# Dipet/pytorch_yolo

Measured on AMD Instinct MI355X. Metric: images/sec YOLOv3-SPP 640x640 bs=32, forward + decode + MERGE-NMS, pipelined batches, higher is better.
Workload: dtype bf16

## Files before the change

### include/yolo_hip.h

```cpp
#ifndef YOLO_HIP_H
#define YOLO_HIP_H

#include <stddef.h>
#include <stdint.h>

#ifdef __cplusplus
extern "C" {
#endif

typedef void* yolo_stream_t;

#if defined(__GNUC__)
#define YOLO_API __attribute__((visibility("default")))
#else
#define YOLO_API
#endif

enum { YOLO_E_ARG = -1, YOLO_E_UNSUPPORTED = -2, YOLO_E_WORKSPACE = -3 };
enum { YOLO_ACT_NONE = 0, YOLO_ACT_LEAKY01 = 1, YOLO_ACT_RELU6 = 2, YOLO_ACT_RELU = 3,
       YOLO_ACT_SWISH = 4  };
enum { YOLO_DT_BF16 = 0, YOLO_DT_F32 = 1, YOLO_DT_F16 = 2  };

YOLO_API const char* yolo_last_error(void);
YOLO_API int yolo_abi_version(void);
YOLO_API int yolo_set_tuning(int knob, int value);

YOLO_API int yolo_pack_input_nchw_f32(const float* x, void* y, int n, int c, int h, int w, int c_pad,
                             yolo_stream_t s);

typedef struct YoloConvDesc {
  int32_t n, h, w;
  int32_t cin;
  int32_t in_c_total, in_c_offset;
  int32_t ho, wo;
  int32_t cout;
  int32_t out_c_total, out_c_offset;
  int32_t ksize, stride, pad;
  int32_t act;
  int32_t upsample2x;
  int32_t out_dtype;
  int32_t kpad;
  int32_t cout_pad;
  int32_t res_c_total, res_c_offset;
  int32_t aux_c_total, aux_c_offset;
} YoloConvDesc;

YOLO_API int yolo_conv2d_fwd(const void* x, const void* w_packed, const float* bias, const void* residual,
                    void* y, void* y_preadd, const YoloConvDesc* d, yolo_stream_t s);

YOLO_API int yolo_conv2d_pick(const YoloConvDesc* d, int has_residual, int has_preadd, char* out, int out_len);

YOLO_API int yolo_conv2d_splitk_plan(const YoloConvDesc* d, int has_residual, int has_preadd, int* splits, size_t* ws_bytes,
                                     int* n_counters);
YOLO_API int yolo_conv2d_splitk_fwd(const void* x, const void* w_packed, const float* bias, const void* residual, void* y,
                                    void* y_preadd, const YoloConvDesc* d, int splits, void* workspace, size_t ws_bytes,
                                    int32_t* counters, yolo_stream_t s);

YOLO_API int yolo_conv1_nchw_f32_fwd(const float* x_nchw, int cin_real, const void* w_packed, const float* bias,
                                     void* y, const YoloConvDesc* d, yolo_stream_t s);
YOLO_API int yolo_conv1_pool_nchw_f32_fwd(const float* x_nchw, int cin_real, const void* w_packed, const float* bias,
                                          void* y_pooled, const YoloConvDesc* d, yolo_stream_t s);

YOLO_API int yolo_pack_conv_weight_f32(const float* w_oihw, int cout, int cin_w, int ksize, int cin,
                              int cout_pad, int kpad, uint16_t* out);

YOLO_API int yolo_conv3x3_pool_supported(int cin, int cout);
YOLO_API int yolo_conv3x3_pool_fwd(const void* x, const void* w_packed, const float* bias, void* y, const YoloConvDesc* d,
                                   int pool, yolo_stream_t s);

YOLO_API int yolo_dwconv3x3_fwd(const void* x, const float* w, const float* bias, void* y, int n, int h, int w_,
                       int c, int in_c_total, int in_c_offset, int ho, int wo, int out_c_total,
                       int out_c_offset, int stride, int act, yolo_stream_t s);

YOLO_API int yolo_dwconv_fwd(const void* x, const float* w, const float* bias, void* y, int n, int h, int w_, int c,
                             int in_c_total, int in_c_offset, int ho, int wo, int out_c_total, int out_c_offset, int ksize,
                             int stride, int pad, int act, yolo_stream_t s);

YOLO_API size_t yolo_se_workspace_bytes(int n, int c);
YOLO_API int yolo_se_fwd(const void* x, void* y, int n, int h, int w, int c, int in_c_total, int in_c_offset, int out_c_total,
                         int out_c_offset, const float* w1, const float* b1, const float* w2, const float* b2, int squeeze,
                         void* workspace, size_t ws_bytes, yolo_stream_t s);

YOLO_API int yolo_channel_shuffle2_fwd(const void* a, const void* b, void* y, int n, int h, int w, int half, int c_slot,
                                       int a_c_total, int a_c_offset, int b_c_total, int b_c_offset, int y_c_total,
                                       int y_c_offset, yolo_stream_t s);

YOLO_API int yolo_maxpool_fwd(const void* x, void* y, int n, int h, int w, int c, int in_c_total, int in_c_offset,
                     int ho, int wo, int out_c_total, int out_c_offset, int ksize, int stride, int pad,
                     int dilation, yolo_stream_t s);

YOLO_API int yolo_spp_fwd(void* buf, int n, int h, int w, int c, yolo_stream_t s);

YOLO_API int yolo_resunit_supported(int c, int h, int w);
YOLO_API int yolo_resunit_form(int c, int n, int h, int w);
YOLO_API int yolo_resunit_fwd(const void* x, const void* w1_packed, const float* b1, const void* w2_packed,
                              const float* b2, void* y, void* y_preadd, const YoloConvDesc* d, int kpad1,
                              int cout_pad1, yolo_stream_t s);

YOLO_API int yolo_stem_supported(int cin_real, int c1, int c2, int h, int w);
YOLO_API int yolo_stem_fwd(const float* x_nchw, int cin_real, const void* w1_packed, const float* b1, int kpad1,
                           const void* w2_packed, const float* b2, void* y, const YoloConvDesc* d, yolo_stream_t s);

typedef struct YoloMbconvDesc {
  int32_t n, h, w, cin, in_c_total, in_c_offset, hidden, cout, out_c_total, out_c_offset, stride, has_expand, has_res, _pad;
} YoloMbconvDesc;
YOLO_API int yolo_mbconv_dstride(int ce);
YOLO_API int yolo_mbconv_supported(int cin, int hidden, int cout, int stride);
YOLO_API int yolo_mbconv_fwd(const void* x, const void* w_exp, const float* b_exp, const float* w_dw, const float* b_dw,
                             const void* w_proj, const float* b_proj, void* y, const YoloMbconvDesc* d, yolo_stream_t s);

YOLO_API int yolo_decode_fwd(const float* head, int head_c_total, const float* anchors_px, int na, int nc, int bs,
                    int ny, int nx, float stride_px, float* io, int io_rows_total, int io_row_offset,
                    float* p, yolo_stream_t s);

YOLO_API int yolo_head_decode_supported(int cout, int na, int nc);
YOLO_API int yolo_head_decode_pick(const YoloConvDesc* d, int na, int nc, int filter, char* out, int out_len);
YOLO_API int yolo_head_decode_fwd(const void* x, const void* w_packed, const float* bias, const YoloConvDesc* d,
                                  const float* anchors_px, int na, int nc, float stride_px, float* io,
                                  int io_rows_total, int io_row_offset, float* p, yolo_stream_t s);

YOLO_API size_t yolo_nms_workspace_bytes(int bs, int rows, int nc);
YOLO_API int yolo_nms_merge(float* pred, int bs, int rows, int nc, float conf_thres, float nms_thres, float min_wh,
                   int max_per_class, int mutate_conf, float* out_dets, int32_t* out_idx,
                   int32_t* out_count, int cap, void* workspace, size_t workspace_bytes, yolo_stream_t s);

YOLO_API size_t yolo_nms_compact_workspace_bytes(int bs, int rows, int nc);
YOLO_API int yolo_head_decode_filter_fwd(const void* x, const void* w_packed, const float* bias, const YoloConvDesc* d,
                                         const float* anchors_px, int na, int nc, float stride_px, int io_rows_total,
                                         int io_row_offset, float conf_thres, float min_wh, void* workspace, size_t workspace_bytes,
                                         float* p, yolo_stream_t s);
YOLO_API int yolo_nms_merge_compact(void* workspace, size_t workspace_bytes, int bs, int rows, int nc, float nms_thres,
// ... 89 lines not shown
```

### pytorch_yolo_amd/_lib.py

```python
from __future__ import annotations

import ctypes as C
import os

_HERE = os.path.dirname(os.path.abspath(__file__))
LIB_PATH = os.environ.get("YOLO_HIP_LIB") or os.path.join(_HERE, "csrc", "libyolo_hip.so")

ABI_VERSION = 2
ACT_NONE, ACT_LEAKY01, ACT_RELU6, ACT_RELU, ACT_SWISH = 0, 1, 2, 3, 4
DT_BF16, DT_F32, DT_F16 = 0, 1, 2
OP_CONV, OP_MAXPOOL, OP_SPP, OP_DWCONV, OP_CONV1_NCHW, OP_RESUNIT, OP_STEM, OP_HEAD_DECODE, OP_CONV1_POOL = 1, 2, 3, 4, 5, 6, 7, 8, 9
OP_MBCONV, OP_CONV_POOL, OP_SHUFFLE, OP_CONV_F32, OP_MAXPOOL_F32, OP_SE = 10, 11, 12, 13, 14, 15
OP_CONV_F16, OP_MAXPOOL_F16, OP_HEAD_DECODE_F16 = 16, 17, 18
OP_CONV_T20_F16 = 19


class YoloConvDesc(C.Structure):
    _fields_ = [(n, C.c_int32) for n in (
        "n", "h", "w", "cin", "in_c_total", "in_c_offset", "ho", "wo", "cout",
        "out_c_total", "out_c_offset", "ksize", "stride", "pad", "act", "upsample2x",
        "out_dtype", "kpad", "cout_pad", "res_c_total", "res_c_offset",
        "aux_c_total", "aux_c_offset")]


class YoloOp(C.Structure):
    _fields_ = [("kind", C.c_int32), ("_pad", C.c_int32),
                ("x", C.c_void_p), ("w", C.c_void_p), ("bias", C.c_void_p),
                ("residual", C.c_void_p), ("y", C.c_void_p), ("y_aux", C.c_void_p),
                ("conv", YoloConvDesc),
                ("w_pre", C.c_void_p), ("bias_pre", C.c_void_p), ("kpad_pre", C.c_int32), ("cout_pad_pre", C.c_int32),
                ("head_anchors_px", C.c_float * 8), ("head_stride_px", C.c_float),
                ("head_na", C.c_int32), ("head_nc", C.c_int32), ("io_rows_total", C.c_int32),
                ("io_row_offset", C.c_int32), ("head_filter_conf", C.c_float),
                ("w_dw", C.c_void_p), ("bias_dw", C.c_void_p),
                ("workspace", C.c_void_p), ("counters", C.c_void_p), ("ws_bytes", C.c_size_t),
                ("splits", C.c_int32), ("head_filter_min_wh", C.c_float)]


class YoloMbconvDesc(C.Structure):
    _fields_ = [(n, C.c_int32) for n in (
        "n", "h", "w", "cin", "in_c_total", "in_c_offset", "hidden", "cout", "out_c_total", "out_c_offset",
        "stride", "has_expand", "has_res", "_pad")]


class YoloPipeStep(C.Structure):
    _fields_ = [("ops", C.POINTER(YoloOp)), ("n_ops", C.c_int32), ("k_io", C.c_int32),
                ("stream", C.c_void_p), ("nms_stream", C.c_void_p),
                ("wait_x", C.c_void_p), ("wait_io", C.c_void_p), ("heads_done", C.c_void_p), ("nms_done", C.c_void_p), ("done", C.c_void_p),
                ("io", C.c_void_p), ("bs", C.c_int32), ("rows", C.c_int32), ("nc", C.c_int32), ("max_per_class", C.c_int32),
                ("conf_thres", C.c_float), ("nms_thres", C.c_float), ("min_wh", C.c_float), ("cap", C.c_int32),
                ("out_dets", C.c_void_p), ("out_idx", C.c_void_p), ("out_count", C.c_void_p), ("workspace", C.c_void_p),
                ("workspace_bytes", C.c_size_t), ("count_host", C.c_void_p)]


SIGNATURES = {
    "yolo_last_error": (C.c_char_p, []),
    "yolo_abi_version": (C.c_int, []),
    "yolo_abi_sizeof": (C.c_int, [C.c_int]),
    "yolo_set_tuning": (C.c_int, [C.c_int, C.c_int]),
    "yolo_pack_input_nchw_f32": (C.c_int, [C.c_void_p, C.c_void_p] + [C.c_int] * 5 + [C.c_void_p]),
    "yolo_conv2d_fwd": (C.c_int, [C.c_void_p] * 6 + [C.POINTER(YoloConvDesc), C.c_void_p]),
    "yolo_conv2d_splitk_plan": (C.c_int, [C.POINTER(YoloConvDesc), C.c_int, C.c_int, C.POINTER(C.c_int), C.POINTER(C.c_size_t),
                                          C.POINTER(C.c_int)]),
    "yolo_conv2d_splitk_fwd": (C.c_int, [C.c_void_p] * 6 + [C.POINTER(YoloConvDesc), C.c_int, C.c_void_p, C.c_size_t, C.c_void_p,
                                         C.c_void_p]),
    "yolo_conv1_nchw_f32_fwd": (C.c_int, [C.c_void_p, C.c_int, C.c_void_p, C.c_void_p, C.c_void_p,
                                          C.POINTER(YoloConvDesc), C.c_void_p]),
    "yolo_conv1_pool_nchw_f32_fwd": (C.c_int, [C.c_void_p, C.c_int, C.c_void_p, C.c_void_p, C.c_void_p,
                                               C.POINTER(YoloConvDesc), C.c_void_p]),
    "yolo_conv2d_pick": (C.c_int, [C.POINTER(YoloConvDesc), C.c_int, C.c_int, C.c_char_p, C.c_int]),
    "yolo_pack_conv_weight_f32": (C.c_int, [C.c_void_p] + [C.c_int] * 6 + [C.c_void_p]),
    "yolo_stem_supported": (C.c_int, [C.c_int] * 5),
    "yolo_stem_fwd": (C.c_int, [C.c_void_p, C.c_int, C.c_void_p, C.c_void_p, C.c_int, C.c_void_p, C.c_void_p, C.c_void_p,
                                C.POINTER(YoloConvDesc), C.c_void_p]),
    "yolo_resunit_supported": (C.c_int, [C.c_int] * 3),
    "yolo_resunit_form": (C.c_int, [C.c_int] * 4),
    "yolo_resunit_fwd": (C.c_int, [C.c_void_p] * 7 + [C.POINTER(YoloConvDesc), C.c_int, C.c_int, C.c_void_p]),
    "yolo_conv3x3_pool_supported": (C.c_int, [C.c_int] * 2),
    "yolo_conv3x3_pool_fwd": (C.c_int, [C.c_void_p] * 4 + [C.POINTER(YoloConvDesc), C.c_int, C.c_void_p]),
    "yolo_mbconv_dstride": (C.c_int, [C.c_int]),
    "yolo_mbconv_supported": (C.c_int, [C.c_int] * 4),
    "yolo_mbconv_fwd": (C.c_int, [C.c_void_p] * 8 + [C.POINTER(YoloMbconvDesc), C.c_void_p]),
    "yolo_dwconv3x3_fwd": (C.c_int, [C.c_void_p] * 4 + [C.c_int] * 12 + [C.c_void_p]),
    "yolo_dwconv_fwd": (C.c_int, [C.c_void_p] * 4 + [C.c_int] * 14 + [C.c_void_p]),
    "yolo_se_workspace_bytes": (C.c_size_t, [C.c_int] * 2),
    "yolo_se_fwd": (C.c_int, [C.c_void_p] * 2 + [C.c_int] * 8 + [C.c_void_p] * 4 + [C.c_int, C.c_void_p, C.c_size_t, C.c_void_p]),
    "yolo_channel_shuffle2_fwd": (C.c_int, [C.c_void_p] * 3 + [C.c_int] * 11 + [C.c_void_p]),
    "yolo_maxpool_fwd": (C.c_int, [C.c_void_p] * 2 + [C.c_int] * 14 + [C.c_void_p]),
    "yolo_spp_fwd": (C.c_int, [C.c_void_p] + [C.c_int] * 4 + [C.c_void_p]),
    "yolo_decode_fwd": (C.c_int, [C.c_void_p, C.c_int, C.c_void_p] + [C.c_int] * 5 + [C.c_float, C.c_void_p,
                                  C.c_int, C.c_int, C.c_void_p, C.c_void_p]),
    "yolo_head_decode_supported": (C.c_int, [C.c_int] * 3),
    "yolo_head_decode_pick": (C.c_int, [C.POINTER(YoloConvDesc), C.c_int, C.c_int, C.c_int, C.c_char_p, C.c_int]),
    "yolo_head_decode_fwd": (C.c_int, [C.c_void_p] * 3 + [C.POINTER(YoloConvDesc), C.c_void_p, C.c_int, C.c_int, C.c_float,
                                       C.c_void_p, C.c_int, C.c_int, C.c_void_p, C.c_void_p]),
    "yolo_nms_workspace_bytes": (C.c_size_t, [C.c_int] * 3),
    "yolo_nms_merge": (C.c_int, [C.c_void_p] + [C.c_int] * 3 + [C.c_float] * 3 + [C.c_int] * 2 +
                       [C.c_void_p] * 3 + [C.c_int, C.c_void_p, C.c_size_t, C.c_void_p]),
    "yolo_nms_compact_workspace_bytes": (C.c_size_t, [C.c_int] * 3),
    "yolo_head_decode_filter_fwd": (C.c_int, [C.c_void_p] * 3 + [C.POINTER(YoloConvDesc), C.c_void_p, C.c_int, C.c_int, C.c_float,
                                              C.c_int, C.c_int, C.c_float, C.c_float, C.c_void_p, C.c_size_t, C.c_void_p, C.c_void_p]),
    "yolo_nms_merge_compact": (C.c_int, [C.c_void_p, C.c_size_t] + [C.c_int] * 3 + [C.c_float, C.c_int] + [C.c_void_p] * 3 +
                               [C.c_int, C.c_void_p]),
    "yolo_scale_coords": (C.c_int, [C.c_void_p, C.c_int, C.c_int, C.c_int, C.c_void_p, C.c_int, C.c_void_p]),
    "yolo_letterbox_u8_fwd": (C.c_int, [C.c_void_p] + [C.c_int] * 4 + [C.c_double] + [C.c_int] * 6 + [C.c_void_p, C.c_void_p] +
                              [C.c_int] * 4 + [C.c_float, C.c_void_p]),
    "yolo_conv2d_f32_fwd": (C.c_int, [C.c_void_p] * 6 + [C.POINTER(YoloConvDesc), C.c_void_p]),
    "yolo_maxpool_f32_fwd": (C.c_int, [C.c_void_p] * 2 + [C.c_int] * 14 + [C.c_void_p]),
    "yolo_pack_input_nchw_f32_nhwc": (C.c_int, [C.c_void_p, C.c_void_p] + [C.c_int] * 5 + [C.c_void_p]),
    "yolo_pack_conv_weight_f32_f32": (C.c_int, [C.c_void_p] + [C.c_int] * 6 + [C.c_void_p]),
    "yolo_conv2d_f16_fwd": (C.c_int, [C.c_void_p] * 6 + [C.POINTER(YoloConvDesc), C.c_void_p]),
    "yolo_conv3x3_t20_f16_supported": (C.c_int, [C.POINTER(YoloConvDesc), C.c_int, C.c_int]),
    "yolo_conv3x3_t20_f16_fwd": (C.c_int, [C.c_void_p] * 6 + [C.POINTER(YoloConvDesc), C.c_int, C.c_void_p]),
    "yolo_conv2d_f16_pick": (C.c_int, [C.POINTER(YoloConvDesc), C.c_int, C.c_int, C.c_char_p, C.c_int]),
    "yolo_head_decode_f16_pick": (C.c_int, [C.POINTER(YoloConvDesc), C.c_int, C.c_int, C.c_int, C.c_char_p, C.c_int]),
    "yolo_head_decode_f16_fwd": (C.c_int, [C.c_void_p] * 3 + [C.POINTER(YoloConvDesc), C.c_void_p, C.c_int, C.c_int, C.c_float,
                                           C.c_void_p, C.c_int, C.c_int, C.c_void_p, C.c_void_p]),
    "yolo_head_decode_filter_f16_fwd": (C.c_int, [C.c_void_p] * 3 + [C.POINTER(YoloConvDesc), C.c_void_p, C.c_int, C.c_int, C.c_float,
                                                  C.c_int, C.c_int, C.c_float, C.c_float, C.c_void_p, C.c_size_t, C.c_void_p, C.c_void_p]),
    "yolo_maxpool_f16_fwd": (C.c_int, [C.c_void_p] * 2 + [C.c_int] * 14 + [C.c_void_p]),
    "yolo_pack_input_nchw_f32_f16": (C.c_int, [C.c_void_p, C.c_void_p] + [C.c_int] * 5 + [C.c_void_p]),
    "yolo_pack_conv_weight_f32_f16": (C.c_int, [C.c_void_p] + [C.c_int] * 6 + [C.c_void_p]),
    "yolo_run_ops": (C.c_int, [C.POINTER(YoloOp), C.c_int, C.c_void_p]),
    "yolo_stream_create_cu_mask": (C.c_int, [C.POINTER(C.c_uint32), C.c_int, C.POINTER(C.c_void_p)]),
    "yolo_stream_destroy": (C.c_int, [C.c_void_p]),
    "yolo_set_launch_cus": (C.c_int, [C.c_int]),
    "yolo_event_create": (C.c_int, [C.POINTER(C.c_void_p)]),
    "yolo_event_destroy": (C.c_int, [C.c_void_p]),
    "yolo_event_record": (C.c_int, [C.c_void_p, C.c_void_p]),
    "yolo_event_synchronize": (C.c_int, [C.c_void_p]),
    "yolo_pipeline_step": (C.c_int, [C.POINTER(YoloPipeStep)]),
    "yolo_pack_detections": (C.c_int, [C.c_void_p, C.c_void_p, C.c_void_p, C.c_int, C.c_int, C.c_void_p, C.c_void_p, C.c_void_p]),
}

_lib = None


def load():
    global _lib
    if _lib is not None:
        return _lib
    if not os.path.exists(LIB_PATH):
        raise RuntimeError(
            f"{LIB_PATH} is missing: build it with `python -m pytorch_yolo_amd.build` "
            "(hipcc --offload-arch=gfx950). pytorch_yolo_amd has no CPU / eager fallback.")
    lib = C.CDLL(LIB_PATH)
    for name, (res, args) in SIGNATURES.items():
        fn = getattr(lib, name)
        fn.restype = res
        fn.argtypes = args
    if lib.yolo_abi_version() != ABI_VERSION:
        raise RuntimeError(f"libyolo_hip.so ABI version {lib.yolo_abi_version()} != {ABI_VERSION} of this binding: rebuild with "
                           "`python -m pytorch_yolo_amd.build --force`")
# ... 12 lines not shown
```

### pytorch_yolo_amd/csrc/conv1x1_stream.hip

```cpp
#include "conv_common.h"

using namespace yolo_conv;

namespace {

struct ActParams {
  bool floor0, swish;
  float slope, hi;
  __device__ explicit ActParams(int act)
      : floor0(act == YOLO_ACT_RELU || act == YOLO_ACT_RELU6), swish(act == YOLO_ACT_SWISH), slope(act == YOLO_ACT_LEAKY01 ? 0.1f : 1.f),
        hi(act_hi(act)) {}
  __device__ __forceinline__ float plain(float v) const { return fminf(fmaxf(v, floor0 ? 0.f : slope * v), hi); }
};

template <int N, int K>
__global__ __launch_bounds__(256, 2) void conv1x1_stream_kernel(const ConvArgs a, int n_tiles_px) {
  constexpr int P = 128, NF = N / 64, KC = K / 32;
  constexpr int XB = KC * P * 64;
  constexpr int SP = N * 2 + 16;
  static_assert((N == 64 || N == 128) && (K == 128 || K == 256), "shape");
  __shared__ __attribute__((aligned(16))) char smem[XB > P * SP ? XB : P * SP];

  const int tid = threadIdx.x, lane = tid & 63;
  const int wave = __builtin_amdgcn_readfirstlane(tid >> 6);
  const YoloConvDesc& d = a.d;
  const ActParams ap(d.act);
  const int c16 = lane & 15, q = lane >> 4;
  const __amdgpu_buffer_rsrc_t rx = __builtin_amdgcn_make_buffer_rsrc((void*)a.x, 0, a.x_bytes, 0x00020000);
  const uint32_t y_pitch = (uint32_t)d.out_c_total * 2u;
  const __amdgpu_buffer_rsrc_t ry = __builtin_amdgcn_make_buffer_rsrc(a.y, 0, (uint32_t)a.M * y_pitch, 0x00020000);

  bf16x8 wreg[NF][KC];
  f32x4 bv[NF];
#pragma unroll
  for (int f = 0; f < NF; ++f) {
    const int row = wave * 16 * NF + f * 16 + c16;
#pragma unroll
    for (int kc = 0; kc < KC; ++kc) wreg[f][kc] = *reinterpret_cast<const bf16x8*>(a.w + (long)row * d.kpad + kc * 32 + q * 8);
    bv[f] = *reinterpret_cast<const f32x4*>(a.bias + wave * 16 * NF + f * 16 + q * 4);
  }
  const int drow = lane >> 2, dchunk = (lane & 3) ^ swz32(lane >> 4);
  const uint32_t x_pitch = (uint32_t)d.in_c_total * 2u;
  const uint32_t lane_src = (uint32_t)drow * x_pitch + (uint32_t)(d.in_c_offset + dchunk * 8) * 2u;
  const uint32_t xfrag = (uint32_t)(c16 * 64 + ((q ^ swz32(c16 >> 2)) << 4));
  constexpr int LPR = N / 8, RPI = 64 / LPR;
  const int orow = lane / LPR, ocol = lane % LPR;

  for (int t = blockIdx.x; t < n_tiles_px; t += gridDim.x) {
    const int p0 = t * P;
#pragma unroll
    for (int i = 0; i < KC * 2; ++i) {
      const int piece = i * 4 + wave, kc = piece >> 3, pb = piece & 7;
      const int px = p0 + pb * 16 + drow;
      const uint32_t vo = px < a.M ? (uint32_t)(p0 + pb * 16) * x_pitch + lane_src : kOobOffset;
      if (!(a.debug & kCdNoPixelDma)) lds_dma16s(rx, smem + piece * 1024, vo, (uint32_t)kc * 64u);
    }
    wait_vmcnt<0>();
    __syncthreads();
    f32x4 acc[NF][8];
#pragma unroll
    for (int f = 0; f < NF; ++f)
#pragma unroll
      for (int j = 0; j < 8; ++j) acc[f][j] = f32x4{0.f, 0.f, 0.f, 0.f};
    if (!(a.debug & kCdNoMfma))
#pragma unroll
    for (int kc = 0; kc < KC; ++kc)
#pragma unroll
      for (int j = 0; j < 8; ++j) {
        const bf16x8 xf = *reinterpret_cast<const bf16x8*>(smem + (kc * 8 + j) * 1024 + xfrag);
#pragma unroll
        for (int f = 0; f < NF; ++f) acc[f][j] = __builtin_amdgcn_mfma_f32_16x16x32_bf16(wreg[f][kc], xf, acc[f][j], 0, 0, 0);
      }
    __syncthreads();
    if (a.debug & kCdNoEpilogue) continue;
    auto stage = [&](auto act) {
#pragma unroll
      for (int f = 0; f < NF; ++f)
#pragma unroll
        for (int j = 0; j < 8; ++j) {
          bf16x4 o;
#pragma unroll
          for (int e = 0; e < 4; ++e) o[e] = (bf16_t)act(acc[f][j][e] + bv[f][e]);
          *reinterpret_cast<bf16x4*>(smem + (j * 16 + c16) * SP + (wave * 16 * NF + f * 16 + q * 4) * 2) = o;
        }
    };
    if (ap.swish) stage([](float v) { return v / (1.f + expf(-v)); });
    else stage([&](float v) { return ap.plain(v); });
    __syncthreads();
#pragma unroll
    for (int i = 0; i < P / (4 * RPI); ++i) {
      const int row = (i * 4 + wave) * RPI + orow;
      const u32x4 v = *reinterpret_cast<const u32x4*>(smem + row * SP + ocol * 16);
      const uint32_t vo = p0 + row < a.M ? (uint32_t)(p0 + row) * y_pitch + (uint32_t)(d.out_c_offset + ocol * 8) * 2u : kOobOffset;
      __builtin_amdgcn_raw_buffer_store_b128(v, ry, vo, 0, 0);
    }
    wait_lds();
    __builtin_amdgcn_s_barrier();
  }
}

template <int N, int K, int P>
__global__ __launch_bounds__(256, 2) void conv1x1_stream2_kernel(const ConvArgs a, int n_tiles_px) {
  constexpr int NF = N / 64, KC = K / 32, PB = P / 16;
  constexpr int XB = KC * P * 64;
  constexpr int SP = N * 2 + 16;
  constexpr int NPW = KC * PB / 4;
  constexpr int LPR = N / 8, RPI = 64 / LPR, NST = P / (4 * RPI);
  constexpr int BUF = ((XB > P * SP ? XB : P * SP) + 1023) / 1024 * 1024;
  static_assert(N == 128 && (KC * PB) % 4 == 0 && P % (4 * RPI) == 0 && 2 * BUF <= 80 * 1024, "shape");
  static_assert(NPW + 2 * NST <= 60, "vmcnt is a 6-bit counter");
  __shared__ __attribute__((aligned(16))) char smem[2 * BUF];

  const int tid = threadIdx.x, lane = tid & 63;
  const int wave = __builtin_amdgcn_readfirstlane(tid >> 6);
  const YoloConvDesc& d = a.d;
  const ActParams ap(d.act);
  const int c16 = lane & 15, q = lane >> 4;
  const __amdgpu_buffer_rsrc_t rx = __builtin_amdgcn_make_buffer_rsrc((void*)a.x, 0, a.x_bytes, 0x00020000);
  const uint32_t y_pitch = (uint32_t)d.out_c_total * 2u;
  const __amdgpu_buffer_rsrc_t ry = __builtin_amdgcn_make_buffer_rsrc(a.y, 0, (uint32_t)a.M * y_pitch, 0x00020000);

  bf16x8 wreg[NF][KC];
  f32x4 bv[NF];
#pragma unroll
  for (int f = 0; f < NF; ++f) {
    const int row = wave * 16 * NF + f * 16 + c16;
#pragma unroll
    for (int kc = 0; kc < KC; ++kc) wreg[f][kc] = *reinterpret_cast<const bf16x8*>(a.w + (long)row * d.kpad + kc * 32 + q * 8);
    bv[f] = *reinterpret_cast<const f32x4*>(a.bias + wave * 16 * NF + f * 16 + q * 4);
  }
  const int drow = lane >> 2, dchunk = (lane & 3) ^ swz32(lane >> 4);
  const uint32_t x_pitch = (uint32_t)d.in_c_total * 2u;
  const uint32_t lane_src = (uint32_t)drow * x_pitch + (uint32_t)(d.in_c_offset + dchunk * 8) * 2u;
  const uint32_t xfrag = (uint32_t)(c16 * 64 + ((q ^ swz32(c16 >> 2)) << 4));
  const int orow = lane / LPR, ocol = lane % LPR;

  auto issue_tile = [&](int j) {
    const long t = (long)blockIdx.x + (long)j * gridDim.x;
    const long p0 = t * P;
    char* const buf = smem + (j & 1) * BUF;
#pragma unroll
    for (int i = 0; i < NPW; ++i) {
      const int piece = i * 4 + wave, kc = piece / PB, pb = piece - kc * PB;
      const long px = p0 + pb * 16 + drow;
      const uint32_t vo = (t < n_tiles_px && px < a.M) ? (uint32_t)(p0 + pb * 16) * x_pitch + lane_src : kOobOffset;
      lds_dma16s(rx, buf + piece * 1024, vo, (uint32_t)kc * 64u);
    }
#if defined(__HIP_DEVICE_COMPILE__)
    asm volatile("" ::: "memory");
#endif
  };

  const int nt = ((int)blockIdx.x < n_tiles_px) ? (n_tiles_px - 1 - (int)blockIdx.x) / (int)gridDim.x + 1 : 0;
  issue_tile(0);
  issue_tile(1);
  for (int j = 0; j < nt; ++j) {
    const long p0 = ((long)blockIdx.x + (long)j * gridDim.x) * P;
    char* const buf = smem + (j & 1) * BUF;
    if (j == 0) wait_vmcnt<NPW>();
    else if (j == 1) wait_vmcnt<NPW + NST>();
    else wait_vmcnt<NPW + 2 * NST>();
    __builtin_amdgcn_s_barrier();
    f32x4 acc[NF][PB];
#pragma unroll
    for (int f = 0; f < NF; ++f)
#pragma unroll
      for (int b = 0; b < PB; ++b) acc[f][b] = f32x4{0.f, 0.f, 0.f, 0.f};
#pragma unroll
    for (int kc = 0; kc < KC; ++kc)
#pragma unroll
      for (int b = 0; b < PB; ++b) {
        const bf16x8 xf = *reinterpret_cast<const bf16x8*>(buf + (kc * PB + b) * 1024 + xfrag);
#pragma unroll
        for (int f = 0; f < NF; ++f) acc[f][b] = __builtin_amdgcn_mfma_f32_16x16x32_bf16(wreg[f][kc], xf, acc[f][b], 0, 0, 0);
      }
    wait_lds();
    __builtin_amdgcn_s_barrier();
    auto stage = [&](auto act) {
#pragma unroll
      for (int f = 0; f < NF; ++f)
#pragma unroll
        for (int b = 0; b < PB; ++b) {
          bf16x4 o;
#pragma unroll
          for (int e = 0; e < 4; ++e) o[e] = (bf16_t)act(acc[f][b][e] + bv[f][e]);
          *reinterpret_cast<bf16x4*>(buf + (b * 16 + c16) * SP + (wave * 16 * NF + f * 16 + q * 4) * 2) = o;
        }
    };
    if (ap.swish) stage([](float v) { return v / (1.f + expf(-v)); });
    else stage([&](float v) { return ap.plain(v); });
    wait_lds();
    __builtin_amdgcn_s_barrier();
    u32x4 v[NST];
#pragma unroll
    for (int i = 0; i < NST; ++i) v[i] = *reinterpret_cast<const u32x4*>(buf + ((i * 4 + wave) * RPI + orow) * SP + ocol * 16);
    wait_lds();
    __builtin_amdgcn_s_barrier();
    issue_tile(j + 2);
#pragma unroll
    for (int i = 0; i < NST; ++i) {
      const int row = (i * 4 + wave) * RPI + orow;
      const uint32_t vo = p0 + row < a.M ? (uint32_t)(p0 + row) * y_pitch + (uint32_t)(d.out_c_offset + ocol * 8) * 2u : kOobOffset;
      __builtin_amdgcn_raw_buffer_store_b128(v[i], ry, vo, 0, 0);
    }
#if defined(__HIP_DEVICE_COMPILE__)
    asm volatile("" ::: "memory");
#endif
  }
  wait_vmcnt<0>();
}

template <int N, int K, int P>
int launch_stream2(const ConvArgs& a, hipStream_t s) {
  const int tiles = (a.M + P - 1) / P;
  const int grid = tiles < 512 ? tiles : 512;
  if (pick_only("stream1x1p<%d couts,K %d,%d px> grid %d", N, K, P, grid)) return 0;
  hipLaunchKernelGGL((conv1x1_stream2_kernel<N, K, P>), dim3((unsigned)grid), dim3(256), 0, s, a, tiles);
  return yolo_check_launch("yolo_conv2d_fwd(1x1 stream, pipelined)");
}

template <int N, int K>
int launch_stream(const ConvArgs& a, hipStream_t s) {
  const int tiles = (a.M + 127) / 128;
  const int grid = tiles < 512 ? tiles : 512;
  if (pick_only("stream1x1<%d couts,K %d> grid %d", N, K, grid)) return 0;
  hipLaunchKernelGGL((conv1x1_stream_kernel<N, K>), dim3((unsigned)grid), dim3(256), 0, s, a, tiles);
  return yolo_check_launch("yolo_conv2d_fwd(1x1 stream)");
}

}

int yolo_conv::launch_stream1x1(const ConvArgs& a, int force, hipStream_t s) {
  const YoloConvDesc& d = a.d;
  if (d.ksize != 1 || d.stride != 1 || d.pad != 0 || d.upsample2x || d.out_dtype != YOLO_DT_BF16 || a.res || a.aux) return 1;
  if (d.in_c_offset % 8 || d.in_c_total % 8 || d.out_c_offset % 8 || d.out_c_total % 8) return 1;
  if ((size_t)a.M * d.out_c_total * 2 >= kOobOffset) return 1;
  if (!force && a.M < 40000) return 1;
  if (!(a.debug & kCdStreamFirstForm)) {
    if (d.cout == 128 && d.cin == 256) return launch_stream2<128, 256, 80>(a, s);
    if (d.cout == 128 && d.cin == 128) return launch_stream2<128, 128, 80>(a, s);
    if (d.cout == 128 && d.cin == 384) return launch_stream2<128, 384, 48>(a, s);
  }
  if (d.cout == 128 && d.cin == 256) return launch_stream<128, 256>(a, s);
  if (d.cout == 128 && d.cin == 128) return launch_stream<128, 128>(a, s);
  if (d.cout == 64 && d.cin == 128) return launch_stream<64, 128>(a, s);
  if (d.cout == 64 && d.cin == 256) return launch_stream<64, 256>(a, s);
  return 1;
}
```

### pytorch_yolo_amd/csrc/conv_common.h

```cpp
#pragma once
#include "common.h"

#include <type_traits>
#include <utility>

namespace yolo_conv {

template <typename F, int... Is>
__device__ __forceinline__ void static_for_impl(F&& f, std::integer_sequence<int, Is...>) {
  (f(std::integral_constant<int, Is>{}), ...);
}
template <int N, typename F>
__device__ __forceinline__ void static_for(F&& f) {
  static_for_impl(f, std::make_integer_sequence<int, N>{});
}

template <typename T>
struct Pack;
template <>
struct Pack<bf16_t> {
  using x4 = bf16x4;
  using x8 = bf16x8;
};
template <>
struct Pack<f16_t> {
  using x4 = f16x4;
  using x8 = f16x8;
};
template <typename T>
__device__ __forceinline__ T narrow(float v) {
  if constexpr (std::is_same<T, f16_t>::value) {
    const float m = __builtin_fabsf(v);
    if (m > 65504.f && m < __builtin_inff()) v = __builtin_copysignf(65504.f, v);
  }
  return (T)v;
}

constexpr uint32_t kOobOffset = 0xF0000000u;

struct HeadDecodeArgs {
  float* io = nullptr;
  float* p = nullptr;
  int na = 0, no = 0, io_rows_total = 0, io_row_offset = 0;
  float stride = 0.f;
  float anchor_w[4] = {}, anchor_h[4] = {};
  float* rec = nullptr;
  unsigned long long* row_keys = nullptr;
  float conf_thres = 0.f, min_wh = 0.f;
};

struct ConvArgs {
  const bf16_t* x = nullptr;
  const bf16_t* w = nullptr;
  const float* bias = nullptr;
  const bf16_t* res = nullptr;
  void* y = nullptr;
  bf16_t* aux = nullptr;
  YoloConvDesc d = {};
  int M = 0;
  int n_tiles = 0;
  int steps = 0;
  uint32_t x_bytes = 0, w_bytes = 0;
  HeadDecodeArgs hd;
  int splits = 1;
  float* ws = nullptr;
  int* cnt = nullptr;
  int debug = 0;
#ifdef YOLO_STAMPS
  unsigned long long* stamps = nullptr;
#endif
};

inline size_t conv_x_bytes(const YoloConvDesc& d) { return (size_t)d.n * d.h * d.w * d.in_c_total * 2; }
inline size_t conv_w_bytes(const YoloConvDesc& d) { return (size_t)d.cout_pad * d.kpad * 2; }

inline ConvArgs make_conv_args(const void* x, const void* w, const float* bias, const void* res, void* y, void* aux, const YoloConvDesc& d) {
  ConvArgs a;
  a.x = (const bf16_t*)x;
  a.w = (const bf16_t*)w;
  a.bias = bias;
  a.res = (const bf16_t*)res;
  a.y = y;
  a.aux = (bf16_t*)aux;
  a.d = d;
  a.M = d.n * d.ho * d.wo;
  a.x_bytes = (uint32_t)conv_x_bytes(d);
  a.w_bytes = (uint32_t)conv_w_bytes(d);
  return a;
}

#ifdef YOLO_STAMPS
struct BlockStamp {
  unsigned long long* base_;
  unsigned long long* p;
  unsigned long long t0, c0;
  __device__ __forceinline__ unsigned long long* slot_() const {
    return base_ + 4 * ((size_t)blockIdx.x + (size_t)gridDim.x * (blockIdx.y + (size_t)gridDim.y * blockIdx.z)) + 1;
  }
  __device__ __forceinline__ explicit BlockStamp(unsigned long long* base) : base_(base), p(nullptr), t0(0), c0(0) {
    if (base && threadIdx.x == 0) {
      p = slot_() - 1;
      t0 = __builtin_amdgcn_s_memrealtime();
      c0 = __builtin_amdgcn_s_memtime();
    }
  }
  __device__ __forceinline__ ~BlockStamp() {
    if (p) {
      const unsigned long long c1 = __builtin_amdgcn_s_memtime();
      const unsigned hw = __builtin_amdgcn_s_getreg((31 << 11) | 4), xcc = __builtin_amdgcn_s_getreg((31 << 11) | 20);
      p[0] = t0;
      p[2] = c1 - c0;
      p[3] = (unsigned long long)hw | ((unsigned long long)xcc << 32);
    }
    if ((threadIdx.x & 63) == 0 && base_) atomicMax(slot_(), (unsigned long long)__builtin_amdgcn_s_memrealtime());
  }
};
inline unsigned long long* stamp_buffer_from_env() {
  static long launch_idx = 0;
  const char* e = getenv("YOLO_STAMP_PTR");
  if (!e) return nullptr;
  const char* st = getenv("YOLO_STAMP_STRIDE");
  const long stride = st ? atol(st) : 0;
  return (unsigned long long*)strtoull(e, nullptr, 0) + stride * launch_idx++;
}
#define YOLO_BLOCK_STAMP(args) BlockStamp block_stamp_((args).stamps)
#define YOLO_SET_STAMPS(args) (args).stamps = stamp_buffer_from_env()
#else
#define YOLO_BLOCK_STAMP(args)
#define YOLO_SET_STAMPS(args)
#endif

__device__ __forceinline__ void lds_dma16(__amdgpu_buffer_rsrc_t rsrc, char* lds_wave_base, uint32_t voffset) {
  __builtin_amdgcn_raw_ptr_buffer_load_lds(rsrc, (__attribute__((address_space(3))) void*)lds_wave_base, 16,
                                           voffset, 0, 0, 0);
}

__device__ __forceinline__ int swz32(int v) { return (0x78 >> (2 * (v & 3))) & 3; }

__device__ __forceinline__ float act_hi(int act) { return act == YOLO_ACT_RELU6 ? 6.f : __builtin_nanf(""); }

__device__ __forceinline__ float apply_act(float v, int act) {
  if (act == YOLO_ACT_SWISH) return v / (1.f + expf(-v));
  const bool floor0 = act == YOLO_ACT_RELU || act == YOLO_ACT_RELU6;
  const float slope = act == YOLO_ACT_LEAKY01 ? 0.1f : 1.f;
  return fminf(fmaxf(v, floor0 ? 0.f : slope * v), act_hi(act));
}

template <int N>
__device__ __forceinline__ void wait_vmcnt() {
#if defined(__HIP_DEVICE_COMPILE__)
  asm volatile("s_waitcnt vmcnt(%0)" ::"n"(N) : "memory");
#endif
}

typedef float f32x2 __attribute__((ext_vector_type(2)));
__device__ __forceinline__ float raw_max(float x, float y) {
  float r;
// ... 163 lines not shown
```

### pytorch_yolo_amd/csrc/conv_igemm.hip

```cpp
#include "conv_common.h"
#include "nms_common.h"
#include "head_epilogue.h"
#include <stdlib.h>

using namespace yolo_conv;

#ifdef YOLO_ABL_NOLDS
template <typename X8>
__device__ __forceinline__ X8 lds_frag_stub() {
  X8 v;
  asm volatile("" : "=v"(v));
  return v;
}
#define YOLO_LDS_FRAG(p) lds_frag_stub<X8>()
#else
#define YOLO_LDS_FRAG(p) (*reinterpret_cast<const X8*>(p))
#endif

namespace {

__device__ __forceinline__ f32x4 mfma16(bf16x8 w, bf16x8 x, f32x4 c) { return __builtin_amdgcn_mfma_f32_16x16x32_bf16(w, x, c, 0, 0, 0); }
__device__ __forceinline__ f32x4 mfma16(f16x8 w, f16x8 x, f32x4 c) { return __builtin_amdgcn_mfma_f32_16x16x32_f16(w, x, c, 0, 0, 0); }
__device__ __forceinline__ f32x16 mfma32(bf16x8 w, bf16x8 x, f32x16 c) { return __builtin_amdgcn_mfma_f32_32x32x16_bf16(w, x, c, 0, 0, 0); }
__device__ __forceinline__ f32x16 mfma32(f16x8 w, f16x8 x, f32x16 c) { return __builtin_amdgcn_mfma_f32_32x32x16_f16(w, x, c, 0, 0, 0); }

template <int BM, int BN, int WAVES_M, int WAVES_N, int BK, int NS, bool FAST, bool LDS_EPI, bool MFMA16 = false, bool DECODE = false,
          int NP = 0, bool SPLITK = false, typename T = bf16_t>
__global__ __launch_bounds__(64 * (WAVES_M * WAVES_N + NP)) void conv_igemm_kernel(const ConvArgs a) {
  using X4 = typename Pack<T>::x4;
  using X8 = typename Pack<T>::x8;
  static_assert(!SPLITK || (FAST && LDS_EPI && MFMA16 && !DECODE), "split-K: 16x16x32 path with the LDS epilogue");
  constexpr int NW = WAVES_M * WAVES_N;
  constexpr int NL = NP > 0 ? NP : NW;
  static_assert(NP == 0 || (NS <= 3 && FAST && NP % 2 == 0), "loader waves: 2- or 3-stage ring, FAST path");
  static_assert(NW == 4 || NW == 8 || NW == 16, "4, 8 or 16 waves");
  static_assert(BK == 32 || BK == 64, "BK");
  static_assert(NS >= 2 && NS <= 4, "ring depth");
  constexpr int TM = BM / WAVES_M, TN = BN / WAVES_N;
  constexpr int NI = TM / 32, MI = TN / 32;
  constexpr int ROWB = BK * 2;
  constexpr int CPR = BK / 8;
  constexpr int RPP = 1024 / ROWB;
  constexpr int BNL = BN < NL * RPP ? NL * RPP : BN;
  constexpr int PIT = BM / (NL * RPP), WIT = BNL / (NL * RPP);
  constexpr int LPS = PIT + WIT;
  constexpr int STAGE_B = (BM + BNL) * ROWB;
  static_assert(TM % 32 == 0 && TN % 32 == 0 && PIT >= 1 && WIT >= 1, "tile");
  static_assert(NS * STAGE_B <= 160 * 1024, "LDS");

  constexpr int RING_B = NS * STAGE_B;
  constexpr int DP = BN + 4;
  constexpr int EPI_B = DECODE ? BM * DP * 4 : (LDS_EPI ? NW * TM * kEpiPitch : 0);
  constexpr int LDS_B = EPI_B > RING_B ? EPI_B : RING_B;
  static_assert(!DECODE || (!LDS_EPI && !MFMA16 && BM % NW == 0), "DECODE instances use the plain 32x32 accumulators");
  __shared__ __attribute__((aligned(16))) char smem[LDS_B];

  YOLO_BLOCK_STAMP(a);
  const int tid = threadIdx.x, lane = tid & 63;
  const int wave = __builtin_amdgcn_readfirstlane(tid >> 6);
  const int wm = wave / WAVES_N, wn = wave % WAVES_N;
  const int lw = NP == 0 ? wave : wave - NW;
  const YoloConvDesc& d = a.d;

  int m0, n0;
  {
    const int swz = xcd_swizzle(blockIdx.x, gridDim.x);
    const int mt = swz / a.n_tiles;
    m0 = mt * BM;
    n0 = (swz - mt * a.n_tiles) * BN;
  }

  const __amdgpu_buffer_rsrc_t rx = __builtin_amdgcn_make_buffer_rsrc((void*)a.x, 0, a.x_bytes, 0x00020000);
  const __amdgpu_buffer_rsrc_t rw = __builtin_amdgcn_make_buffer_rsrc((void*)a.w, 0, a.w_bytes, 0x00020000);

  const int frow = lane / CPR;
  const int fsw = (BK == 32) ? swz32(lane >> 4) : (((lane >> 4) + 4 * (lw & 1)) & 7);
  const int chunk = (lane & (CPR - 1)) ^ fsw;
  const int ntaps = d.ksize * d.ksize;
  int px_base[PIT], px_hi0[PIT], px_wi0[PIT];
  uint32_t px_mask[PIT];
  const int hw_out = d.ho * d.wo;
#pragma unroll
  for (int it = 0; it < PIT; ++it) {
    const int m = m0 + (it * NL + lw) * RPP + frow;
    const bool ok = m < a.M;
    const int mm = ok ? m : 0;
    const int b = mm / hw_out, rem = mm - b * hw_out;
    const int oh = rem / d.wo, ow = rem - oh * d.wo;
    px_hi0[it] = oh * d.stride - d.pad;
    px_wi0[it] = ow * d.stride - d.pad;
    px_base[it] = ((b * d.h + px_hi0[it]) * d.w + px_wi0[it]) * d.in_c_total + d.in_c_offset;
    uint32_t mask;
    if (d.ksize == 3) {
      uint32_t cb = 0, rb = 0;
#pragma unroll
      for (int t = 0; t < 3; ++t) {
        cb |= (uint32_t)((unsigned)(px_wi0[it] + t) < (unsigned)d.w) << t;
        rb |= (uint32_t)((unsigned)(px_hi0[it] + t) < (unsigned)d.h) << t;
      }
      mask = ((rb & 1) ? cb : 0) | ((rb & 2) ? cb << 3 : 0) | ((rb & 4) ? cb << 6 : 0);
    } else {
      mask = ((unsigned)px_hi0[it] < (unsigned)d.h && (unsigned)px_wi0[it] < (unsigned)d.w) ? 1u : 0u;
    }
    if (!ok) mask = 0;
    px_mask[it] = mask;
    if (FAST) px_base[it] = (px_base[it] + chunk * 8) * 2;
  }
  uint32_t w_off[WIT];
#pragma unroll
  for (int it = 0; it < WIT; ++it) {
    const int row = (it * NL + lw) * RPP + frow;
    w_off[it] = row < BN ? (uint32_t)(((n0 + row) * d.kpad + chunk * 8) * 2) : kOobOffset;
  }
  int tap = FAST ? 0 : (chunk * 8) / d.cin;
  int kc = FAST ? 0 : chunk * 8 - tap * d.cin;
  if constexpr (SPLITK) {
    const int k0 = blockIdx.y * a.steps * BK;
    tap = k0 / d.cin;
    kc = k0 - tap * d.cin;
#pragma unroll
    for (int it = 0; it < WIT; ++it)
      if (w_off[it] != kOobOffset) w_off[it] += (uint32_t)k0 * 2u;
  }

  int st_dh = 0, st_dw = 0;
  auto stage_begin = [&]() {
    st_dh = st_dw = 0;
    if (d.ksize == 3) {
      st_dh = (tap * 11) >> 5;
      st_dw = tap - 3 * st_dh;
    }
  };
  auto issue = [&](int buf, int step, int lo, int hi) {
    char* const wb = smem + buf * STAGE_B + lw * 1024;
    char* const xb = wb + BNL * ROWB;
    if (FAST) {
      const uint32_t tap_off = (uint32_t)(((st_dh * d.w + st_dw) * d.in_c_total + kc) * 2);
      const uint32_t bit = (kc + chunk * 8 < d.cin) ? 1u << tap : 0u;
#pragma unroll
      for (int it = 0; it < PIT; ++it) {
        if (it < lo || it >= hi) continue;
        const uint32_t voff = (px_mask[it] & bit) ? (uint32_t)px_base[it] + tap_off : kOobOffset;
        if (!(a.debug & kCdNoPixelDma)) lds_dma16(rx, xb + it * (NL * 1024), voff);
      }
#pragma unroll
      for (int it = 0; it < WIT; ++it) {
        if (PIT + it < lo || PIT + it >= hi) continue;
        if (!(a.debug & kCdNoWeightDma)) lds_dma16s(rw, wb + it * (NL * 1024), w_off[it], (uint32_t)step * (BK * 2u));
      }
    } else {
      const bool tap_ok = tap < ntaps;
      const int tap_off = (st_dh * d.w + st_dw) * d.in_c_total + kc;
#pragma unroll
      for (int it = 0; it < PIT; ++it) {
        if (it < lo || it >= hi) continue;
        const bool ok = tap_ok && ((px_mask[it] >> (tap_ok ? tap : 0)) & 1u);
        const uint32_t voff = ok ? (uint32_t)(px_base[it] + tap_off) * 2u : kOobOffset;
        lds_dma16(rx, xb + it * (NL * 1024), voff);
      }
#pragma unroll
      for (int it = 0; it < WIT; ++it) {
        if (PIT + it < lo || PIT + it >= hi) continue;
        const uint32_t voff = w_off[it] == kOobOffset ? kOobOffset : w_off[it] + (uint32_t)step * (BK * 2u);
        lds_dma16(rw, wb + it * (NL * 1024), voff);
      }
    }
  };
  auto stage_end = [&]() {
    kc += BK;
    if (FAST) {
      if (kc >= d.cin) {
        kc = 0;
        ++tap;
      }
    } else {
      while (kc >= d.cin) {
        kc -= d.cin;
        ++tap;
      }
    }
  };

  if constexpr (NP > 0) {
    if (wave >= NW) {
#pragma unroll
      for (int p = 0; p < NS - 1; ++p)
        if (p < a.steps) {
          stage_begin();
          issue(p, p, 0, LPS);
          stage_end();
        }
      int slot = NS - 1;
      for (int s = 0; s < a.steps; ++s) {
        if (NS == 3 && s + 1 < a.steps) wait_vmcnt<LPS>();
        else wait_vmcnt<0>();
        __builtin_amdgcn_s_barrier();
        if (s + NS - 1 < a.steps) {
          stage_begin();
          issue(slot, s + NS - 1, 0, LPS);
          stage_end();
        }
        if (++slot == NS) slot = 0;
      }
      return;
    }
  }

  static_assert(!MFMA16 || LDS_EPI, "the 16x16x32 path only has the LDS epilogue");
  constexpr int MI16 = MFMA16 ? TN / 16 : 1, NI16 = MFMA16 ? TM / 16 : 1;
  f32x16 acc[MFMA16 ? 1 : MI][MFMA16 ? 1 : NI];
  f32x4 acc16[MI16][NI16];
#pragma unroll
  for (int i = 0; i < (MFMA16 ? 1 : MI); ++i)
#pragma unroll
    for (int j = 0; j < (MFMA16 ? 1 : NI); ++j)
#pragma unroll
      for (int e = 0; e < 16; ++e) acc[i][j][e] = 0.f;
#pragma unroll
  for (int i = 0; i < MI16; ++i)
#pragma unroll
    for (int j = 0; j < NI16; ++j)
#pragma unroll
      for (int e = 0; e < 4; ++e) acc16[i][j][e] = 0.f;

  const int r32 = lane & 31, khalf = lane >> 5;
  const int steps = a.steps;
  constexpr int KS = BK / 16;

  if constexpr (NP == 0) {
#pragma unroll
  for (int p = 0; p < NS - 1; ++p)
    if (p < steps) {
      stage_begin();
      issue(p, p, 0, LPS);
      stage_end();
    }
  }

  auto pix_of = [&](int row) -> long {
    const int pix = m0 + wm * TM + row;
    return pix < a.M ? (long)pix : -1L;
  };

  int buf = 0;
  for (int s = 0; s < steps; ++s) {
    if constexpr (NP == 0) {
      const int younger = min(NS - 2, steps - 1 - s);
      if (younger >= 2) wait_vmcnt<2 * LPS>();
      else if (younger == 1) wait_vmcnt<1 * LPS>();
      else wait_vmcnt<0>();
    }
#ifndef YOLO_ABL_NOBARRIER
    __builtin_amdgcn_s_barrier();
#endif
    const bool more = NP == 0 && s + NS - 1 < steps;
    int nb = buf + NS - 1;
    if (nb >= NS) nb -= NS;
    if (more) stage_begin();
    const char* wbuf = smem + buf * STAGE_B;
    const char* xbuf = wbuf + BNL * ROWB;
// ... 141 lines not shown
            for (int z = 0; z < a.splits; ++z)
#pragma unroll
              for (int e = 0; e < 4; ++e) sum[e] += __hip_atomic_load(a.ws + z * slice + o + e, __ATOMIC_RELAXED, __HIP_MEMORY_SCOPE_AGENT);
          acc16[i][j] = sum;
        }
      if (tid == 0) __hip_atomic_store(a.cnt + blockIdx.x, 0, __ATOMIC_RELAXED, __HIP_MEMORY_SCOPE_AGENT);
    }
    epilogue_lds16<MI, NI16, TM, T>(a, acc16, smem + wave * (TM * kEpiPitch), lane, n0 + wn * TN, pix_of);
  } else if constexpr (LDS_EPI) {
    __syncthreads();
    epilogue_lds<MI, NI, TM, T>(a, acc, smem + wave * (TM * kEpiPitch), lane, n0 + wn * TN, pix_of);
  } else {
#pragma unroll
  for (int j = 0; j < NI; ++j) {
    const int pix = m0 + wm * TM + j * 32 + r32;
    if (pix >= a.M) continue;
    long out_pix = pix;
    int out_row_pitch = 0;
    if (d.upsample2x) {
      const int b = pix / hw_out, rem = pix - b * hw_out;
      const int oh = rem / d.wo, ow = rem - oh * d.wo;
      out_row_pitch = 2 * d.wo;
      out_pix = ((long)(b * 2 * d.ho + 2 * oh)) * out_row_pitch + 2 * ow;
    }
#pragma unroll
    for (int i = 0; i < MI; ++i) {
#pragma unroll
      for (int g4 = 0; g4 < 4; ++g4) {
        const int c0 = n0 + wn * TN + i * 32 + g4 * 8 + khalf * 4;
        if (c0 >= d.cout) continue;
        const f32x4 bv = *reinterpret_cast<const f32x4*>(a.bias + c0);
        float v[4];
#pragma unroll
        for (int e = 0; e < 4; ++e) v[e] = apply_act(acc[i][j][g4 * 4 + e] + bv[e], d.act);
        const bool full = c0 + 3 < d.cout;
        if (a.aux) {
          T* ap = reinterpret_cast<T*>(a.aux) + (long)pix * d.aux_c_total + d.aux_c_offset + c0;
          if (full) {
            X4 o = {narrow<T>(v[0]), narrow<T>(v[1]), narrow<T>(v[2]), narrow<T>(v[3])};
            *reinterpret_cast<X4*>(ap) = o;
          } else {
            for (int e = 0; e < 4 && c0 + e < d.cout; ++e) ap[e] = narrow<T>(v[e]);
          }
        }
        if (a.res) {
          const T* rp = reinterpret_cast<const T*>(a.res) + (long)pix * d.res_c_total + d.res_c_offset + c0;
          if (full) {
            const X4 rv = *reinterpret_cast<const X4*>(rp);
#pragma unroll
            for (int e = 0; e < 4; ++e) v[e] += (float)rv[e];
          } else {
            for (int e = 0; e < 4 && c0 + e < d.cout; ++e) v[e] += (float)rp[e];
          }
        }
        const int reps = d.upsample2x ? 4 : 1;
        for (int rep = 0; rep < reps; ++rep) {
          const long op = out_pix + (rep >> 1) * out_row_pitch + (rep & 1);
          const long eo = op * d.out_c_total + d.out_c_offset + c0;
          if (f32_out) {
            float* yp = reinterpret_cast<float*>(a.y) + eo;
            if (full) {
              f32x4 o = {v[0], v[1], v[2], v[3]};
              *reinterpret_cast<f32x4*>(yp) = o;
            } else {
              for (int e = 0; e < 4 && c0 + e < d.cout; ++e) yp[e] = v[e];
            }
          } else {
            T* yp = reinterpret_cast<T*>(a.y) + eo;
            if (full) {
              X4 o = {narrow<T>(v[0]), narrow<T>(v[1]), narrow<T>(v[2]), narrow<T>(v[3])};
              *reinterpret_cast<X4*>(yp) = o;
            } else {
              for (int e = 0; e < 4 && c0 + e < d.cout; ++e) yp[e] = narrow<T>(v[e]);
            }
          }
        }
      }
    }
  }
  }
}

template <int BM, int BN, int WAVES_M, int WAVES_N, int BK, int NS, bool FAST, bool LDS_EPI, bool MFMA16 = false, bool DECODE = false,
          int NP = 0, bool SPLITK = false, typename T = bf16_t>
int launch_cfg(const ConvArgs& a, hipStream_t s) {
  const int m_tiles = (a.M + BM - 1) / BM;
  ConvArgs b = a;
  b.n_tiles = (a.d.cout + BN - 1) / BN;
  b.steps = (a.d.ksize * a.d.ksize * a.d.cin + BK - 1) / BK;
  const long grid = (long)m_tiles * b.n_tiles;
  if (grid > 0x7fffffffL) return yolo_set_error(YOLO_E_UNSUPPORTED, "conv grid too large");
  if (pick_only("%s<%dx%d,%dx%d waves%s,BK%d,%d stages%s%s%s%s> grid %ld", std::is_same<T, f16_t>::value ? "igemm_f16" : "igemm", BM, BN, WAVES_M, WAVES_N, NP ? "+4 loaders" : "", BK, NS,
                FAST ? "" : ",generic", MFMA16 ? ",16x16x32" : ",32x32x16", DECODE ? ",decode" : "", SPLITK ? ",splitK" : "", grid))
    return 0;
  unsigned gy = 1;
  if constexpr (SPLITK) {
    YOLO_REQUIRE(a.splits >= 2 && b.steps % a.splits == 0 && a.ws && a.cnt, "split-K: %d K steps do not split %d ways", b.steps, a.splits);
    b.steps /= a.splits;
    gy = (unsigned)a.splits;
  }
  hipLaunchKernelGGL((conv_igemm_kernel<BM, BN, WAVES_M, WAVES_N, BK, NS, FAST, LDS_EPI, MFMA16, DECODE, NP, SPLITK, T>),
                     dim3((unsigned)grid, gy), dim3(64 * (WAVES_M * WAVES_N + NP)), 0, s, b);
  return yolo_check_launch("yolo_conv2d_fwd");
}

}

namespace yolo_conv {
static thread_local char* g_pick = nullptr;
static thread_local int g_pick_len = 0;
char* pick_buffer() { return g_pick; }
bool pick_only(const char* fmt, ...) {
  if (!g_pick) return false;
  va_list ap;
  va_start(ap, fmt);
  vsnprintf(g_pick, g_pick_len, fmt, ap);
  va_end(ap);
  return true;
}
}

static int env_int(const char* name, int unset) {
  const char* e = getenv(name);
  return e ? atoi(e) : unset;
}
Tuning& tuning() {
  static Tuning t{env_int("YOLO_CONV_VARIANT", -1), env_int("YOLO_CONV_DEBUG", 0), env_int("YOLO_CONV_PP", 0),
                  env_int("YOLO_RESUNIT_DEBUG", 0), env_int("YOLO_MBCONV_DEBUG", 0)};
  return t;
}

extern "C" int yolo_set_tuning(int knob, int value) {
  static constexpr int Tuning::* kKnobs[] = {&Tuning::variant, &Tuning::conv_debug, &Tuning::families, &Tuning::resunit, &Tuning::mbconv};
  YOLO_REQUIRE(knob >= 0 && knob < 5, "set_tuning: unknown knob %d", knob);
  int& slot = tuning().*kKnobs[knob];
  const int old = slot;
  slot = value;
  return old;
}

namespace {

#define YOLO_IGEMM_INSTANCES(X)                                                         \
  X(k64x256_8w_decode, 64, 256, 1, 8, 64, 2, true, false, false, true, 0, false)        \
  X(k64x256_bk32_decode, 64, 256, 1, 4, 32, 2, true, false, false, true, 0, false)      \
  X(k64x256_bk32_generic_decode, 64, 256, 1, 4, 32, 2, false, false, false, true, 0, false) \
  X(k256x32_m32, 256, 32, 4, 1, 32, 2, true, true, false, false, 0, false)              \
  X(k256x32_m32_direct, 256, 32, 4, 1, 32, 2, true, false, false, false, 0, false)      \
  X(k256x32_m32_generic, 256, 32, 4, 1, 32, 2, false, true, false, false, 0, false)     \
  X(k256x32_m32_generic_direct, 256, 32, 4, 1, 32, 2, false, false, false, false, 0, false) \
  X(k256x64_m32, 256, 64, 4, 1, 32, 2, true, true, false, false, 0, false)              \
  X(k256x64_m32_direct, 256, 64, 4, 1, 32, 2, true, false, false, false, 0, false)      \
  X(k256x64_m32_generic, 256, 64, 4, 1, 32, 2, false, true, false, false, 0, false)     \
  X(k256x64_m32_generic_direct, 256, 64, 4, 1, 32, 2, false, false, false, false, 0, false) \
  X(k128x128_bk32_3st_m32, 128, 128, 2, 2, 32, 3, true, true, false, false, 0, false)   \
  X(k128x128_bk32_3st_m32_direct, 128, 128, 2, 2, 32, 3, true, false, false, false, 0, false) \
  X(k128x128_bk32_3st_m32_generic, 128, 128, 2, 2, 32, 3, false, true, false, false, 0, false) \
  X(k128x128_bk32_3st_m32_generic_direct, 128, 128, 2, 2, 32, 3, false, false, false, false, 0, false) \
  X(k128x128_m32, 128, 128, 2, 2, 64, 2, true, true, false, false, 0, false)            \
  X(k128x128_m32_direct, 128, 128, 2, 2, 64, 2, true, false, false, false, 0, false)    \
  X(k128x128_bk32_m32, 128, 128, 2, 2, 32, 2, true, true, false, false, 0, false)       \
  X(k128x128_bk32_m32_direct, 128, 128, 2, 2, 32, 2, true, false, false, false, 0, false) \
  X(k128x64_m32, 128, 64, 2, 2, 64, 2, true, true, false, false, 0, false)              \
  X(k128x64_m32_direct, 128, 64, 2, 2, 64, 2, true, false, false, false, 0, false)      \
  X(k64x128_m32, 64, 128, 2, 2, 64, 2, true, true, false, false, 0, false)              \
  X(k64x128_m32_direct, 64, 128, 2, 2, 64, 2, true, false, false, false, 0, false)      \
  X(k64x64_m32, 64, 64, 2, 2, 64, 2, true, true, false, false, 0, false)                \
  X(k64x64_m32_direct, 64, 64, 2, 2, 64, 2, true, false, false, false, 0, false)        \
  X(k256x128_8w_m32, 256, 128, 4, 2, 64, 2, true, true, false, false, 0, false)         \
  X(k256x128_8w_m32_direct, 256, 128, 4, 2, 64, 2, true, false, false, false, 0, false) \
  X(k256x128_8w_bk32_m32, 256, 128, 4, 2, 32, 2, true, true, false, false, 0, false)    \
  X(k256x128_8w_bk32_m32_direct, 256, 128, 4, 2, 32, 2, true, false, false, false, 0, false) \
  X(k256x256_8w_m32, 256, 256, 4, 2, 64, 2, true, true, false, false, 0, false)         \
  X(k256x256_8w_m32_direct, 256, 256, 4, 2, 64, 2, true, false, false, false, 0, false) \
  X(k64x64_4st, 64, 64, 2, 2, 64, 4, true, true, true, false, 0, false)                 \
  X(k64x64_4st_splitk, 64, 64, 2, 2, 64, 4, true, true, true, false, 0, true)           \
  X(k64x64, 64, 64, 2, 2, 64, 2, true, true, true, false, 0, false)                     \
  X(k128x128, 128, 128, 2, 2, 64, 2, true, true, true, false, 0, false)                 \
  X(k128x128_8w, 128, 128, 2, 4, 64, 2, true, true, true, false, 0, false)              \
  X(k128x128_8w_3st, 128, 128, 2, 4, 64, 3, true, true, true, false, 0, false)          \
  X(k128x256_8w, 128, 256, 2, 4, 64, 2, true, true, true, false, 0, false)              \
  X(k128x256_16w_3st, 128, 256, 2, 8, 64, 3, true, true, true, false, 0, false)         \
  X(k128x256_loaders, 128, 256, 2, 4, 64, 2, true, true, true, false, 4, false)         \
  X(k128x256_loaders_3st, 128, 256, 2, 4, 64, 3, true, true, true, false, 4, false)     \
// ... 87 lines not shown
    case 8: return EPI(k128x64_m32);
    case 10: return EPI(k64x128_m32);
    case 11: return EPI(k64x64_m32);
    case 9: return EPI(k256x128_8w_bk32_m32);
    case 5: return EPI(k256x256_8w_m32);
    default: return EPI(k128x128_m32);
  }
#undef EPI
}

#define YOLO_IGEMM_F16_INSTANCES(X)                                                     \
  X(k64x256_8w_decode, 64, 256, 1, 8, 64, 2, true, false, false, true, 0, false)        \
  X(k64x256_bk32_decode, 64, 256, 1, 4, 32, 2, true, false, false, true, 0, false)      \
  X(k64x256_bk32_generic_decode, 64, 256, 1, 4, 32, 2, false, false, false, true, 0, false) \
  X(k256x32_m32, 256, 32, 4, 1, 32, 2, true, true, false, false, 0, false)              \
  X(k256x32_m32_direct, 256, 32, 4, 1, 32, 2, true, false, false, false, 0, false)      \
  X(k256x32_m32_generic, 256, 32, 4, 1, 32, 2, false, true, false, false, 0, false)     \
  X(k256x32_m32_generic_direct, 256, 32, 4, 1, 32, 2, false, false, false, false, 0, false) \
  X(k256x64_m32, 256, 64, 4, 1, 32, 2, true, true, false, false, 0, false)              \
  X(k256x64_m32_direct, 256, 64, 4, 1, 32, 2, true, false, false, false, 0, false)      \
  X(k256x64_m32_generic, 256, 64, 4, 1, 32, 2, false, true, false, false, 0, false)     \
  X(k256x64_m32_generic_direct, 256, 64, 4, 1, 32, 2, false, false, false, false, 0, false) \
  X(k128x128_bk32_3st_m32, 128, 128, 2, 2, 32, 3, true, true, false, false, 0, false)   \
  X(k128x128_bk32_3st_m32_direct, 128, 128, 2, 2, 32, 3, true, false, false, false, 0, false) \
  X(k128x128_bk32_3st_m32_generic, 128, 128, 2, 2, 32, 3, false, true, false, false, 0, false) \
  X(k128x128_bk32_3st_m32_generic_direct, 128, 128, 2, 2, 32, 3, false, false, false, false, 0, false) \
  X(k64x64_4st, 64, 64, 2, 2, 64, 4, true, true, true, false, 0, false)                 \
  X(k64x64, 64, 64, 2, 2, 64, 2, true, true, true, false, 0, false)                     \
  X(k64x64_m32_direct, 64, 64, 2, 2, 64, 2, true, false, false, false, 0, false)        \
  X(k128x128_8w, 128, 128, 2, 4, 64, 2, true, true, true, false, 0, false)              \
  X(k128x128_8w_3st, 128, 128, 2, 4, 64, 3, true, true, true, false, 0, false)          \
  X(k128x128_m32_direct, 128, 128, 2, 2, 64, 2, true, false, false, false, 0, false)    \
  X(k128x256_8w, 128, 256, 2, 4, 64, 2, true, true, true, false, 0, false)              \
  X(k128x256_16w_3st, 128, 256, 2, 8, 64, 3, true, true, true, false, 0, false)         \
  X(k256x128_8w_bk32, 256, 128, 4, 2, 32, 2, true, true, true, false, 0, false)         \
  X(k256x128_8w_bk32_m32_direct, 256, 128, 4, 2, 32, 2, true, false, false, false, 0, false) \
  X(k256x256_16w, 256, 256, 4, 4, 64, 2, true, true, true, false, 0, false)             \
  X(k256x256_8w_m32_direct, 256, 256, 4, 2, 64, 2, true, false, false, false, 0, false)

enum class IgemmF16Id {
#define X(id, ...) id,
  YOLO_IGEMM_F16_INSTANCES(X)
#undef X
};

int launch_igemm_f16(IgemmF16Id id, const ConvArgs& a, hipStream_t s) {
  switch (id) {
#define X(id, ...) \
  case IgemmF16Id::id: return launch_cfg<__VA_ARGS__, f16_t>(a, s);
    YOLO_IGEMM_F16_INSTANCES(X)
#undef X
  }
  return yolo_set_error(YOLO_E_UNSUPPORTED, "conv: unknown fp16 kernel instance %d", (int)id);
}

IgemmF16Id choose_igemm_f16(const YoloConvDesc& d, bool has_res, bool has_aux, bool head, int n_cu) {
  using I = IgemmF16Id;
  if (head) {
    if (d.cin % 64 == 0) return I::k64x256_8w_decode;
    return d.cin % 32 == 0 ? I::k64x256_bk32_decode : I::k64x256_bk32_generic_decode;
  }
  const long M = (long)d.n * d.ho * d.wo;
  const bool one_tap = d.ksize == 1 && d.cin % 8 == 0;
  const bool fast64 = d.cin % 64 == 0, fast32 = d.cin % 32 == 0 || one_tap;
  const bool epi = lds_epilogue_views(d, has_res, has_aux, YOLO_DT_F16);
#define EPI(id) (epi ? I::id : I::id##_direct)
  if (d.cout <= 32) return fast32 ? EPI(k256x32_m32) : EPI(k256x32_m32_generic);
  if (few_pixels_64_couts(d, M, n_cu) && epi) return I::k64x64_4st;
  if (d.cout <= 64) return fast32 ? EPI(k256x64_m32) : EPI(k256x64_m32_generic);
  if (!fast64) return fast32 ? EPI(k128x128_bk32_3st_m32) : EPI(k128x128_bk32_3st_m32_generic);
#undef EPI
  const long tiles128 = ((M + 127) / 128) * ((d.cout + 127) / 128);
  if (d.ksize == 1 && tiles128 < n_cu) {
    if (!epi) return I::k64x64_m32_direct;
    return tiles128 >= 64 ? I::k128x128_8w_3st : I::k64x64;
  }
  if (d.ksize == 1 && d.cin <= 512 && M >= 40000) return epi ? I::k256x128_8w_bk32 : I::k256x128_8w_bk32_m32_direct;
  if (fills_256x256(d, M, n_cu)) return epi ? I::k256x256_16w : I::k256x256_8w_m32_direct;
  if (!epi) return I::k128x128_m32_direct;
  if (one_round_128x256(d, M, n_cu)) return d.ksize == 1 ? I::k128x256_16w_3st : I::k128x256_8w;
  return I::k128x128_8w;
}

struct SplitK {
  int splits = 1;
  float* ws = nullptr;
  int* cnt = nullptr;
};

int conv2d_launch_ex(const void* x, const void* w, const float* bias, const void* res, void* y, void* y_aux, const YoloConvDesc* dp,
                     const HeadDecodeArgs* hd, const SplitK& sk, hipStream_t s, int dt = YOLO_DT_BF16) {
  YOLO_REQUIRE(x && w && bias && (y || hd) && dp, "conv: null pointer");
  const YoloConvDesc& d = *dp;
  YOLO_REQUIRE(d.ksize == 1 || d.ksize == 3, "conv: ksize %d unsupported (1 or 3)", d.ksize);
  YOLO_REQUIRE(d.stride == 1 || d.stride == 2, "conv: stride %d unsupported", d.stride);
  YOLO_REQUIRE(d.cin > 0 && d.cin % 8 == 0, "conv: cin %d must be a positive multiple of 8", d.cin);
  YOLO_REQUIRE(d.in_c_offset % 8 == 0 && d.in_c_total % 8 == 0 && d.in_c_offset + d.cin <= d.in_c_total,
               "conv: bad input view (cin %d, offset %d, total %d)", d.cin, d.in_c_offset, d.in_c_total);
  YOLO_REQUIRE(d.out_c_offset % 4 == 0 && d.out_c_total % 4 == 0 && d.out_c_offset + d.cout <= d.out_c_total,
               "conv: bad output view (cout %d, offset %d, total %d)", d.cout, d.out_c_offset, d.out_c_total);
  YOLO_REQUIRE(d.kpad % 64 == 0 && d.kpad >= d.ksize * d.ksize * d.cin, "conv: kpad %d must be a multiple of 64", d.kpad);
  YOLO_REQUIRE(d.cout_pad % 128 == 0 && d.cout_pad >= d.cout, "conv: cout_pad %d", d.cout_pad);
  const int ho_std = (d.h + 2 * d.pad - d.ksize) / d.stride + 1, wo_std = (d.w + 2 * d.pad - d.ksize) / d.stride + 1;
  YOLO_REQUIRE((d.ho == ho_std || (d.ho == ho_std + 1 && (d.ho - 1) * d.stride - d.pad < d.h)) &&
                   (d.wo == wo_std || (d.wo == wo_std + 1 && (d.wo - 1) * d.stride - d.pad < d.w)),
               "conv: output size %dx%d inconsistent with input %dx%d k%d s%d p%d", d.ho, d.wo, d.h, d.w, d.ksize,
               d.stride, d.pad);
  const bool std_out = d.ho == ho_std && d.wo == wo_std;
  if (res) YOLO_REQUIRE(d.res_c_total % 4 == 0 && d.res_c_offset % 4 == 0 && !d.upsample2x, "conv: bad residual view");
  if (y_aux) YOLO_REQUIRE(d.aux_c_total % 4 == 0 && d.aux_c_offset % 4 == 0, "conv: bad aux view");
  YOLO_REQUIRE(conv_x_bytes(d) < kOobOffset && conv_w_bytes(d) < kOobOffset, "conv: tensor larger than 3.75 GiB not supported");
  const long M = (long)d.n * d.ho * d.wo;
  YOLO_REQUIRE(M > 0 && M < 0x7fffffffL / 4, "conv: M out of range");

  const Tuning& t = tuning();
  ConvArgs a = make_conv_args(x, w, bias, res, y, y_aux, d);
  a.debug = t.conv_debug;
  a.splits = sk.splits;
  a.ws = sk.ws;
  a.cnt = sk.cnt;
  YOLO_SET_STAMPS(a);
  if (hd) a.hd = *hd;
  if (dt == YOLO_DT_F16) {
    YOLO_REQUIRE(d.out_dtype == YOLO_DT_F16 || d.out_dtype == YOLO_DT_F32, "conv_f16: out_dtype %d (YOLO_DT_F16 or YOLO_DT_F32)", d.out_dtype);
    YOLO_REQUIRE(a.splits <= 1, "conv_f16: no split-K form");
    a.debug = 0;
    return launch_igemm_f16(choose_igemm_f16(d, res != nullptr, y_aux != nullptr, hd != nullptr, g_launch_cus), a, s);
  }
  const bool others = !hd && t.variant < 0 && std_out && lds_epilogue_views(d, res != nullptr, y_aux != nullptr) && !(t.conv_debug & kCdNoLdsEpilogue);
  if (others && !(t.families & kFamT20Never) && a.splits <= 1) {
    const int rc = launch_t20_3x3(a, t.families & kFamT20Always ? 1 : 0, s);
    if (rc != 1) return rc;
  }
  if (others && d.ksize == 1 && !(t.families & kFamStreamNever) && a.splits <= 1) {
    const int rc = launch_stream1x1(a, t.families & kFamStreamAlways ? 1 : 0, s);
    if (rc != 1) return rc;
  }
  if (others && !(t.conv_debug & kCdNoHalo) && !(t.families & kFamNoHalo)) {
    const int rc = launch_halo3x3(a, s);
    if (rc != 1) return rc;
  }
  return launch_igemm(choose_igemm(d, res != nullptr, y_aux != nullptr, hd != nullptr, a.splits, g_launch_cus, t), a, s);
}

YoloConvDesc head_desc(const YoloConvDesc& d) {
  YoloConvDesc dd = d;
  dd.out_dtype = YOLO_DT_F32;
  dd.out_c_total = (d.cout + 3) & ~3;
  dd.out_c_offset = 0;
  return dd;
}

HeadDecodeArgs make_head_args(float* io, float* p, int na, int nc, int io_rows_total, int io_row_offset, float stride_px,
                              const float* anchors_px) {
  HeadDecodeArgs h;
  h.io = io;
  h.p = p;
  h.na = na;
  h.no = nc + 5;
  h.io_rows_total = io_rows_total;
  h.io_row_offset = io_row_offset;
  h.stride = stride_px;
  for (int i = 0; i < na; ++i) {
    h.anchor_w[i] = anchors_px[2 * i] / stride_px;
    h.anchor_h[i] = anchors_px[2 * i + 1] / stride_px;
  }
  return h;
}

}

namespace yolo_conv {
int launch_cus() { return g_launch_cus; }
}

extern "C" int yolo_set_launch_cus(int n_cu) {
  YOLO_REQUIRE(n_cu >= 8 && n_cu <= 1024, "set_launch_cus: %d out of range", n_cu);
  const int old = g_launch_cus;
  g_launch_cus = n_cu;
  return old;
}

int yolo_conv2d_launch(const void* x, const void* w, const float* bias, const void* res, void* y, void* y_aux,
                       const YoloConvDesc* dp, hipStream_t s) {
  return conv2d_launch_ex(x, w, bias, res, y, y_aux, dp, nullptr, SplitK(), s);
}

static int conv1_nchw(const float* x_nchw, int cin_real, const void* w_packed, const float* bias, void* y, const YoloConvDesc* dp,
                      bool pool, yolo_stream_t s) {
  YOLO_REQUIRE(x_nchw && w_packed && bias && y && dp, "conv1: null pointer");
  const YoloConvDesc& d = *dp;
  YOLO_REQUIRE(cin_real >= 1 && cin_real <= 8 && d.cin == 8, "conv1: 1..8 input channels (packed K uses cin = 8)");
  YOLO_REQUIRE(d.out_c_offset % 8 == 0 && d.out_c_total % 8 == 0 && d.out_c_offset + d.cout <= d.out_c_total, "conv1: bad output view");
  YOLO_REQUIRE((d.stride == 1 && d.ho == d.h && d.wo == d.w) ||
                   (d.stride == 2 && !pool && d.ho == (d.h - 1) / 2 + 1 && d.wo == (d.w - 1) / 2 + 1),
               "conv1: 3x3 / pad 1 at stride 1, or at stride 2 (cout 32, no pool) only");
  ConvArgs a = make_conv_args(nullptr, w_packed, bias, nullptr, y, nullptr, d);
  a.n_tiles = 1;
  a.x_bytes = a.w_bytes = 0;
  YOLO_SET_STAMPS(a);
  const int rc = d.stride == 2 ? launch_conv1_s2_nchw(a, x_nchw, cin_real, (hipStream_t)s)
                               : launch_conv1_nchw(a, x_nchw, cin_real, pool, (hipStream_t)s);
  if (rc == 1) return yolo_set_error(YOLO_E_UNSUPPORTED, "conv1: shape not covered (3x3 s1 with cout 16 or 32, 3x3 s2 with cout 32; bf16 out)");
  return rc;
}

extern "C" int yolo_conv1_nchw_f32_fwd(const float* x_nchw, int cin_real, const void* w_packed, const float* bias, void* y,
                                       const YoloConvDesc* dp, yolo_stream_t s) {
  return conv1_nchw(x_nchw, cin_real, w_packed, bias, y, dp, false, s);
}

extern "C" int yolo_conv1_pool_nchw_f32_fwd(const float* x_nchw, int cin_real, const void* w_packed, const float* bias,
                                            void* y_pooled, const YoloConvDesc* dp, yolo_stream_t s) {
  return conv1_nchw(x_nchw, cin_real, w_packed, bias, y_pooled, dp, true, s);
}

static int conv2d_pick(const YoloConvDesc* d, int has_residual, int has_preadd, char* out, int out_len, int dt) {
  YOLO_REQUIRE(d && out && out_len > 0, "conv2d_pick: bad arguments");
  out[0] = 0;
  yolo_conv::g_pick = out;
  yolo_conv::g_pick_len = out_len;
  static const char dummy[16] = {0};
  const int rc = conv2d_launch_ex(dummy, dummy, (const float*)dummy, has_residual ? dummy : nullptr, (void*)dummy,
                                  has_preadd ? (void*)dummy : nullptr, d, nullptr, SplitK(), nullptr, dt);
  yolo_conv::g_pick = nullptr;
  return rc;
}
extern "C" int yolo_conv2d_pick(const YoloConvDesc* d, int has_residual, int has_preadd, char* out, int out_len) {
  return conv2d_pick(d, has_residual, has_preadd, out, out_len, YOLO_DT_BF16);
}
extern "C" int yolo_conv2d_f16_pick(const YoloConvDesc* d, int has_residual, int has_preadd, char* out, int out_len) {
  return conv2d_pick(d, has_residual, has_preadd, out, out_len, YOLO_DT_F16);
}

extern "C" int yolo_conv2d_f16_fwd(const void* x, const void* w_packed, const float* bias, const void* residual, void* y,
                                   void* y_preadd, const YoloConvDesc* d, yolo_stream_t s) {
  return conv2d_launch_ex(x, w_packed, bias, residual, y, y_preadd, d, nullptr, SplitK(), (hipStream_t)s, YOLO_DT_F16);
}

extern "C" int yolo_conv2d_fwd(const void* x, const void* w_packed, const float* bias, const void* residual, void* y,
                               void* y_preadd, const YoloConvDesc* d, yolo_stream_t s) {
  return yolo_conv2d_launch(x, w_packed, bias, residual, y, y_preadd, d, (hipStream_t)s);
}

extern "C" int yolo_conv2d_splitk_plan(const YoloConvDesc* dp, int has_residual, int has_preadd, int* splits, size_t* ws_bytes,
                                       int* n_counters) {
  YOLO_REQUIRE(dp && splits && ws_bytes && n_counters, "splitk_plan: null pointer");
  const YoloConvDesc& d = *dp;
  *splits = 1;
  *ws_bytes = 0;
  *n_counters = 0;
  constexpr int kPlanCus = 256;
  const long M = (long)d.n * d.ho * d.wo;
  if (!lds_epilogue_views(d, has_residual, has_preadd) || d.cin % 64 != 0 || d.upsample2x || (long)d.h * d.w >= 80 * 80) return 0;
  long tiles;
  if (few_pixels_64_couts(d, M, kPlanCus)) tiles = (M + 63) / 64;
  else if (d.ksize == 3 && d.stride == 1 && !fills_256x256(d, M, kPlanCus) && one_round_128x256(d, M, kPlanCus)) tiles = ((M + 127) / 128) * (d.cout / 256);
  else return 0;
  const int steps = d.ksize * d.ksize * d.cin / 64;
  if (tiles == 0 || tiles >= 200) return 0;
  int best = 1;
  for (int sp = 2; sp <= 8; ++sp)
    if (steps % sp == 0 && steps / sp >= 6 && tiles * sp <= 256) best = sp;
  if (best > 1) {
    *splits = best;
    *ws_bytes = (size_t)best * d.n * d.ho * d.wo * d.cout * sizeof(float);
    *n_counters = (int)tiles;
  }
  return 0;
}

extern "C" int yolo_conv2d_splitk_fwd(const void* x, const void* w_packed, const float* bias, const void* residual, void* y,
                                      void* y_preadd, const YoloConvDesc* d, int splits, void* workspace, size_t ws_bytes,
                                      int32_t* counters, yolo_stream_t s) {
  YOLO_REQUIRE(d && splits >= 2 && workspace && counters, "splitk: bad arguments");
  int want;
  size_t need;
  int ncnt;
  const int rc0 = yolo_conv2d_splitk_plan(d, residual != nullptr, y_preadd != nullptr, &want, &need, &ncnt);
  if (rc0) return rc0;
  YOLO_REQUIRE(want >= 2, "splitk: this layer does not take a split-K launch");
  YOLO_REQUIRE((size_t)splits * d->n * d->ho * d->wo * d->cout * sizeof(float) <= ws_bytes, "splitk: workspace too small");
  return conv2d_launch_ex(x, w_packed, bias, residual, y, y_preadd, d, nullptr, SplitK{splits, (float*)workspace, counters}, (hipStream_t)s);
}

extern "C" int yolo_head_decode_supported(int cout, int na, int nc) {
  return na >= 1 && na <= 4 && nc >= 1 && cout == na * (5 + nc) && cout <= 256 && 5 + nc <= 128;
}

static int head_decode(const void* x, const void* w_packed, const float* bias, const YoloConvDesc* dp, const float* anchors_px, int na,
                       int nc, float stride_px, float* io, int io_rows_total, int io_row_offset, float* p, yolo_stream_t s, int dt) {
  YOLO_REQUIRE(dp && anchors_px && io, "head_decode: null pointer");
  const YoloConvDesc& d = *dp;
  YOLO_REQUIRE(yolo_head_decode_supported(d.cout, na, nc), "head_decode: cout %d != na*(5+nc) = %d*%d or out of range", d.cout, na,
               5 + nc);
  YOLO_REQUIRE(d.stride == 1 && !d.upsample2x, "head_decode: stride-1 head convs only");
  YOLO_REQUIRE(io_row_offset >= 0 && io_row_offset + na * d.ho * d.wo <= io_rows_total, "head_decode: rows out of range");
  YOLO_REQUIRE(stride_px > 0.f, "head_decode: bad stride");
  const HeadDecodeArgs h = make_head_args(io, p, na, nc, io_rows_total, io_row_offset, stride_px, anchors_px);
  const YoloConvDesc dd = head_desc(d);
  return conv2d_launch_ex(x, w_packed, bias, nullptr, nullptr, nullptr, &dd, &h, SplitK(), (hipStream_t)s, dt);
}
extern "C" int yolo_head_decode_fwd(const void* x, const void* w_packed, const float* bias, const YoloConvDesc* dp,
                                    const float* anchors_px, int na, int nc, float stride_px, float* io, int io_rows_total,
                                    int io_row_offset, float* p, yolo_stream_t s) {
  return head_decode(x, w_packed, bias, dp, anchors_px, na, nc, stride_px, io, io_rows_total, io_row_offset, p, s, YOLO_DT_BF16);
}
extern "C" int yolo_head_decode_f16_fwd(const void* x, const void* w_packed, const float* bias, const YoloConvDesc* dp,
                                        const float* anchors_px, int na, int nc, float stride_px, float* io, int io_rows_total,
                                        int io_row_offset, float* p, yolo_stream_t s) {
  return head_decode(x, w_packed, bias, dp, anchors_px, na, nc, stride_px, io, io_rows_total, io_row_offset, p, s, YOLO_DT_F16);
}

static int head_decode_pick(const YoloConvDesc* dp, int na, int nc, int filter, char* out, int out_len, int dt) {
  YOLO_REQUIRE(dp && out && out_len > 0, "head_decode_pick: bad arguments");
  YOLO_REQUIRE(yolo_head_decode_supported(dp->cout, na, nc), "head_decode_pick: cout %d != na*(5+nc)", dp->cout);
  out[0] = 0;
  static float dummy[16] = {0};
  static const float ones[8] = {1.f, 1.f, 1.f, 1.f, 1.f, 1.f, 1.f, 1.f};
  HeadDecodeArgs h = make_head_args(filter ? nullptr : dummy, nullptr, na, nc, na * dp->ho * dp->wo, 0, 1.f, ones);
// ... 105 lines not shown
```

### pytorch_yolo_amd/csrc/runtime.hip

```cpp
#include "common.h"

static thread_local char g_err[512] = "";

int yolo_set_error(int code, const char* fmt, ...) {
  va_list ap;
  va_start(ap, fmt);
  vsnprintf(g_err, sizeof(g_err), fmt, ap);
  va_end(ap);
  return code;
}

extern "C" const char* yolo_last_error(void) { return g_err; }
extern "C" int yolo_abi_version(void) { return 2; }
extern "C" int yolo_abi_sizeof(int which) {
  switch (which) {
    case 0: return (int)sizeof(YoloConvDesc);
    case 1: return (int)sizeof(YoloOp);
    case 2: return (int)sizeof(YoloMbconvDesc);
    case 3: return (int)sizeof(YoloPipeStep);
    default: return -1;
  }
}

extern "C" int yolo_stream_create_cu_mask(const uint32_t* cu_mask, int n_words, yolo_stream_t* out) {
  YOLO_REQUIRE(cu_mask && out && n_words > 0 && n_words <= 64, "stream_create_cu_mask: bad arguments");
  bool any = false;
  for (int i = 0; i < n_words; ++i) any |= cu_mask[i] != 0;
  YOLO_REQUIRE(any, "stream_create_cu_mask: empty mask");
  hipStream_t st = nullptr;
  hipError_t e = hipExtStreamCreateWithCUMask(&st, (uint32_t)n_words, cu_mask);
  if (e != hipSuccess) return yolo_set_error((int)e, "hipExtStreamCreateWithCUMask: %s", hipGetErrorString(e));
  *out = (yolo_stream_t)st;
  return 0;
}
extern "C" int yolo_stream_destroy(yolo_stream_t s) {
  YOLO_REQUIRE(s, "stream_destroy: null stream");
  hipError_t e = hipStreamDestroy((hipStream_t)s);
  if (e != hipSuccess) return yolo_set_error((int)e, "hipStreamDestroy: %s", hipGetErrorString(e));
  return 0;
}

extern "C" int yolo_run_ops(const YoloOp* ops, int n_ops, yolo_stream_t s) {
  YOLO_REQUIRE(ops || n_ops == 0, "run_ops: null op list");
  for (int i = 0; i < n_ops; ++i) {
    const YoloOp& o = ops[i];
    const YoloConvDesc& d = o.conv;
    int rc;
    switch (o.kind) {
      case YOLO_OP_CONV:
        rc = o.splits >= 2 ? yolo_conv2d_splitk_fwd(o.x, o.w, o.bias, o.residual, o.y, o.y_aux, &d, o.splits, o.workspace, o.ws_bytes,
                                                    o.counters, s)
                           : yolo_conv2d_launch(o.x, o.w, o.bias, o.residual, o.y, o.y_aux, &d, (hipStream_t)s);
        break;
      case YOLO_OP_CONV1_NCHW:
        rc = yolo_conv1_nchw_f32_fwd((const float*)o.x, d.res_c_total, o.w, o.bias, o.y, &d, s);
        break;
      case YOLO_OP_CONV1_POOL:
        rc = yolo_conv1_pool_nchw_f32_fwd((const float*)o.x, d.res_c_total, o.w, o.bias, o.y, &d, s);
        break;
      case YOLO_OP_MAXPOOL:
        rc = yolo_maxpool_fwd(o.x, o.y, d.n, d.h, d.w, d.cin, d.in_c_total, d.in_c_offset, d.ho, d.wo, d.out_c_total,
                              d.out_c_offset, d.ksize, d.stride, d.pad, d.upsample2x , s);
        break;
      case YOLO_OP_SPP:
        rc = yolo_spp_fwd(o.y, d.n, d.h, d.w, d.cin, s);
        break;
      case YOLO_OP_DWCONV:
        rc = d.ksize == 0 ? yolo_dwconv3x3_fwd(o.x, (const float*)o.w, o.bias, o.y, d.n, d.h, d.w, d.cin, d.in_c_total, d.in_c_offset, d.ho,
                                               d.wo, d.out_c_total, d.out_c_offset, d.stride, d.act, s)
                          : yolo_dwconv_fwd(o.x, (const float*)o.w, o.bias, o.y, d.n, d.h, d.w, d.cin, d.in_c_total, d.in_c_offset, d.ho,
                                            d.wo, d.out_c_total, d.out_c_offset, d.ksize, d.stride, d.pad, d.act, s);
        break;
      case YOLO_OP_SE:
        rc = yolo_se_fwd(o.x, o.y, d.n, d.h, d.w, d.cin, d.in_c_total, d.in_c_offset, d.out_c_total, d.out_c_offset, (const float*)o.w,
                         o.bias, (const float*)o.w_pre, o.bias_pre, o.kpad_pre, o.workspace, o.ws_bytes, s);
        break;
      case YOLO_OP_RESUNIT:
        rc = yolo_resunit_fwd(o.x, o.w_pre, o.bias_pre, o.w, o.bias, o.y, o.y_aux, &d, o.kpad_pre, o.cout_pad_pre, s);
        break;
      case YOLO_OP_STEM:
        rc = yolo_stem_fwd((const float*)o.x, d.res_c_total, o.w_pre, o.bias_pre, o.kpad_pre, o.w, o.bias, o.y, &d, s);
        break;
      case YOLO_OP_HEAD_DECODE:
        if (!o.y && o.workspace) {
          rc = yolo_head_decode_filter_fwd(o.x, o.w, o.bias, &d, o.head_anchors_px, o.head_na, o.head_nc, o.head_stride_px, o.io_rows_total,
                                           o.io_row_offset, o.head_filter_conf, o.head_filter_min_wh, o.workspace, o.ws_bytes,
                                           (float*)o.y_aux, s);
          break;
        }
        rc = yolo_head_decode_fwd(o.x, o.w, o.bias, &d, o.head_anchors_px, o.head_na, o.head_nc, o.head_stride_px, (float*)o.y,
                                  o.io_rows_total, o.io_row_offset, (float*)o.y_aux, s);
        break;
      case YOLO_OP_SHUFFLE:
        rc = yolo_channel_shuffle2_fwd(o.x, o.residual, o.y, d.n, d.h, d.w, d.cout, d.cin, d.in_c_total, d.in_c_offset, d.res_c_total,
                                       d.res_c_offset, d.out_c_total, d.out_c_offset, s);
        break;
      case YOLO_OP_CONV_F32:
        rc = yolo_conv2d_f32_fwd((const float*)o.x, (const float*)o.w, o.bias, (const float*)o.residual, (float*)o.y, (float*)o.y_aux, &d, s);
        break;
      case YOLO_OP_MAXPOOL_F32:
        rc = yolo_maxpool_f32_fwd((const float*)o.x, (float*)o.y, d.n, d.h, d.w, d.cin, d.in_c_total, d.in_c_offset, d.ho, d.wo,
                                  d.out_c_total, d.out_c_offset, d.ksize, d.stride, d.pad, d.upsample2x , s);
        break;
      case YOLO_OP_CONV_F16:
        rc = yolo_conv2d_f16_fwd(o.x, o.w, o.bias, o.residual, o.y, o.y_aux, &d, s);
        break;
      case YOLO_OP_CONV_T20_F16:
        rc = yolo_conv3x3_t20_f16_fwd(o.x, o.w, o.bias, o.residual, o.y, o.y_aux, &d, 1, s);
        break;
      case YOLO_OP_MAXPOOL_F16:
        rc = yolo_maxpool_f16_fwd(o.x, o.y, d.n, d.h, d.w, d.cin, d.in_c_total, d.in_c_offset, d.ho, d.wo, d.out_c_total, d.out_c_offset,
                                  d.ksize, d.stride, d.pad, d.upsample2x , s);
        break;
      case YOLO_OP_HEAD_DECODE_F16:
        if (!o.y && o.workspace) {
          rc = yolo_head_decode_filter_f16_fwd(o.x, o.w, o.bias, &d, o.head_anchors_px, o.head_na, o.head_nc, o.head_stride_px,
                                               o.io_rows_total, o.io_row_offset, o.head_filter_conf, o.head_filter_min_wh, o.workspace,
                                               o.ws_bytes, (float*)o.y_aux, s);
          break;
        }
        rc = yolo_head_decode_f16_fwd(o.x, o.w, o.bias, &d, o.head_anchors_px, o.head_na, o.head_nc, o.head_stride_px, (float*)o.y,
                                      o.io_rows_total, o.io_row_offset, (float*)o.y_aux, s);
        break;
      case YOLO_OP_CONV_POOL:
        rc = yolo_conv3x3_pool_fwd(o.x, o.w, o.bias, o.y, &d, 1, s);
        break;
      case YOLO_OP_MBCONV: {
        YoloMbconvDesc m;
        m.n = d.n, m.h = d.h, m.w = d.w, m.cin = d.cin, m.in_c_total = d.in_c_total, m.in_c_offset = d.in_c_offset;
        m.hidden = o.kpad_pre, m.cout = d.cout, m.out_c_total = d.out_c_total, m.out_c_offset = d.out_c_offset;
        m.stride = d.stride, m.has_expand = o.w_pre != nullptr, m.has_res = d.res_c_total != 0, m._pad = 0;
        rc = yolo_mbconv_fwd(o.x, o.w_pre, o.bias_pre, o.w_dw, o.bias_dw, o.w, o.bias, o.y, &m, s);
// ... 66 lines not shown
```

### pytorch_yolo_amd/csrc/tuning.h

```cpp
#pragma once

struct Tuning {
  int variant = -1, conv_debug = 0, families = 0, resunit = 0, mbconv = 0;
};
Tuning& tuning();

enum : int {
  kCdNoPixelDma = 1,
  kCdNoWeightDma = 2,
  kCdNoMfma = 4,
  kCdNoEpilogue = 8,
  kCdNoLdsEpilogue = 16,
  kCdNoHalo = 32,
  kCdNo128x256 = 128,
  kCdNoLoaderWaves = 256,
  kCd256x256EightWaves = 512,
  kCdHalo256Couts = 1024,
  kCdMfma32x32 = 2048,
  kCdFourWaves = 8192,
  kCdLoadersTwoStages = 16384,
  kCdTinyGrid64x64 = 32768,
  kCdHaloMfma32x32 = 65536,
  kCd64x64TwoStages = 4194304,
  kCdT20NoChunkPairs = 16777216,
  kCdStreamFirstForm = 33554432,
  kCdOneTapGeneric = 268435456,
};

enum : int {
  kFamNoHalo = 8,
  kFamT20Always = 16,
  kFamT20Never = 64,
  kFamStreamNever = 1024,
  kFamStreamAlways = 2048,
};

enum : int {
  kRuNoMfmaA = 1,
  kRuNoMfmaB = 2,
  kRuNoEpilogue = 4,
  kRuNoPixelDma = 8,
  kRuT20NoEpilogue = 8,
  kRuNoMidRows = 16,
  kRuGeneric64 = 32,
  kRuT20Always = 64,
  kRuT20Never = 128,
  kRuT20OnePerCu = 512,
  kRuT20DumpTile0 = 1024,
};

enum : int {
  kMbFullTile = 1,
  kMbNoExpand = 2,
  kMbNoDepthwise = 4,
  kMbNoProject = 8,
  kMbNoXLoads = 16,
  kMbHalfTile = 32,
  kMbStripForm = 128,
  kMbFullBarriers = 256,
};

enum : int {
  kStemNoLoads = 1,
  kStemNoPhaseA = 2,
  kStemNoPhaseB = 4,
  kStemNoStores = 8,
  kStemProducersOnly = 64,
};

enum : int {
  kMbwNoExpand = 2,
  kMbwNoDepthwise = 4,
  kMbwNoProject = 8,
  kMbwNoWeightDma = 16,
};

enum : int {
  kDwOnePixel = 1,
  kDwFourRows = 2,
};
```

### pytorch_yolo_amd/diag.py

```python
from __future__ import annotations

import os

import torch

from ._lib import OP_CONV, OP_HEAD_DECODE, OP_RESUNIT, OP_STEM, YoloOp

DEPTH_FIRST_DEFAULT = ""


class GuardedAlloc:
    REDZONE_BYTE = 0x7F

    def _redzone(self) -> int:
        return int(os.environ.get("YOLO_REDZONE", "0")) // 256 * 256

    def _guarded(self, nbytes: int):
        rz = self._redzone()
        raw = torch.full((nbytes + 2 * rz,), self.REDZONE_BYTE, dtype=torch.uint8, device=self.device)
        self._redzones.append((raw, rz, nbytes))
        return raw, rz

    def _zeros(self, shape, dtype):
        if not self._redzone():
# ... 22 lines not shown
    def redzone_report(self):
        bad = []
        for i, (raw, rz, nbytes) in enumerate(self._redzones):
            lo = int((raw[:rz] != self.REDZONE_BYTE).sum())
            hi = int((raw[rz + nbytes:] != self.REDZONE_BYTE).sum())
            if lo or hi:
                bad.append((i, nbytes, lo, hi))
        return bad


def rewrite_list(plan, ops, op_launches):
    if plan.f32 or plan.f16:
        return ops, op_launches
    _shrink(plan, ops)
    return _depth_first(plan, ops, op_launches)


def _shrink(plan, ops):
    n = plan.rec.input.n
    for i in (int(v) for v in os.environ.get("YOLO_SHRINK_OPS", "").split(",") if v.strip()):
        op = ops[i]
        if op.kind != OP_HEAD_DECODE and op.splits < 2 and op.conv.n == n and op.conv.n > 1:
            sub = YoloOp.from_buffer_copy(op)
            sub.conv.n = 1
            ops[i] = sub


def _depth_first(plan, ops, op_launches):
    n = plan.rec.input.n
    spec = os.environ.get("YOLO_DEPTH_FIRST", DEPTH_FIRST_DEFAULT if n >= 16 else "")
    plan.depth_first = []
    plan._x_patch = [(0, 0)]
    if not spec or spec == "0":
        return ops, op_launches
    segs = []
    for part in spec.split(","):
        rng, s_ = part.split(":")
        a, b = (int(v) for v in rng.split("-"))
        s_ = int(s_)
        b = min(b, len(ops))
        ok = s_ >= 2 and n % s_ == 0 and 0 <= a < b and (not segs or a >= segs[-1][1])
        ok = ok and all(op.kind in (OP_STEM, OP_RESUNIT, OP_CONV) and op.splits < 2 and op.conv.n == n for op in ops[a:b])
        if ok:
            segs.append((a, b, s_))
    if not segs:
        return ops, op_launches
    new_ops, new_launches, pos = [], [], 0
    x_patch = []
    for a, b, s_ in segs:
        new_ops += ops[pos:a]; new_launches += op_launches[pos:a]
        for j in range(s_):
            for i in range(a, b):
                sub, x_off = _sub_op(ops[i], j, s_, plan.rec.c_in)
                if i == 0 and plan.fused_input:
                    x_patch.append((len(new_ops), x_off))
                new_ops.append(sub); new_launches.append(op_launches[i])
        pos = b
        plan.depth_first.append((a, b, s_))
    new_ops += ops[pos:]; new_launches += op_launches[pos:]
    if x_patch:
        plan._x_patch = x_patch
    return new_ops, new_launches


def _sub_op(op, j, s_, c_in):
    sub = YoloOp.from_buffer_copy(op)
    d = sub.conv
    n_sub = d.n // s_
    first = j * n_sub
    d.n = n_sub
    x_off = 0
    if op.kind == OP_STEM:
        x_off = first * c_in * d.h * d.w * 4
    else:
        sub.x = op.x + first * op.conv.h * op.conv.w * op.conv.in_c_total * 2
    up = 4 if op.conv.upsample2x else 1
    m_out = first * op.conv.ho * op.conv.wo
    if op.y:
        sub.y = op.y + m_out * up * op.conv.out_c_total * 2
    if op.residual:
        sub.residual = op.residual + m_out * op.conv.res_c_total * 2
    if op.y_aux:
        sub.y_aux = op.y_aux + m_out * op.conv.aux_c_total * 2
    return sub, x_off
```

### pytorch_yolo_amd/emit.py

```python
from __future__ import annotations

import os

import torch

from . import diag
from . import kernels as K
from ._lib import (ACT_LEAKY01, ACT_NONE, ACT_RELU, ACT_RELU6, ACT_SWISH, DT_BF16, DT_F16, DT_F32, OP_SE, OP_CONV, OP_CONV1_NCHW, OP_CONV_F16, OP_CONV_T20_F16,
                   OP_CONV_F32, OP_DWCONV, OP_CONV1_POOL, OP_CONV_POOL, OP_HEAD_DECODE_F16, OP_MAXPOOL_F16, OP_MAXPOOL_F32, OP_MBCONV,
                   OP_SHUFFLE, OP_HEAD_DECODE, OP_MAXPOOL, OP_RESUNIT, OP_SPP, OP_STEM, YoloOp)

_ACT = {"leaky": ACT_LEAKY01, "relu6": ACT_RELU6, "relu": ACT_RELU, "none": ACT_NONE, "swish": ACT_SWISH}


def _ptr(s):
    return s.buf.tensor.data_ptr()


def _in_view(d, x):
    d.n, d.h, d.w, d.cin, d.in_c_total, d.in_c_offset = x.n, x.h, x.w, x.c, x.buf.c_total, x.c_offset


def _out_view(d, y):
    d.ho, d.wo, d.out_c_total, d.out_c_offset = y.h, y.w, y.buf.c_total, y.c_offset
# ... 2 lines not shown
def _slice_of(s):
    return (s.buf.c_total, s.c_offset) if s is not None else (0, 0)


def _keep(plan, *tensors):
    return tuple(None if t is None else plan._dev(t).data_ptr() for t in tensors)


def _op(kind, **fields):
    op = YoloOp()
    op.kind = kind
    for name, value in fields.items():
        setattr(op, name, value)
    return op


def _emit_stem(plan, L):
    nd1, nd, y = L.pre[0], L.node, L.dst
    mid = nd.srcs[0]
    w1p, b1p, kpad1, _ = K.pack_conv_weight(*nd1.attrs["weight"], 8)
    w2p, b2p, kpad2, cout_pad2 = K.pack_conv_weight(*nd.attrs["weight"], 32)
    op = _op(OP_STEM, x=None, y=_ptr(y), kpad_pre=kpad1)
    op.w_pre, op.bias_pre, op.w, op.bias = _keep(plan, w1p, b1p, w2p, b2p)
    op.conv = K.conv_desc(n=mid.n, h=mid.h, w=mid.w, cin=32, in_c_total=32, in_c_offset=0, cout=64,
                          out_c_total=y.buf.c_total, out_c_offset=y.c_offset, ksize=3, stride=2,
                          act=_ACT[nd.attrs["act"]], kpad=kpad2, cout_pad=cout_pad2)
    op.conv.res_c_total = plan.rec.c_in
    return [op]


def _emit_head(plan, L):
    nd, x = L.node, L.src
    hd = next(h for h in plan.heads if h["sym"] is nd.outs[0])
    w, b = nd.attrs["weight"]
    wp, bp, kpad, cout_pad = (K.pack_conv_weight_f16 if plan.f16 else K.pack_conv_weight)(w, b, x.c)
    op = _op(OP_HEAD_DECODE_F16 if plan.f16 else OP_HEAD_DECODE, x=_ptr(x), y=None, y_aux=None)
    op.w, op.bias = _keep(plan, wp, bp)
    op.conv = K.conv_desc(n=x.n, h=x.h, w=x.w, cin=x.c, in_c_total=x.buf.c_total, in_c_offset=x.c_offset,
                          cout=w.shape[0], out_c_total=K.roundup(w.shape[0], 8), out_c_offset=0,
                          ksize=w.shape[2], stride=1, act=_ACT[nd.attrs["act"]], kpad=kpad,
                          cout_pad=cout_pad, out_dtype=DT_F32)
    for i, (aw, ah) in enumerate(hd["anchors"]):
        op.head_anchors_px[2 * i], op.head_anchors_px[2 * i + 1] = float(aw), float(ah)
    op.head_stride_px, op.head_na, op.head_nc = float(hd["stride"]), hd["na"], plan.n_class
    op.io_rows_total, op.io_row_offset = plan.rows_total, hd["row"]
    hd["op"] = op
    return [op]


def _emit_mbconv(plan, L):
    nd, dwn, x, y = L.node, L.pre[-1], L.src, L.dst
    we_b = L.pre[0].attrs["weight"] if len(L.pre) == 2 else (None, None)
    packed = K.pack_mbconv(we_b[0], we_b[1], *dwn.attrs["weight"], *nd.attrs["weight"], stride=dwn.attrs["stride"])
    op = _op(OP_MBCONV, x=_ptr(x), y=_ptr(y), kpad_pre=dwn.srcs[0].c)
    op.w_pre, op.bias_pre, op.w_dw, op.bias_dw, op.w, op.bias = _keep(plan, *packed)
    d = op.conv
    _in_view(d, x)
    _out_view(d, y)
    d.cout, d.ksize, d.stride, d.res_c_total = y.c, 3, dwn.attrs["stride"], 1 if nd.attrs["has_res"] else 0
    return [op]


def _emit_resunit(plan, L):
    nd, pa, x, y = L.node, L.pre[0], L.src, L.dst
    mid = nd.srcs[0]
    aux = nd.outs[1] if len(nd.outs) > 1 else None
    w1p, b1p, kpad1, cout_pad1 = K.pack_conv_weight(*pa.attrs["weight"], x.c)
    w2p, b2p, kpad2, cout_pad2 = K.pack_conv_weight(*nd.attrs["weight"], mid.c)
    op = _op(OP_RESUNIT, x=_ptr(x), y=_ptr(y), y_aux=_ptr(aux) if aux is not None else None, kpad_pre=kpad1, cout_pad_pre=cout_pad1)
    op.w_pre, op.bias_pre, op.w, op.bias = _keep(plan, w1p, b1p, w2p, b2p)
    op.conv = K.conv_desc(n=x.n, h=x.h, w=x.w, cin=mid.c, in_c_total=x.buf.c_total, in_c_offset=x.c_offset,
                          cout=x.c, out_c_total=y.buf.c_total, out_c_offset=y.c_offset, ksize=3, stride=1,
                          act=_ACT[nd.attrs["act"]], kpad=kpad2, cout_pad=cout_pad2, aux=_slice_of(aux))
    return [op]


def _emit_conv(plan, L):
    nd, x, dst = L.node, L.src, L.dst
    y = nd.outs[0]
    w, b = nd.attrs["weight"]
    pack, plain = (K.pack_conv_weight_f32, OP_CONV_F32) if plan.f32 else (K.pack_conv_weight, OP_CONV)
    if plan.f16:
        pack, plain = K.pack_conv_weight_f16, OP_CONV_F16
    wp, bp, kpad, cout_pad = pack(w, b, x.c)
    res = nd.srcs[1] if nd.attrs["has_res"] else None
    aux = nd.outs[1] if len(nd.outs) > 1 else None
    d = K.conv_desc(n=x.n, h=x.h, w=x.w, cin=x.c, in_c_total=x.buf.c_total if x.buf is not None else x.c, in_c_offset=x.c_offset,
                    cout=w.shape[0], out_c_total=dst.buf.c_total, out_c_offset=dst.c_offset,
                    ksize=w.shape[2], stride=nd.attrs["stride"], act=_ACT[nd.attrs["act"]],
                    kpad=kpad, cout_pad=cout_pad, upsample2x=1 if L.up else 0,
                    out_dtype=DT_F32 if (plan.f32 or y.f32) else (DT_F16 if plan.f16 else DT_BF16), pad=nd.attrs.get("pad"),
                    res=_slice_of(res), aux=_slice_of(aux))
    if not L.up and not L.pooled:
        d.ho, d.wo = y.h, y.w
    if L.reads_nchw:
        kind = OP_CONV1_POOL if L.pooled else OP_CONV1_NCHW
        d.res_c_total = plan.rec.c_in
    else:
        kind = OP_CONV_POOL if L.pooled else plain
        if kind == OP_CONV_F16 and os.environ.get("YOLO_FP16_T20", "1") != "0" and K.conv3x3_t20_f16_supported(d, res is not None, aux is not None):
            kind = OP_CONV_T20_F16
    op = _op(kind, x=None if L.reads_nchw else _ptr(x), y=_ptr(dst), residual=_ptr(res) if res is not None else None,
             y_aux=_ptr(aux) if aux is not None else None, conv=d)
    op.w, op.bias = _keep(plan, wp, bp)
    if kind == OP_CONV and os.environ.get("YOLO_SPLITK", "0") == "1":
        sp, wb, _ = K.conv2d_splitk_plan(d, res is not None, aux is not None)
        if sp >= 2:
            op.splits, op.ws_bytes = sp, wb
    return [op]


def _emit_dwconv(plan, L):
    nd, x, y = L.node, L.src, L.dst
    w, b = nd.attrs["weight"]
    kk = w.shape[2] * w.shape[3]
    op = _op(OP_DWCONV, x=_ptr(x), y=_ptr(y))
    op.w, op.bias = _keep(plan, w.detach().float().reshape(x.c, kk).t().contiguous(), b.detach().float().contiguous())
    d = op.conv
    _in_view(d, x)
    _out_view(d, y)
    d.stride, d.act = nd.attrs["stride"], _ACT[nd.attrs["act"]]
    d.ksize, d.pad = nd.attrs.get("ksize", 0), nd.attrs.get("pad", 0)
    return [op]


def _emit_se(plan, L):
    nd, x, y = L.node, L.src, L.dst
    sq = nd.attrs["w1"].shape[0]
    f = lambda t: t.detach().float()
    ws_bytes = K.se_workspace_bytes(x.n, x.c) // 4 * 4
    op = _op(OP_SE, x=_ptr(x), y=_ptr(y), kpad_pre=sq, ws_bytes=ws_bytes)
    op.w, op.w_pre, op.bias, op.bias_pre, op.workspace = _keep(plan, f(nd.attrs["w1"]).reshape(sq, x.c).contiguous(),
                               f(nd.attrs["w2"]).reshape(x.c, sq).t().contiguous(),
                               f(nd.attrs["b1"]).contiguous(), f(nd.attrs["b2"]).contiguous(),
                               torch.zeros(ws_bytes // 4, dtype=torch.float32))
    _in_view(op.conv, x)
    _out_view(op.conv, y)
    return [op]


def _emit_shuffle(plan, L):
    nd, y = L.node, L.dst
    a_, b_ = nd.srcs
    op = _op(OP_SHUFFLE, x=_ptr(a_), residual=_ptr(b_), y=_ptr(y))
    d = op.conv
    _in_view(d, a_)
    d.res_c_total, d.res_c_offset = b_.buf.c_total, b_.c_offset
    d.out_c_total, d.out_c_offset, d.cout = y.buf.c_total, y.c_offset, nd.attrs["half"]
    return [op]


def _maxpool(kind, x, y, size, stride, pad, dil, out_c_offset):
    op = _op(kind, x=_ptr(x), y=_ptr(y))
    d = op.conv
    _in_view(d, x)
    _out_view(d, y)
    d.out_c_offset = out_c_offset
    d.ksize, d.stride, d.pad, d.upsample2x = size, stride, pad, dil
    return op


def _emit_pool(plan, L):
    a = L.node.attrs
    return [_maxpool(OP_MAXPOOL_F32 if plan.f32 else (OP_MAXPOOL_F16 if plan.f16 else OP_MAXPOOL), L.src, L.dst, a["size"], a["stride"], a["pad"], a["dil"], L.dst.c_offset)]


def _emit_spp(plan, L):
    x, y = L.src, L.dst
    if plan.f32:
        return [_maxpool(OP_MAXPOOL_F32, x, y, k, 1, k // 2, 1, y.c_offset + lvl * x.c) for lvl, k in enumerate((5, 9, 13))]
    op = _op(OP_SPP, y=_ptr(y))
    op.conv.n, op.conv.h, op.conv.w, op.conv.cin = x.n, x.h, x.w, x.c
    return [op]


EMITTERS = {"conv": _emit_conv, "stem": _emit_stem, "resunit": _emit_resunit, "mbconv": _emit_mbconv, "head": _emit_head,
            "dwconv": _emit_dwconv, "se": _emit_se, "shuffle": _emit_shuffle, "pool": _emit_pool, "spp": _emit_spp}


def build_ops(plan):
    plan.heads = []
    row = 0
    for x, layer in plan.rec.heads:
        na = len(layer.anchors_px)
        stride = plan.img_size / max(x.w, x.h)
        plan.heads.append(dict(sym=x, anchors=layer.anchors_px, stride=stride, row=row, na=na, layer=layer, op=None))
        row += na * x.h * x.w
    plan.rows_total = row
    ops, op_launches = [], []
    for L in plan.launches:
        if (plan.f32 or plan.f16) and L.kind in ("dwconv", "shuffle", "se"):
            raise NotImplementedError(f"precision='{plan.precision}' covers the Darknet families (YOLOv3-SPP / -tiny / YOLOv3 / Lite); "
                                      f"no {plan.precision} kernel for '{L.kind}' layers")
        assert not (L.reads_nchw and ops)
        for op in EMITTERS[L.kind](plan, L):
            ops.append(op); op_launches.append(L)
    ops, op_launches = diag.rewrite_list(plan, ops, op_launches)
    index = {id(op): i for i, op in enumerate(ops)}
    for hd in plan.heads:
        if hd["op"] is not None:
            hd["op"] = index[id(hd["op"])]
    splitk = [K.conv2d_splitk_plan(op.conv, bool(op.residual), bool(op.y_aux)) for op in ops if op.splits >= 2]
    if splitk:
        plan._splitk_ws = torch.empty((max(wb for _, wb, _ in splitk) + 3) // 4, dtype=torch.float32, device=plan.device)
        plan._splitk_cnt = torch.zeros(max(nc for _, _, nc in splitk), dtype=torch.int32, device=plan.device)
        for op in ops:
            if op.splits >= 2:
                op.workspace, op.counters = plan._splitk_ws.data_ptr(), plan._splitk_cnt.data_ptr()
    plan.n_ops = len(ops)
    plan.op_launches = op_launches
    plan.op_nodes = [L.node for L in op_launches]
    plan.op_array = (YoloOp * len(ops))(*ops)


_CONVS = (OP_CONV, OP_CONV1_NCHW, OP_CONV1_POOL, OP_CONV_POOL, OP_HEAD_DECODE, OP_CONV_F32, OP_CONV_F16, OP_HEAD_DECODE_F16, OP_CONV_T20_F16)


def conv_flops(op_array, n_ops: int, c_in: int) -> float:
    total = 0.0
    first = True
    for i in range(n_ops):
        op = op_array[i]
        d = op.conv
        if op.kind in _CONVS:
            cin = c_in if first else d.cin
            first = False
            total += 2.0 * d.n * d.ho * d.wo * d.cout * d.ksize * d.ksize * cin
        elif op.kind == OP_STEM:
            first = False
            total += 2.0 * d.n * d.h * d.w * 32 * 9 * c_in + 2.0 * d.n * d.ho * d.wo * 64 * 9 * 32
        elif op.kind == OP_RESUNIT:
            total += 2.0 * d.n * d.h * d.w * (d.cout * d.cin) * 10
        elif op.kind == OP_DWCONV:
            total += 2.0 * d.n * d.ho * d.wo * d.cin * 9
        elif op.kind == OP_MBCONV:
            hid = op.kpad_pre
            total += (2.0 * d.n * d.h * d.w * d.cin * hid if op.w_pre else 0.0) + 2.0 * d.n * d.ho * d.wo * hid * (9 + d.cout)
    return total


def algorithmic_bytes(op_array, n_ops: int, c_in: int, detect: bool = False) -> float:
    total = 0.0
    first = True
    for i in range(n_ops):
        op = op_array[i]
        d = op.conv
        m_in, m_out = d.n * d.h * d.w, d.n * d.ho * d.wo
        if op.kind in _CONVS:
            x_b = m_in * (c_in * 4 if (first and op.kind in (OP_CONV1_NCHW, OP_CONV1_POOL)) else d.cin * (4 if op.kind == OP_CONV_F32 else 2))
            first = False
            pooled = 4 if op.kind in (OP_CONV1_POOL, OP_CONV_POOL) else 1
            y_b = m_out * d.cout * (4 if d.out_dtype == DT_F32 else 2) * (4 if d.upsample2x else 1) / pooled
            if op.kind in (OP_HEAD_DECODE, OP_HEAD_DECODE_F16):
                y_b = 2.0 * m_out * d.cout * 4
                if detect:
                    y_b = m_out * op.head_na * 8.0
            total += x_b + y_b + d.cout * d.ksize * d.ksize * d.cin * 2
            total += (m_out * d.cout * 2 if op.residual else 0) + (m_out * d.cout * 2 if op.y_aux else 0)
        elif op.kind == OP_STEM:
            first = False
            total += m_in * c_in * 4 + m_out * 64 * 2
        elif op.kind == OP_RESUNIT:
            total += m_in * d.cout * 2 * (3 if op.y_aux else 2)
        elif op.kind == OP_MBCONV:
            total += m_in * d.cin * 2 + m_out * d.cout * 2
        elif op.kind in (OP_MAXPOOL, OP_DWCONV, OP_MAXPOOL_F32, OP_MAXPOOL_F16):
            total += (m_in + m_out) * d.cin * (4 if op.kind == OP_MAXPOOL_F32 else 2)
        elif op.kind == OP_SE:
            total += 3.0 * m_in * d.cin * 2
        elif op.kind == OP_SPP:
            total += m_in * d.cin * 2 * 4
        elif op.kind == OP_SHUFFLE:
            total += 2.0 * m_in * d.cin * 2
    return total
```

### pytorch_yolo_amd/engine.py

```python
from __future__ import annotations

import atexit
import ctypes as C
import os

import torch

from . import emit, planner
from . import kernels as K
from ._lib import YoloOp
from .diag import DEPTH_FIRST_DEFAULT, GuardedAlloc
from .graph import Buf, Node, Recorder, Sym
from .planner import FUSE_RESUNIT_DEFAULT, Launch


class _Runs:
    def new_outputs(self, want_p: bool = True):
        no = self.n_class + 5
        io = torch.empty((self.bs, self.rows_total, no), dtype=torch.float32, device=self.device)
        ps = tuple(torch.empty((self.bs, hd["na"], hd["sym"].h, hd["sym"].w, no), dtype=torch.float32, device=self.device) if want_p else None
                   for hd in self.heads)
        return io, ps

    def run(self, x: torch.Tensor):
        io, ps = self.new_outputs()
        self._launch(x, io, ps)
        return io, ps

    def run_graph(self, x: torch.Tensor):
        if self._graph is None:
            self._static_x = torch.empty_like(x)
            self._static_out = self.new_outputs()
            side = torch.cuda.Stream(device=self.device)
            side.wait_stream(torch.cuda.current_stream())
            with torch.cuda.stream(side):
                self._static_x.copy_(x)
                self._launch(self._static_x, *self._static_out)
            torch.cuda.current_stream().wait_stream(side)
            graph = torch.cuda.CUDAGraph()
            with torch.cuda.graph(graph):
                self._launch(self._static_x, *self._static_out)
            self._graph = graph
        self._static_x.copy_(x)
        self._graph.replay()
        return self._static_out


class Plan(GuardedAlloc, _Runs):
    n_streams = 1

    def __init__(self, rec: Recorder, device, n_class: int, img_size: int, precision: str = "bf16"):
        if precision not in ("bf16", "fp32", "fp16"):
            raise ValueError(f"precision must be 'bf16', 'fp32' or 'fp16', got {precision!r}")
        self.f32 = precision == "fp32"
        self.f16 = precision == "fp16"
        self.precision = precision
        self.device = device
        self.rec = rec
        self.bs = rec.input.n
        self.n_class = n_class
        self.img_size = img_size
        self._keep = []
        self._redzones = []
        self._compact_ws = None
        self._bound = None
        self._graph = None
        self._static_out = None
        self.depth_first, self._x_patch = [], [(0, 0)]
        self.launches = planner.fuse(rec, self.f32, n_class, self.f16)
        self.fused_input = any(L.reads_nchw for L in self.launches)
        self._bufs = planner.place(rec, self.launches)
        self.shared_buffers = planner.alloc(rec, self.launches, self._bufs, self.f32, self._zeros, self.f16)
        emit.build_ops(self)

    def set_input_ptr(self, ptr: int):
        for idx, off in self._x_patch:
            self.op_array[idx].x = ptr + off

    @property
    def input_buffer(self) -> torch.Tensor:
        return self.rec.input.buf.tensor

    def feed(self, x: torch.Tensor):
        if self.fused_input:
            if x.dtype != torch.float32 or not x.is_contiguous() or tuple(x.shape[1:]) != (self.rec.c_in, self.rec.input.h, self.rec.input.w):
                raise RuntimeError("input must be contiguous float32 NCHW of the planned shape")
            self.set_input_ptr(x.data_ptr())
        elif self.f32:
            K.pack_input_f32(x, self.input_buffer)
        elif self.f16:
            K.pack_input_f16(x, self.input_buffer)
        else:
            K.pack_input(x, self.input_buffer)

    def _launch(self, x: torch.Tensor, io: torch.Tensor, ps, timing=None, before_io=None, compact=None):
        self.feed(x)
        self._bind_outputs(io, ps, compact)
        if timing is not None:
            timing[0].record()
        fused = [hd["op"] for hd in self.heads if hd["op"] is not None]
        k = min(fused) if fused else self.n_ops
        if before_io is None or k == 0:
            if before_io is not None:
                before_io()
            K.run_ops(self.op_array, self.n_ops)
        else:
            K.run_ops(self.op_array, k)
            before_io()
            if k < self.n_ops:
                K.run_ops(C.cast(C.byref(self.op_array, k * C.sizeof(YoloOp)), C.POINTER(YoloOp)), self.n_ops - k)
        if timing is not None:
            timing[1].record()
        self._decode_unfused(io, ps)

    @property
    def compact_ok(self) -> bool:
        return not self.f32 and all(hd["op"] is not None for hd in self.heads)

    def compact_workspace(self) -> torch.Tensor:
        ws = self._compact_ws
        if ws is None:
            ws = self._compact_ws = torch.empty(K.nms_compact_workspace_bytes(self.rec.input.n, self.rows_total, self.n_class),
                                                dtype=torch.uint8, device=self.device)
        return ws

    def _bind_outputs(self, io, ps, compact=None):
        if compact is not None:
            if not self.compact_ok:
                raise RuntimeError("the compact NMS form needs every head to decode in its conv epilogue")
            ws, conf, min_wh = compact
            for hd, p in zip(self.heads, ps):
                op = self.op_array[hd["op"]]
                op.y, op.y_aux = None, (p.data_ptr() if p is not None else None)
                op.workspace, op.ws_bytes = ws.data_ptr(), ws.numel()
                op.head_filter_conf, op.head_filter_min_wh = float(conf), float(min_wh)
            self._bound = (ws.data_ptr(), float(conf), tuple(None if p is None else p.data_ptr() for p in ps))
            return
        if io.shape[1] != self.rows_total or not io.is_contiguous():
            raise RuntimeError("io must be a contiguous [bs, rows_total, 5+nc] tensor")
        for hd, p in zip(self.heads, ps):
            if hd["op"] is not None:
                op = self.op_array[hd["op"]]
                op.y, op.y_aux = io.data_ptr(), (p.data_ptr() if p is not None else None)
                op.workspace, op.ws_bytes = None, 0
        self._bound = (io.data_ptr(), None, tuple(None if p is None else p.data_ptr() for p in ps))

    def _decode_unfused(self, io, ps):
        for hd, p in zip(self.heads, ps):
            if hd["op"] is None:
                K.decode(hd["sym"].buf.tensor, hd["anchors"], self.n_class, hd["stride"], io, hd["row"], p)

    def launch_detect(self, x, io, ps, nms_out, conf_thres, nms_thres, timing=None, join=True, after_nms=None, whole_batch=False,
# ... 360 lines not shown
```

### pytorch_yolo_amd/kernels.py

```python
from __future__ import annotations

import ctypes as C

import torch

from . import _lib
from ._lib import (ACT_LEAKY01, ACT_NONE, ACT_RELU6, DT_BF16, DT_F16, DT_F32, YoloConvDesc, YoloMbconvDesc,
                   check, load)

__all__ = ["stream_ptr", "pack_input", "conv2d", "conv2d_pick", "head_decode_pick", "stem", "resunit", "resunit_supported", "resunit_form", "maxpool", "spp", "dwconv3x3", "dwconv", "se", "se_workspace_bytes", "mbconv", "mbconv_supported", "mbconv_form", "pack_mbconv", "conv3x3_pool", "conv3x3_pool_supported", "conv2d_splitk", "conv2d_splitk_plan", "decode", "head_decode", "head_decode_supported",
           "nms_merge", "pack_conv_weight", "roundup", "run_ops"]


def roundup(v: int, m: int) -> int:
    return (v + m - 1) // m * m


def stream_ptr() -> int:
    return torch.cuda.current_stream().cuda_stream


def _ptr(t):
    return None if t is None else C.c_void_p(t.data_ptr())

# ... 82 lines not shown
def conv2d_f16_pick(desc: YoloConvDesc, has_residual=False, has_preadd=False) -> str:
    buf = C.create_string_buffer(256)
    check(load().yolo_conv2d_f16_pick(C.byref(desc), int(has_residual), int(has_preadd), buf, 256), "conv2d_f16_pick")
    return buf.value.decode()


def head_decode_f16_pick(desc: YoloConvDesc, na: int, nc: int, filter: bool = False) -> str:
    buf = C.create_string_buffer(256)
    check(load().yolo_head_decode_f16_pick(C.byref(desc), na, nc, int(filter), buf, 256), "head_decode_f16_pick")
    return buf.value.decode()


def maxpool_f16(x, y, *, n, h, w, c, in_view, out_view, ksize, stride, pad, dilation=1):
    _need_cuda(x, y)
    ho = (h + 2 * pad - dilation * (ksize - 1) - 1) // stride + 1
    wo = (w + 2 * pad - dilation * (ksize - 1) - 1) // stride + 1
    check(load().yolo_maxpool_f16_fwd(_ptr(x), _ptr(y), n, h, w, c, in_view[0], in_view[1], ho, wo, out_view[0],
                                      out_view[1], ksize, stride, pad, dilation, stream_ptr()), "maxpool_f16")
    return y


def head_decode_f16(x, w_packed, bias, desc: YoloConvDesc, anchors_px, nc, stride_px, io, io_row_offset, p=None):
    _need_cuda(x, w_packed, bias, io, p)
    na = len(anchors_px)
    flat = (C.c_float * (2 * na))(*[float(v) for a in anchors_px for v in a])
    check(load().yolo_head_decode_f16_fwd(_ptr(x), _ptr(w_packed), _ptr(bias), C.byref(desc), flat, na, nc, float(stride_px),
                                          _ptr(io), io.shape[1], io_row_offset, _ptr(p), stream_ptr()), "head_decode_f16")
    return io


def head_decode_filter_f16(x, w_packed, bias, desc: YoloConvDesc, anchors_px, nc, stride_px, rows_total, io_row_offset, conf_thres,
                           workspace, *, min_wh=2.0, p=None):
    _need_cuda(x, w_packed, bias, workspace, p)
    na = len(anchors_px)
    flat = (C.c_float * (2 * na))(*[float(v) for a in anchors_px for v in a])
    check(load().yolo_head_decode_filter_f16_fwd(_ptr(x), _ptr(w_packed), _ptr(bias), C.byref(desc), flat, na, nc, float(stride_px),
                                                 rows_total, io_row_offset, float(conf_thres), float(min_wh), _ptr(workspace),
                                                 workspace.numel() * workspace.element_size(), _ptr(p), stream_ptr()),
          "head_decode_filter_f16")


def pack_input_f32(x: torch.Tensor, out: torch.Tensor) -> torch.Tensor:
    _need_cuda(x, out)
    if x.dtype != torch.float32 or not x.is_contiguous():
        raise RuntimeError("pack_input_f32: x must be contiguous float32 NCHW")
    n, c, h, w = x.shape
    if out.dtype != torch.float32 or tuple(out.shape[:3]) != (n, h, w) or not out.is_contiguous():
        raise RuntimeError("pack_input_f32: out must be contiguous f32 [n,h,w,c_pad]")
    check(load().yolo_pack_input_nchw_f32_nhwc(_ptr(x), _ptr(out), n, c, h, w, out.shape[3], stream_ptr()), "pack_input_f32")
    return out


def conv2d_f32(x, w_packed, bias, y, desc: YoloConvDesc, residual=None, y_preadd=None):
    _need_cuda(x, w_packed, bias, y, residual, y_preadd)
    for t in (x, w_packed, bias, y, residual, y_preadd):
        if t is not None and t.dtype != torch.float32:
            raise RuntimeError("conv2d_f32: every tensor must be float32")
    check(load().yolo_conv2d_f32_fwd(_ptr(x), _ptr(w_packed), _ptr(bias), _ptr(residual), _ptr(y), _ptr(y_preadd),
                                     C.byref(desc), stream_ptr()), "conv2d_f32")
    return y


def maxpool_f32(x, y, *, n, h, w, c, in_view, out_view, ksize, stride, pad, dilation=1):
    _need_cuda(x, y)
    ho = (h + 2 * pad - dilation * (ksize - 1) - 1) // stride + 1
    wo = (w + 2 * pad - dilation * (ksize - 1) - 1) // stride + 1
    check(load().yolo_maxpool_f32_fwd(_ptr(x), _ptr(y), n, h, w, c, in_view[0], in_view[1], ho, wo, out_view[0],
                                      out_view[1], ksize, stride, pad, dilation, stream_ptr()), "maxpool_f32")
    return y


def pack_input(x: torch.Tensor, out: torch.Tensor) -> torch.Tensor:
    _need_cuda(x, out)
    if x.dtype != torch.float32 or not x.is_contiguous():
        raise RuntimeError("pack_input: x must be contiguous float32 NCHW")
    n, c, h, w = x.shape
    if out.dtype != torch.bfloat16 or tuple(out.shape[:3]) != (n, h, w) or not out.is_contiguous():
        raise RuntimeError("pack_input: out must be contiguous bf16 [n,h,w,c_pad]")
    check(load().yolo_pack_input_nchw_f32(_ptr(x), _ptr(out), n, c, h, w, out.shape[3], stream_ptr()), "pack_input")
    return out


def conv_desc(*, n, h, w, cin, in_c_total, in_c_offset, cout, out_c_total, out_c_offset, ksize, stride,
              act, kpad, cout_pad, upsample2x=0, out_dtype=DT_BF16, res=(0, 0), aux=(0, 0), pad=None) -> YoloConvDesc:
    pad = (ksize - 1) // 2 if pad is None else pad
    d = YoloConvDesc()
    d.n, d.h, d.w, d.cin, d.in_c_total, d.in_c_offset = n, h, w, cin, in_c_total, in_c_offset
    d.ho, d.wo = (h + 2 * pad - ksize) // stride + 1, (w + 2 * pad - ksize) // stride + 1
    d.cout, d.out_c_total, d.out_c_offset = cout, out_c_total, out_c_offset
    d.ksize, d.stride, d.pad, d.act, d.upsample2x, d.out_dtype = ksize, stride, pad, act, upsample2x, out_dtype
    d.kpad, d.cout_pad = kpad, cout_pad
    d.res_c_total, d.res_c_offset = res
    d.aux_c_total, d.aux_c_offset = aux
    return d


def conv2d_pick(desc: YoloConvDesc, has_residual=False, has_preadd=False) -> str:
    buf = C.create_string_buffer(256)
    check(load().yolo_conv2d_pick(C.byref(desc), int(has_residual), int(has_preadd), buf, 256), "conv2d_pick")
    return buf.value.decode()


def head_decode_pick(desc: YoloConvDesc, na: int, nc: int, filter: bool = False) -> str:
    buf = C.create_string_buffer(256)
    check(load().yolo_head_decode_pick(C.byref(desc), na, nc, int(filter), buf, 256), "head_decode_pick")
    return buf.value.decode()


def conv2d(x, w_packed, bias, y, desc: YoloConvDesc, residual=None, y_preadd=None):
    _need_cuda(x, w_packed, bias, y, residual, y_preadd)
    check(load().yolo_conv2d_fwd(_ptr(x), _ptr(w_packed), _ptr(bias), _ptr(residual), _ptr(y), _ptr(y_preadd),
                                 C.byref(desc), stream_ptr()), "conv2d")
    return y


def conv2d_splitk_plan(desc: YoloConvDesc, has_residual=False, has_preadd=False):
    sp, wb, nc = C.c_int(1), C.c_size_t(0), C.c_int(0)
    check(load().yolo_conv2d_splitk_plan(C.byref(desc), int(has_residual), int(has_preadd), C.byref(sp), C.byref(wb), C.byref(nc)),
          "conv2d_splitk_plan")
    return sp.value, wb.value, nc.value


def conv2d_splitk(x, w_packed, bias, y, desc: YoloConvDesc, splits, workspace, counters, residual=None, y_preadd=None):
    _need_cuda(x, w_packed, bias, y, residual, y_preadd, workspace, counters)
    check(load().yolo_conv2d_splitk_fwd(_ptr(x), _ptr(w_packed), _ptr(bias), _ptr(residual), _ptr(y), _ptr(y_preadd), C.byref(desc),
                                        splits, _ptr(workspace), workspace.numel() * workspace.element_size(), _ptr(counters),
                                        stream_ptr()), "conv2d_splitk")
    return y


def stem(x_nchw, cin_real, w1_packed, b1, kpad1, w2_packed, b2, y, desc: YoloConvDesc):
    _need_cuda(x_nchw, w1_packed, b1, w2_packed, b2, y)
    check(load().yolo_stem_fwd(_ptr(x_nchw), cin_real, _ptr(w1_packed), _ptr(b1), kpad1, _ptr(w2_packed), _ptr(b2), _ptr(y),
                               C.byref(desc), stream_ptr()), "stem")
    return y


def resunit_supported(c: int, h: int, w: int) -> bool:
    return bool(load().yolo_resunit_supported(c, h, w))


def resunit_form(c: int, n: int, h: int, w: int) -> int:
    return int(load().yolo_resunit_form(c, n, h, w))


def resunit(x, w1_packed, b1, w2_packed, b2, y, desc: YoloConvDesc, kpad1: int, cout_pad1: int, y_preadd=None):
    _need_cuda(x, w1_packed, b1, w2_packed, b2, y, y_preadd)
    check(load().yolo_resunit_fwd(_ptr(x), _ptr(w1_packed), _ptr(b1), _ptr(w2_packed), _ptr(b2), _ptr(y), _ptr(y_preadd),
                                  C.byref(desc), kpad1, cout_pad1, stream_ptr()), "resunit")
    return y


def maxpool(x, y, *, n, h, w, c, in_view, out_view, ksize, stride, pad, dilation=1):
    _need_cuda(x, y)
    ho = (h + 2 * pad - dilation * (ksize - 1) - 1) // stride + 1
    wo = (w + 2 * pad - dilation * (ksize - 1) - 1) // stride + 1
    check(load().yolo_maxpool_fwd(_ptr(x), _ptr(y), n, h, w, c, in_view[0], in_view[1], ho, wo, out_view[0],
                                  out_view[1], ksize, stride, pad, dilation, stream_ptr()), "maxpool")
    return y


def spp(buf, *, n, h, w, c):
    _need_cuda(buf)
    check(load().yolo_spp_fwd(_ptr(buf), n, h, w, c, stream_ptr()), "spp")
    return buf


def se_workspace_bytes(n, c) -> int:
    return int(load().yolo_se_workspace_bytes(n, c))


def dwconv(x, wkc, bias, y, *, n, h, w, c, in_view, out_view, ho, wo, ksize, stride, pad, act):
    _need_cuda(x, wkc, bias, y)
    check(load().yolo_dwconv_fwd(_ptr(x), _ptr(wkc), _ptr(bias), _ptr(y), n, h, w, c, in_view[0], in_view[1], ho, wo, out_view[0],
                                 out_view[1], ksize, stride, pad, act, stream_ptr()), "dwconv")
    return y


def se(x, y, w1, b1, w2, b2, workspace, *, n, h, w, c, in_view, out_view):
    _need_cuda(x, y, w1, b1, w2, b2, workspace)
    check(load().yolo_se_fwd(_ptr(x), _ptr(y), n, h, w, c, in_view[0], in_view[1], out_view[0], out_view[1], _ptr(w1), _ptr(b1),
                             _ptr(w2), _ptr(b2), w1.shape[0], _ptr(workspace), workspace.numel() * workspace.element_size(),
                             stream_ptr()), "se")
# ... 210 lines not shown
```

### pytorch_yolo_amd/models/yolo_base.py

```python
from __future__ import annotations

import os
from collections import OrderedDict

import numpy as np
import torch
from torch import nn

from .. import engine
from ..utils.torch_utils import fold_conv_bn, fuse_conv_and_bn
from .yolo_layer import YOLOLayer

DEFAULT_ANCHORS = (((10.0, 14.0), (23.0, 27.0), (37.0, 58.0)),
                   ((81.0, 82.0), (135.0, 169.0), (344.0, 319.0)))

_STRUCT_EPOCH = [0]
_DATA_PTR = torch.Tensor.data_ptr
_VERSION = __import__("operator").attrgetter("_version")
MAX_CACHED_PLANS = 8


class ConvBlock(nn.Module):

    def __init__(self, in_channels, out_channels, size=3, stride=1, pad=True):
# ... 4 lines not shown
            raise NotImplementedError("HIP conv supports 1x1/3x3, stride 1/2")
        self.sequence = nn.Sequential(OrderedDict([
            ("conv", nn.Conv2d(in_channels, out_channels, size, stride, (size - 1) // 2, bias=False)),
            ("batch_norm", nn.BatchNorm2d(out_channels)),
            ("activation", nn.LeakyReLU(0.1, inplace=True)),
        ]))
        self.in_channels, self.out_channels = in_channels, out_channels
        self.size, self.stride = size, stride

    @property
    def is_fused(self) -> bool:
        return not hasattr(self.sequence, "batch_norm")

    def folded(self):
        if self.is_fused:
            conv = self.sequence[0]
            return conv.weight.detach().float().cpu(), conv.bias.detach().float().cpu()
        conv, bn = self.sequence.conv, self.sequence.batch_norm
        return fold_conv_bn(conv.weight, conv.bias, bn.weight, bn.bias, bn.running_mean, bn.running_var, bn.eps)

    def fuse(self):
        if self.is_fused:
            return
        rest = [m for name, m in self.sequence.named_children() if name not in ("conv", "batch_norm")]
        self.sequence = nn.Sequential(fuse_conv_and_bn(self.sequence.conv, self.sequence.batch_norm), *rest)
        _STRUCT_EPOCH[0] += 1

    def _trace(self, g: engine.Recorder, x, **kw):
        return g.conv(x, self.folded(), stride=self.stride, act="leaky", name=getattr(self, "_trace_name", None), **kw)

    def forward(self, x):
        return engine.run_standalone(lambda g, s: self._trace(g, s), x)


class MaxPool(nn.Module):

    def __init__(self, size, stride):
        super().__init__()
        self.size, self.stride = size, stride

    def _trace(self, g, x):
        return g.maxpool(x, self.size, self.stride)

    def forward(self, x):
        return engine.run_standalone(lambda g, s: self._trace(g, s), x)


class ConvPoolBlock(ConvBlock):

    def __init__(self, in_channels, out_channels, conv_size=3, conv_stride=1, conv_pad=True,
                 pool_size=2, pool_stride=2):
        super().__init__(in_channels, out_channels, conv_size, conv_stride, conv_pad)
        self.sequence.add_module("max_pool", MaxPool(pool_size, pool_stride))

    @property
    def pool(self) -> MaxPool:
        return self.sequence[-1]

    def _trace(self, g, x, **kw):
        return self.pool._trace(g, super()._trace(g, x, **kw))


class YOLOBase(nn.Module):

    def __init__(self, in_channels=3, n_class=80, kernels_divider=1, anchors=DEFAULT_ANCHORS,
                 onnx=False, in_shape=None, hyper_params=None):
        super().__init__()
        if onnx:
            raise NotImplementedError("onnx=True selects the export branch, which is out of scope (SURVEY §2 #13)")
        self.header_info = np.zeros(5, dtype=np.int32)
        self.seen = self.header_info[3]
        self.hyper_params = hyper_params
        self.n_class = n_class
        self.onnx = False
        self.in_channels = in_channels
        self.anchors = anchors
        self.kernels_divider = kernels_divider
        self.in_shape = in_shape
        self.yolo_layer_input_size = 15 + 3 * n_class
        self.encoder = None
        self._plans = {}
        self._tensors = None
        self.use_hip_graph = False
        self.n_streams = 2
        self.precision = os.environ.get("YOLO_PRECISION", "bf16")

    def _create_yolo_layers(self, device="cpu"):
        return [YOLOLayer(a, self.n_class, self.anchors, False) for a in self.anchors]

    def invalidate(self):
        self._plans = {}
        self._tensors = None

    def _fingerprint(self):
        if self.__dict__.get("_tensors") is None or self.__dict__.get("_epoch_seen") != _STRUCT_EPOCH[0]:
            self._epoch_seen = _STRUCT_EPOCH[0]
            for m in self.modules():
                if not m.__dict__.get("_yolo_hooked"):
                    m.register_load_state_dict_post_hook(lambda _mod, _keys, _self=self: _self.invalidate())
                    m.__dict__["_yolo_hooked"] = True
            self._tensors = list(self.parameters()) + list(self.buffers())
        return hash((self._epoch_seen, tuple(map(_DATA_PTR, self._tensors)), tuple(map(_VERSION, self._tensors))))

    def _apply(self, fn, *a, **kw):
        self.invalidate()
        return super()._apply(fn, *a, **kw)

    def load_state_dict(self, *a, **kw):
        self.invalidate()
        return super().load_state_dict(*a, **kw)

    def fuse(self):
        for m in self.modules():
            if isinstance(m, ConvBlock):
                m.fuse()
        self.invalidate()

    def load_darknet_weights(self, weights_path, warnings=True):
        from ..utils.darknet_io import load_darknet_weights
        return load_darknet_weights(self, weights_path)

    def save_darknet_weights(self, path, warnings=True):
        from ..utils.darknet_io import save_darknet_weights
        save_darknet_weights(self, path)

    def _trace(self, g: engine.Recorder, x):
        raise NotImplementedError

    def plan_for(self, x: torch.Tensor) -> engine.Plan:
        if x.dim() != 4 or x.shape[1] != self.in_channels:
            raise RuntimeError(f"expected input [bs,{self.in_channels},H,W], got {tuple(x.shape)}")
        if not x.is_cuda:
            raise RuntimeError("pytorch_yolo_amd runs on a ROCm device only: move the input to cuda "
                               "(there is no CPU fallback)")
        bs, c, h, w = x.shape
        n_streams = self.n_streams if (self.n_streams > 1 and bs % self.n_streams == 0 and bs // self.n_streams >= 4) else 1
        key = (tuple(x.shape), x.device, n_streams, self.precision)
        fp = self._fingerprint()
        if self.__dict__.get("_plans_fp") != fp:
            self._plans = {}
            self._plans_fp = fp
        plan = self._plans.pop(key, None)
        if plan is not None:
            self._plans[key] = plan
        if plan is None:
            for name, m in self.named_modules():
                m._trace_name = name

            def make(sub_bs):
                rec = engine.Recorder(sub_bs, c, h, w)
                self._trace(rec, rec.input)
                return engine.Plan(rec, x.device, self.n_class, max(h, w), self.precision)
            with torch.cuda.device(x.device):
                plan = make(bs) if n_streams == 1 else engine.StreamedPlan(make, bs, n_streams, x.device)
            self._plans[key] = plan
            while len(self._plans) > MAX_CACHED_PLANS:
                self._plans.pop(next(iter(self._plans)))
        return plan

    def forward(self, x):
        if self.training:
            raise NotImplementedError(
                "training-mode forward (batch-statistics BN, raw p list) is outside the inference hot path; "
                "call .eval() first")
        if x.dtype != torch.float32:
            x = x.float()
        x = x.contiguous()
        plan = self.plan_for(x)
        for hd in plan.heads:
            hd["layer"]._sync_grid_attrs(hd["sym"].h, hd["sym"].w, plan.img_size, x.device)
        with torch.cuda.device(x.device):
            if self.use_hip_graph:
                return plan.run_graph(x)
            return plan.run(x)

    def detect_stream(self, batches, conf_thres=0.5, nms_thres=0.5, depth=None):
        from ..utils.utils import nms_capacity, split_detections
        if self.training:
            raise NotImplementedError("detect_stream() is an inference call: .eval() first")
        ring, pending, plan, shape, dev = [], [], None, None, None
        try:
            for x in batches:
                x = x.float().contiguous()
                if shape is None:
                    shape, dev = tuple(x.shape), x.device
                    plan = self.plan_for(x)
                    if depth is None:
                        depth = max(2, plan.n_streams) * (2 if plan.conv_flops() < 1e12 else 1)
                    depth = max(2, int(depth))
                    cap = nms_capacity(plan.rows_total, self.n_class)
                    pool = plan.__dict__.setdefault("_stream_rings", {})
                    ring = pool.pop(depth, None) or []
                    for item in ring:
                        if item[4] is not None:
                            item[4].step.conf_thres, item[4].step.nms_thres = float(conf_thres), float(nms_thres)
                    with torch.cuda.device(x.device):
                        for slot in range(0 if ring else depth):
                            out = (torch.empty((shape[0], cap, 7), dtype=torch.float32, device=x.device),
                                   torch.empty((shape[0], cap), dtype=torch.int32, device=x.device),
                                   torch.empty((shape[0],), dtype=torch.int32, device=x.device))
                            fast = plan.fast_pipeline(slot, None, out, conf_thres, nms_thres) if hasattr(plan, "fast_pipeline") else None
                            io, ps = (None, ()) if fast is not None else plan.new_outputs(want_p=False)
                            ring.append((io, ps, out, torch.cuda.Event(), fast))
                elif tuple(x.shape) != shape or x.device != dev:
                    raise RuntimeError(f"detect_stream: batch {tuple(x.shape)} on {x.device} differs from the first one "
                                       f"{shape} on {dev}")
                while len(pending) >= len(ring):
                    yield self._collect(pending.pop(0))
                k = self.__dict__.setdefault("_stream_calls", 0)
                self._stream_calls = k + 1
                io, ps, out, done, fast = ring[k % len(ring)]
                with torch.cuda.device(x.device):
                    pending.append((x, out, done, fast))
                    if fast is not None:
                        fast.launch(x)
                        continue
                    ready = torch.cuda.Event()
                    ready.record()
                    plan.launch_detect(x, io, ps, out, conf_thres, nms_thres, join=False, whole_batch=True, wait_for=ready, compact=True,
                                       after_nms=lambda i, lo, hi, done=done: done.record(torch.cuda.current_stream()))
            while pending:
                yield self._collect(pending.pop(0))
        finally:
            if pending and dev is not None:
                torch.cuda.synchronize(dev)
                pending.clear()
            if plan is not None and ring and len(ring) == depth:
                plan.__dict__.setdefault("_stream_rings", {})[depth] = ring

    @staticmethod
    def _collect(item):
        from ..utils.utils import split_detections
        _, out, done, fast = item
        if fast is not None:
            return fast.collect()
# ... 22 lines not shown
```

### pytorch_yolo_amd/planner.py

```python
from __future__ import annotations

import os
from dataclasses import dataclass
from typing import List, Optional

import torch

from . import kernels as K
from .graph import Buf, Node, Recorder, Sym

FUSE_RESUNIT_DEFAULT = 64 | 128

NO_LAUNCH = ("input", "up", "cat", "slice", "head")


@dataclass(eq=False)
class Launch:
    kind: str
    node: Node
    pre: tuple = ()
    src: Optional[Sym] = None
    dst: Optional[Sym] = None
    up: bool = False
    pooled: bool = False
    reads_nchw: bool = False
    layer: object = None


class _Fusion:

    def __init__(self, rec: Recorder, f32: bool, n_class: int, f16: bool = False):
        env = os.environ.get
        self.rec, self.n_class = rec, n_class
        plain = f32 or f16
        self.resunit_mask = 0 if plain else int(env("YOLO_FUSE_RESUNIT", str(FUSE_RESUNIT_DEFAULT)))
        self.mbconv = "0" if plain else env("YOLO_FUSE_MBCONV", "1")
        self.pool, self.stem, self.conv1_s2 = (not plain and env(k, "1") == "1" for k in (
            "YOLO_FUSE_POOL", "YOLO_FUSE_STEM", "YOLO_FUSE_CONV1_S2"))
        self.head = not f32 and env("YOLO_FUSE_HEAD", "1") == "1"
        self.nchw = not plain


def _ksize(nd):
    return nd.attrs["weight"][0].shape[2]


def _only_consumer(s: Sym, kind: str):
    return s.consumers[0] if len(s.consumers) == 1 and s.consumers[0].kind == kind else None


def _pool_2x2(s: Sym):
    ndp = _only_consumer(s, "pool")
    if ndp is None or (ndp.attrs["size"], ndp.attrs["stride"], ndp.attrs["pad"], ndp.attrs["dil"]) != (2, 2, 0, 1) or s.h % 2 or s.w % 2:
        return None
    return ndp


def fuse_upsample(fz, nd):
    if nd.kind != "up":
        return None
    x = nd.srcs[0]
    if x.producer.kind != "conv" or len(x.consumers) != 1:
        raise RuntimeError("upsample must directly follow a conv with no other consumer")
    return Launch("conv", x.producer, pre=(nd,), src=x.producer.srcs[0], dst=nd.outs[0], up=True)


def fuse_resunit(fz, nd):
    if nd.kind != "conv" or not nd.attrs["has_res"]:
        return None
    mid, res = nd.srcs
    pa = mid.producer
    if pa is None or pa.kind != "conv" or pa.attrs["has_res"] or len(pa.outs) != 1 or len(mid.consumers) != 1:
        return None
    (w1, _), (w2, _) = pa.attrs["weight"], nd.attrs["weight"]
    c = res.c
    if (pa.srcs[0] is not res or w1.shape[2] != 1 or w2.shape[2] != 3 or nd.attrs["stride"] != 1 or pa.attrs["stride"] != 1
            or w2.shape[0] != c or w1.shape[0] * 2 != c or w1.shape[1] != c or pa.attrs["act"] != nd.attrs["act"] or nd.outs[0].f32):
        return None
    if (fz.resunit_mask & c) and K.resunit_supported(c, res.h, res.w) and (c == 64 or K.resunit_form(c, res.n, res.h, res.w) == 3):
        return Launch("resunit", nd, pre=(pa,), src=res, dst=nd.outs[0])
    return None


def fuse_mbconv(fz, nd):
    if (fz.mbconv == "0" or nd.kind != "conv" or len(nd.outs) != 1 or nd.outs[0].f32 or nd.attrs["act"] != "none"
            or nd.attrs["stride"] != 1 or _ksize(nd) != 1):
        return None
    dsym = nd.srcs[0]
    dwn = dsym.producer
    if dwn is None or dwn.kind != "dwconv" or dwn.attrs["act"] != "relu6" or len(dsym.consumers) != 1:
        return None
    esym = dwn.srcs[0]
    ex = esym.producer
    has_exp = (ex is not None and ex.kind == "conv" and _ksize(ex) == 1 and ex.attrs["act"] == "relu6" and ex.attrs["stride"] == 1
               and not ex.attrs["has_res"] and len(ex.outs) == 1 and len(esym.consumers) == 1 and not esym.f32)
    x = ex.srcs[0] if has_exp else esym
    if x is fz.rec.input or x.f32 or (nd.attrs["has_res"] and nd.srcs[1] is not x):
        return None
    form = K.mbconv_form(x.c, esym.c, nd.attrs["weight"][0].shape[0], dwn.attrs["stride"])
    if form == 1 or (form == 2 and has_exp and fz.mbconv != "narrow"):
        return Launch("mbconv", nd, pre=(ex, dwn) if has_exp else (dwn,), src=x, dst=nd.outs[0])
    return None


def fuse_conv_pool(fz, nd):
    if (not fz.pool or nd.kind != "conv" or nd.attrs["has_res"] or len(nd.outs) != 1 or nd.attrs["stride"] != 1
            or nd.srcs[0] is fz.rec.input):
        return None
    w, _ = nd.attrs["weight"]
    mid = nd.outs[0]
    ndp = _pool_2x2(mid)
    if w.shape[2] != 3 or mid.f32 or ndp is None or not K.conv3x3_pool_supported(w.shape[1], w.shape[0]):
        return None
    return Launch("conv", nd, pre=(ndp,), src=nd.srcs[0], dst=ndp.outs[0], pooled=True)


def _first_conv_stride(fz, nd):
    x = fz.rec.input
    if not fz.nchw or nd.kind != "conv" or nd.srcs[0] is not x or len(x.consumers) != 1 or fz.rec.c_in > 8:
        return 0
    cout, stride = nd.attrs["weight"][0].shape[0], nd.attrs["stride"]
    s1 = cout in (16, 32) and stride == 1
    s2 = cout == 32 and stride == 2 and fz.conv1_s2
    ok = (s1 or s2) and _ksize(nd) == 3 and "pad" not in nd.attrs and not nd.attrs["has_res"] and len(nd.outs) == 1 and not nd.outs[0].f32
    return stride if ok else 0


def fuse_stem(fz, nd1):
    nd2 = _only_consumer(nd1.outs[0], "conv") if fz.stem and _first_conv_stride(fz, nd1) == 1 else None
    if (nd2 is None or tuple(nd2.attrs["weight"][0].shape) != (64, 32, 3, 3) or nd2.attrs["stride"] != 2 or nd2.attrs["has_res"]
            or len(nd2.outs) != 1 or nd2.outs[0].f32 or nd2.attrs["act"] != nd1.attrs["act"] or nd2.srcs[0] is not nd1.outs[0]):
        return None
    return Launch("stem", nd2, pre=(nd1,), src=nd1.srcs[0], dst=nd2.outs[0], reads_nchw=True)


def fuse_conv1_pool(fz, nd):
    ndp = _pool_2x2(nd.outs[0]) if fz.pool and _first_conv_stride(fz, nd) == 1 else None
    return None if ndp is None else Launch("conv", nd, pre=(ndp,), src=nd.srcs[0], dst=ndp.outs[0], pooled=True, reads_nchw=True)


def fuse_conv1_nchw(fz, nd):
    return Launch("conv", nd, src=nd.srcs[0], dst=nd.outs[0], reads_nchw=True) if _first_conv_stride(fz, nd) else None


def _head_layer(rec, nd):
    if nd.kind != "conv" or not nd.outs[0].f32 or _only_consumer(nd.outs[0], "head") is None:
        return None
    return next((layer for x, layer in rec.heads if x is nd.outs[0]), None)


def fuse_head(fz, nd):
    layer = _head_layer(fz.rec, nd) if fz.head else None
    if layer is None or nd.attrs["has_res"] or len(nd.outs) != 1 or nd.attrs["stride"] != 1:
        return None
    if not K.head_decode_supported(nd.attrs["weight"][0].shape[0], len(layer.anchors_px), fz.n_class):
        return None
    return Launch("head", nd, src=nd.srcs[0], layer=layer)


RULES = (fuse_upsample,
         fuse_resunit,
         fuse_mbconv,
         fuse_conv_pool,
         fuse_stem,
         fuse_conv1_pool,
         fuse_conv1_nchw,
         fuse_head)


def fuse(rec: Recorder, f32: bool, n_class: int, f16: bool = False) -> List[Launch]:
    fz = _Fusion(rec, f32, n_class, f16)
    claimed = {}
    for rule in RULES:
        for nd in rec.nodes:
            launch = rule(fz, nd)
            if launch is not None and not any(id(m) in claimed for m in (launch.node,) + launch.pre):
                claimed.update((id(m), launch) for m in (launch.node,) + launch.pre)
    launches = []
    for nd in rec.nodes:
        launch = claimed.get(id(nd))
        if launch is None and nd.kind not in NO_LAUNCH:
            launch = Launch(nd.kind, nd, src=nd.srcs[0], dst=nd.outs[0])
        if launch is not None and launch.node is nd:
            launches.append(launch)
    return launches


def place(rec: Recorder, launches: List[Launch]) -> List[Buf]:
    nodes = rec.nodes
    order = {id(nd): i for i, nd in enumerate(nodes)}
    by_node = {id(L.node): L for L in launches}
    swallowed = {id(m) for L in launches for m in L.pre}
    bufs = []

    def own_buf(s: Sym):
        s.buf, s.c_offset = Buf(s.n, s.h, s.w, s.c, f32=s.f32), 0
        bufs.append(s.buf)

    for nd in nodes:
        if nd.kind == "cat":
            y = nd.outs[0]
            if y.buf is None:
                own_buf(y)
            off = y.c_offset
            for x in nd.srcs:
                if x.buf is not None:
                    raise RuntimeError("a tensor feeds two concats: needs a copy (not required by any model here)")
                x.buf, x.c_offset = y.buf, off
                off += x.c
        elif nd.kind == "spp":
            y, x = nd.outs[0], nd.srcs[0]
            if y.buf is None:
                own_buf(y)
            if y.c_offset != 0 or y.buf.c_total != y.c:
                raise RuntimeError("spp output must own its buffer")
            if x.buf is not None:
                raise RuntimeError("spp input already placed")
            x.buf, x.c_offset = y.buf, 3 * x.c
    for nd in nodes:
        if nd.kind == "up" and nd.outs[0].buf is None:
            own_buf(nd.outs[0])
    in_place = []
    for L in launches:
        nd = L.node
        if L.kind == "conv" and nd.attrs["has_res"]:
            res, y = nd.srcs[1], nd.outs[0]
            dead = all(order[id(cn)] <= order[id(nd)] for cn in res.consumers)
            if dead and y.buf is None and res.buf is not None and not y.f32:
                y.buf, y.c_offset = res.buf, res.c_offset
            elif dead and y.buf is None and res.buf is None:
                in_place.append(nd)
    fused_input = any(L.reads_nchw for L in launches)
    for nd in nodes:
        L = by_node.get(id(nd))
        if id(nd) in swallowed or nd.kind == "slice" or (L is not None and L.kind == "head") or (nd.kind == "input" and fused_input):
            continue
        if L is not None and L.pooled:
            if L.dst.buf is None:
                own_buf(L.dst)
            continue
        for o in nd.outs:
            if o.buf is None and not (o.slot == 0 and L is not None and (L.up or nd in in_place)):
                own_buf(o)
    for nd in nodes:
        if nd.kind == "slice":
            src, y = nd.srcs[0], nd.outs[0]
            y.buf, y.c_offset = src.buf, src.c_offset + nd.attrs["offset"]
    for nd in in_place:
        res, y = nd.srcs[1], nd.outs[0]
        y.buf, y.c_offset = res.buf, res.c_offset
    return bufs


def _live_ranges(rec: Recorder, launches: List[Launch]):
    order = {id(nd): i for i, nd in enumerate(rec.nodes)}
    rng = {}
    pinned = set()

    def touch(s: Optional[Sym], i):
        if s is not None and s.buf is not None:
            lo, hi = rng.get(id(s.buf), (i, i))
            rng[id(s.buf)] = (min(lo, i), max(hi, i))

    for nd in rec.nodes:
        for s_ in nd.srcs + nd.outs:
            touch(s_, order[id(nd)])
            if nd.kind in ("input", "head") and s_.buf is not None:
                pinned.add(id(s_.buf))
    for L in launches:
        touch(L.src, order[id(L.node)])
        touch(L.dst, order[id(L.node)])
    return rng, pinned


def alloc(rec: Recorder, launches: List[Launch], bufs: List[Buf], f32: bool, zeros, f16: bool = False) -> int:
    reuse = os.environ.get("YOLO_REUSE_BUFFERS", "1") == "1" and not f32
    rng, pinned = _live_ranges(rec, launches) if reuse else ({}, set())
    filled = {}
    for nd in rec.nodes:
        for s_ in nd.outs:
            if s_.buf is not None:
                filled[id(s_.buf)] = filled.get(id(s_.buf), 0) + s_.c
    pool = {}
    shared = 0
    for b in sorted(bufs, key=lambda b_: rng.get(id(b_), (0, 0))[0]):
        dt = torch.float32 if (b.f32 or f32) else (torch.float16 if f16 else torch.bfloat16)
        ct = K.roundup(b.c_total, 8)
        exact = ct == b.c_total and filled.get(id(b), 0) == b.c_total
        b.c_total = ct
        lo, hi = rng.get(id(b), (None, None))
        if reuse and exact and lo is not None and id(b) not in pinned:
            free = pool.setdefault((b.n, b.h, b.w, ct, dt), [])
            hit = next((e for e in free if e[0] < lo), None)
            if hit is not None:
                free.remove(hit)
                b.tensor = hit[1]
                shared += 1
            else:
                b.tensor = zeros((b.n, b.h, b.w, ct), dt)
            free.append((hi, b.tensor))
        else:
            b.tensor = zeros((b.n, b.h, b.w, ct), dt)
    return shared
```

Baseline: 6720.

## Fuse nearest-upsample and concat into following 1x1 conv via two-source loads

Adds a two-source 1x1 convolution form that reads the upsampled half of a concat directly from the half-resolution tensor via index mapping, and the other half from the skip tensor. This removes materializing the 2x upsampled tensor and the concat buffer in YOLOv3's neck. The planner detects the up->cat->1x1 conv pattern and is enabled by default. Costs extra address arithmetic per pixel and new kernel instances, plus more complex buffer placement.

Result: no change. 6734, median of 6 (+0.2%).

```diff
diff --git a/include/yolo_hip.h b/include/yolo_hip.h
--- a/include/yolo_hip.h
+++ b/include/yolo_hip.h
@@ -47,6 +47,10 @@
 
 YOLO_API int yolo_conv2d_fwd(const void* x, const void* w_packed, const float* bias, const void* residual,
                     void* y, void* y_preadd, const YoloConvDesc* d, yolo_stream_t s);
+
+YOLO_API int yolo_conv2d_up2_supported(const YoloConvDesc* d);
+YOLO_API int yolo_conv2d_up2_fwd(const void* a_half, const void* x, const void* w_packed, const float* bias, void* y,
+                                 const YoloConvDesc* d, yolo_stream_t s);
 
 YOLO_API int yolo_conv2d_pick(const YoloConvDesc* d, int has_residual, int has_preadd, char* out, int out_len);
 
diff --git a/pytorch_yolo_amd/_lib.py b/pytorch_yolo_amd/_lib.py
--- a/pytorch_yolo_amd/_lib.py
+++ b/pytorch_yolo_amd/_lib.py
@@ -69,6 +69,8 @@
     "yolo_conv1_pool_nchw_f32_fwd": (C.c_int, [C.c_void_p, C.c_int, C.c_void_p, C.c_void_p, C.c_void_p,
                                                C.POINTER(YoloConvDesc), C.c_void_p]),
     "yolo_conv2d_pick": (C.c_int, [C.POINTER(YoloConvDesc), C.c_int, C.c_int, C.c_char_p, C.c_int]),
+    "yolo_conv2d_up2_supported": (C.c_int, [C.POINTER(YoloConvDesc)]),
+    "yolo_conv2d_up2_fwd": (C.c_int, [C.c_void_p] * 5 + [C.POINTER(YoloConvDesc), C.c_void_p]),
     "yolo_pack_conv_weight_f32": (C.c_int, [C.c_void_p] + [C.c_int] * 6 + [C.c_void_p]),
     "yolo_stem_supported": (C.c_int, [C.c_int] * 5),
     "yolo_stem_fwd": (C.c_int, [C.c_void_p, C.c_int, C.c_void_p, C.c_void_p, C.c_int, C.c_void_p, C.c_void_p, C.c_void_p,
diff --git a/pytorch_yolo_amd/csrc/conv1x1_stream.hip b/pytorch_yolo_amd/csrc/conv1x1_stream.hip
--- a/pytorch_yolo_amd/csrc/conv1x1_stream.hip
+++ b/pytorch_yolo_amd/csrc/conv1x1_stream.hip
@@ -99,7 +99,7 @@
   }
 }
 
-template <int N, int K, int P>
+template <int N, int K, int P, bool SRC2 = false>
 __global__ __launch_bounds__(256, 2) void conv1x1_stream2_kernel(const ConvArgs a, int n_tiles_px) {
   constexpr int NF = N / 64, KC = K / 32, PB = P / 16;
   constexpr int XB = KC * P * 64;
@@ -117,6 +117,7 @@
   const ActParams ap(d.act);
   const int c16 = lane & 15, q = lane >> 4;
   const __amdgpu_buffer_rsrc_t rx = __builtin_amdgcn_make_buffer_rsrc((void*)a.x, 0, a.x_bytes, 0x00020000);
+  const __amdgpu_buffer_rsrc_t rx2 = __builtin_amdgcn_make_buffer_rsrc((void*)(SRC2 ? a.x2 : a.x), 0, SRC2 ? a.x2_bytes : a.x_bytes, 0x00020000);
   const uint32_t y_pitch = (uint32_t)d.out_c_total * 2u;
   const __amdgpu_buffer_rsrc_t ry = __builtin_amdgcn_make_buffer_rsrc(a.y, 0, (uint32_t)a.M * y_pitch, 0x00020000);
 
@@ -134,6 +135,9 @@
   const uint32_t lane_src = (uint32_t)drow * x_pitch + (uint32_t)(d.in_c_offset + dchunk * 8) * 2u;
   const uint32_t xfrag = (uint32_t)(c16 * 64 + ((q ^ swz32(c16 >> 2)) << 4));
   const int orow = lane / LPR, ocol = lane % LPR;
+  const int kc2 = SRC2 ? up2_c(d) / 32 : 0;
+  const uint32_t x2_pitch = (uint32_t)d.aux_c_total * 2u;
+  const uint32_t lane_src2 = (uint32_t)(d.aux_c_offset + dchunk * 8) * 2u;
 
   auto issue_tile = [&](int j) {
     const long t = (long)blockIdx.x + (long)j * gridDim.x;
@@ -143,8 +147,14 @@
     for (int i = 0; i < NPW; ++i) {
       const int piece = i * 4 + wave, kc = piece / PB, pb = piece - kc * PB;
       const long px = p0 + pb * 16 + drow;
-      const uint32_t vo = (t < n_tiles_px && px < a.M) ? (uint32_t)(p0 + pb * 16) * x_pitch + lane_src : kOobOffset;
-      lds_dma16s(rx, buf + piece * 1024, vo, (uint32_t)kc * 64u);
+      const bool ok = t < n_tiles_px && px < a.M;
+      if (SRC2 && kc < kc2) {
+        const uint32_t vo = ok ? up2_src_pixel((uint32_t)px, (uint32_t)d.h, (uint32_t)d.w) * x2_pitch + lane_src2 : kOobOffset;
+        lds_dma16s(rx2, buf + piece * 1024, vo, (uint32_t)kc * 64u);
+      } else {
+        const uint32_t vo = ok ? (uint32_t)(p0 + pb * 16) * x_pitch + lane_src : kOobOffset;
+        lds_dma16s(rx, buf + piece * 1024, vo, (uint32_t)(kc - kc2) * 64u);
+      }
     }
 #if defined(__HIP_DEVICE_COMPILE__)
     asm volatile("" ::: "memory");
@@ -210,12 +220,12 @@
   wait_vmcnt<0>();
 }
 
-template <int N, int K, int P>
+template <int N, int K, int P, bool SRC2 = false>
 int launch_stream2(const ConvArgs& a, hipStream_t s) {
   const int tiles = (a.M + P - 1) / P;
   const int grid = tiles < 512 ? tiles : 512;
-  if (pick_only("stream1x1p<%d couts,K %d,%d px> grid %d", N, K, P, grid)) return 0;
-  hipLaunchKernelGGL((conv1x1_stream2_kernel<N, K, P>), dim3((unsigned)grid), dim3(256), 0, s, a, tiles);
+  if (pick_only("stream1x1p%s<%d couts,K %d,%d px> grid %d", SRC2 ? "_up2" : "", N, K, P, grid)) return 0;
+  hipLaunchKernelGGL((conv1x1_stream2_kernel<N, K, P, SRC2>), dim3((unsigned)grid), dim3(256), 0, s, a, tiles);
   return yolo_check_launch("yolo_conv2d_fwd(1x1 stream, pipelined)");
 }
 
@@ -236,6 +246,11 @@
   if (d.in_c_offset % 8 || d.in_c_total % 8 || d.out_c_offset % 8 || d.out_c_total % 8) return 1;
   if ((size_t)a.M * d.out_c_total * 2 >= kOobOffset) return 1;
   if (!force && a.M < 40000) return 1;
+  if (up2_c(d) > 0) {
+    if (a.debug & kCdStreamFirstForm) return 1;
+    if (d.cout == 128 && d.cin + up2_c(d) == 384 && up2_c(d) % 32 == 0) return launch_stream2<128, 384, 48, true>(a, s);
+    return 1;
+  }
   if (!(a.debug & kCdStreamFirstForm)) {
     if (d.cout == 128 && d.cin == 256) return launch_stream2<128, 256, 80>(a, s);
     if (d.cout == 128 && d.cin == 128) return launch_stream2<128, 128, 80>(a, s);
diff --git a/pytorch_yolo_amd/csrc/conv_common.h b/pytorch_yolo_amd/csrc/conv_common.h
--- a/pytorch_yolo_amd/csrc/conv_common.h
+++ b/pytorch_yolo_amd/csrc/conv_common.h
@@ -61,6 +61,8 @@
   int n_tiles = 0;
   int steps = 0;
   uint32_t x_bytes = 0, w_bytes = 0;
+  const bf16_t* x2 = nullptr;
+  uint32_t x2_bytes = 0;
   HeadDecodeArgs hd;
   int splits = 1;
   float* ws = nullptr;
@@ -73,6 +75,14 @@
 
 inline size_t conv_x_bytes(const YoloConvDesc& d) { return (size_t)d.n * d.h * d.w * d.in_c_total * 2; }
 inline size_t conv_w_bytes(const YoloConvDesc& d) { return (size_t)d.cout_pad * d.kpad * 2; }
+__host__ __device__ inline int up2_c(const YoloConvDesc& d) { return d.res_c_total < 0 ? -d.res_c_total : 0; }
+inline size_t conv_x2_bytes(const YoloConvDesc& d) { return (size_t)d.n * (d.h / 2) * (d.w / 2) * d.aux_c_total * 2; }
+
+__host__ __device__ inline uint32_t up2_src_pixel(uint32_t px, uint32_t h, uint32_t w) {
+  const uint32_t hw = h * w, img = px / hw, rem = px - img * hw;
+  const uint32_t y = rem / w, x = rem - y * w;
+  return (img * (h >> 1) + (y >> 1)) * (w >> 1) + (x >> 1);
+}
 
 inline ConvArgs make_conv_args(const void* x, const void* w, const float* bias, const void* res, void* y, void* aux, const YoloConvDesc& d) {
   ConvArgs a;
diff --git a/pytorch_yolo_amd/csrc/conv_igemm.hip b/pytorch_yolo_amd/csrc/conv_igemm.hip
--- a/pytorch_yolo_amd/csrc/conv_igemm.hip
+++ b/pytorch_yolo_amd/csrc/conv_igemm.hip
@@ -25,10 +25,11 @@
 __device__ __forceinline__ f32x16 mfma32(f16x8 w, f16x8 x, f32x16 c) { return __builtin_amdgcn_mfma_f32_32x32x16_f16(w, x, c, 0, 0, 0); }
 
 template <int BM, int BN, int WAVES_M, int WAVES_N, int BK, int NS, bool FAST, bool LDS_EPI, bool MFMA16 = false, bool DECODE = false,
-          int NP = 0, bool SPLITK = false, typename T = bf16_t>
+          int NP = 0, bool SPLITK = false, typename T = bf16_t, bool SRC2 = false>
 __global__ __launch_bounds__(64 * (WAVES_M * WAVES_N + NP)) void conv_igemm_kernel(const ConvArgs a) {
   using X4 = typename Pack<T>::x4;
   using X8 = typename Pack<T>::x8;
+  static_assert(!SRC2 || (FAST && !DECODE && !SPLITK && NP == 0), "two-source form: fast 1x1 path, plain instances");
   static_assert(!SPLITK || (FAST && LDS_EPI && MFMA16 && !DECODE), "split-K: 16x16x32 path with the LDS epilogue");
   constexpr int NW = WAVES_M * WAVES_N;
   constexpr int NL = NP > 0 ? NP : NW;
@@ -72,6 +73,8 @@
 
   const __amdgpu_buffer_rsrc_t rx = __builtin_amdgcn_make_buffer_rsrc((void*)a.x, 0, a.x_bytes, 0x00020000);
   const __amdgpu_buffer_rsrc_t rw = __builtin_amdgcn_make_buffer_rsrc((void*)a.w, 0, a.w_bytes, 0x00020000);
+  const __amdgpu_buffer_rsrc_t rx2 = __builtin_amdgcn_make_buffer_rsrc((void*)(SRC2 ? a.x2 : a.x), 0, SRC2 ? a.x2_bytes : a.x_bytes, 0x00020000);
+  const int cin_k = SRC2 ? d.cin + up2_c(d) : d.cin;
 
   const int frow = lane / CPR;
   const int fsw = (BK == 32) ? swz32(lane >> 4) : (((lane >> 4) + 4 * (lw & 1)) & 7);
@@ -79,6 +82,7 @@
   const int ntaps = d.ksize * d.ksize;
   int px_base[PIT], px_hi0[PIT], px_wi0[PIT];
   uint32_t px_mask[PIT];
+  uint32_t px_base2[SRC2 ? PIT : 1];
   const int hw_out = d.ho * d.wo;
 #pragma unroll
   for (int it = 0; it < PIT; ++it) {
@@ -105,6 +109,8 @@
     if (!ok) mask = 0;
     px_mask[it] = mask;
     if (FAST) px_base[it] = (px_base[it] + chunk * 8) * 2;
+    if constexpr (SRC2)
+      px_base2[it] = (up2_src_pixel((uint32_t)mm, (uint32_t)d.h, (uint32_t)d.w) * (uint32_t)d.aux_c_total + (uint32_t)(d.aux_c_offset + chunk * 8)) * 2u;
   }
   uint32_t w_off[WIT];
 #pragma unroll
@@ -112,12 +118,12 @@
     const int row = (it * NL + lw) * RPP + frow;
     w_off[it] = row < BN ? (uint32_t)(((n0 + row) * d.kpad + chunk * 8) * 2) : kOobOffset;
   }
-  int tap = FAST ? 0 : (chunk * 8) / d.cin;
-  int kc = FAST ? 0 : chunk * 8 - tap * d.cin;
+  int tap = FAST ? 0 : (chunk * 8) / cin_k;
+  int kc = FAST ? 0 : chunk * 8 - tap * cin_k;
   if constexpr (SPLITK) {
     const int k0 = blockIdx.y * a.steps * BK;
-    tap = k0 / d.cin;
-    kc = k0 - tap * d.cin;
+    tap = k0 / cin_k;
+    kc = k0 - tap * cin_k;
 #pragma unroll
     for (int it = 0; it < WIT; ++it)
       if (w_off[it] != kOobOffset) w_off[it] += (uint32_t)k0 * 2u;
@@ -136,12 +142,22 @@
     char* const xb = wb + BNL * ROWB;
     if (FAST) {
       const uint32_t tap_off = (uint32_t)(((st_dh * d.w + st_dw) * d.in_c_total + kc) * 2);
-      const uint32_t bit = (kc + chunk * 8 < d.cin) ? 1u << tap : 0u;
-#pragma unroll
-      for (int it = 0; it < PIT; ++it) {
-        if (it < lo || it >= hi) continue;
-        const uint32_t voff = (px_mask[it] & bit) ? (uint32_t)px_base[it] + tap_off : kOobOffset;
-        if (!(a.debug & kCdNoPixelDma)) lds_dma16(rx, xb + it * (NL * 1024), voff);
+      const uint32_t bit = (kc + chunk * 8 < cin_k) ? 1u << tap : 0u;
+      if (SRC2 && kc < up2_c(d)) {
+#pragma unroll
+        for (int it = 0; it < PIT; ++it) {
+          if (it < lo || it >= hi) continue;
+          const uint32_t voff = (px_mask[it] & bit) ? px_base2[it] + (uint32_t)kc * 2u : kOobOffset;
+          if (!(a.debug & kCdNoPixelDma)) lds_dma16(rx2, xb + it * (NL * 1024), voff);
+        }
+      } else {
+        const uint32_t src_off = SRC2 ? tap_off - (uint32_t)up2_c(d) * 2u : tap_off;
+#pragma unroll
+        for (int it = 0; it < PIT; ++it) {
+          if (it < lo || it >= hi) continue;
+          const uint32_t voff = (px_mask[it] & bit) ? (uint32_t)px_base[it] + src_off : kOobOffset;
+          if (!(a.debug & kCdNoPixelDma)) lds_dma16(rx, xb + it * (NL * 1024), voff);
+        }
       }
 #pragma unroll
       for (int it = 0; it < WIT; ++it) {
@@ -169,13 +185,13 @@
   auto stage_end = [&]() {
     kc += BK;
     if (FAST) {
-      if (kc >= d.cin) {
+      if (kc >= cin_k) {
         kc = 0;
         ++tap;
       }
     } else {
-      while (kc >= d.cin) {
-        kc -= d.cin;
+      while (kc >= cin_k) {
+        kc -= cin_k;
         ++tap;
       }
     }
@@ -483,15 +499,15 @@
 }
 
 template <int BM, int BN, int WAVES_M, int WAVES_N, int BK, int NS, bool FAST, bool LDS_EPI, bool MFMA16 = false, bool DECODE = false,
-          int NP = 0, bool SPLITK = false, typename T = bf16_t>
+          int NP = 0, bool SPLITK = false, typename T = bf16_t, bool SRC2 = false>
 int launch_cfg(const ConvArgs& a, hipStream_t s) {
   const int m_tiles = (a.M + BM - 1) / BM;
   ConvArgs b = a;
   b.n_tiles = (a.d.cout + BN - 1) / BN;
-  b.steps = (a.d.ksize * a.d.ksize * a.d.cin + BK - 1) / BK;
+  b.steps = (a.d.ksize * a.d.ksize * (a.d.cin + (SRC2 ? up2_c(a.d) : 0)) + BK - 1) / BK;
   const long grid = (long)m_tiles * b.n_tiles;
   if (grid > 0x7fffffffL) return yolo_set_error(YOLO_E_UNSUPPORTED, "conv grid too large");
-  if (pick_only("%s<%dx%d,%dx%d waves%s,BK%d,%d stages%s%s%s%s> grid %ld", std::is_same<T, f16_t>::value ? "igemm_f16" : "igemm", BM, BN, WAVES_M, WAVES_N, NP ? "+4 loaders" : "", BK, NS,
+  if (pick_only("%s<%dx%d,%dx%d waves%s,BK%d,%d stages%s%s%s%s> grid %ld", SRC2 ? "igemm_up2" : std::is_same<T, f16_t>::value ? "igemm_f16" : "igemm", BM, BN, WAVES_M, WAVES_N, NP ? "+4 loaders" : "", BK, NS,
                 FAST ? "" : ",generic", MFMA16 ? ",16x16x32" : ",32x32x16", DECODE ? ",decode" : "", SPLITK ? ",splitK" : "", grid))
     return 0;
   unsigned gy = 1;
@@ -500,7 +516,7 @@
     b.steps /= a.splits;
     gy = (unsigned)a.splits;
   }
-  hipLaunchKernelGGL((conv_igemm_kernel<BM, BN, WAVES_M, WAVES_N, BK, NS, FAST, LDS_EPI, MFMA16, DECODE, NP, SPLITK, T>),
+  hipLaunchKernelGGL((conv_igemm_kernel<BM, BN, WAVES_M, WAVES_N, BK, NS, FAST, LDS_EPI, MFMA16, DECODE, NP, SPLITK, T, SRC2>),
                      dim3((unsigned)grid, gy), dim3(64 * (WAVES_M * WAVES_N + NP)), 0, s, b);
   return yolo_check_launch("yolo_conv2d_fwd");
 }
@@ -754,6 +770,43 @@
   return I::k128x128_8w;
 }
 
+#define YOLO_IGEMM_UP2_INSTANCES(X)                                                     \
+  X(k256x32_m32, 256, 32, 4, 1, 32, 2, true, true, false, false, 0, false)              \
+  X(k256x64_m32, 256, 64, 4, 1, 32, 2, true, true, false, false, 0, false)              \
+  X(k128x128_bk32_3st_m32, 128, 128, 2, 2, 32, 3, true, true, false, false, 0, false)   \
+  X(k64x64_4st, 64, 64, 2, 2, 64, 4, true, true, true, false, 0, false)                 \
+  X(k64x64, 64, 64, 2, 2, 64, 2, true, true, true, false, 0, false)                     \
+  X(k128x128_8w, 128, 128, 2, 4, 64, 2, true, true, true, false, 0, false)              \
+  X(k128x128_8w_3st, 128, 128, 2, 4, 64, 3, true, true, true, false, 0, false)          \
+  X(k128x256_16w_3st, 128, 256, 2, 8, 64, 3, true, true, true, false, 0, false)         \
+  X(k256x128_8w_bk32, 256, 128, 4, 2, 32, 2, true, true, true, false, 0, false)         \
+  X(k256x256_16w, 256, 256, 4, 4, 64, 2, true, true, true, false, 0, false)
+
+int launch_igemm_up2(IgemmId id, const ConvArgs& a, hipStream_t s) {
+  switch (id) {
+#define X(id, ...) \
+  case IgemmId::id: return launch_cfg<__VA_ARGS__, bf16_t, true>(a, s);
+    YOLO_IGEMM_UP2_INSTANCES(X)
+#undef X
+    default: return 1;
+  }
+}
+
+const char* up2_form_error(const YoloConvDesc& d, bool has_res, bool has_aux, const Tuning& t) {
+  const int kChunk = (up2_c(d) + d.cin) % 64 == 0 ? 64 : 32;
+  if (t.families & kFamTwoSourceNever) return "switched off (kFamTwoSourceNever)";
+  if (up2_c(d) <= 0) return "up2_c is 0";
+  if (d.ksize != 1 || d.stride != 1 || d.pad != 0) return "1x1 / stride 1 / pad 0 only";
+  if (has_res || has_aux || d.upsample2x) return "no residual, pre-add copy or upsampling store";
+  if (d.h % 2 || d.w % 2 || d.ho != d.h || d.wo != d.w) return "h and w must be even";
+  if (d.cin <= 0 || up2_c(d) % kChunk || d.cin % kChunk) return "up2_c and cin must be multiples of the K-chunk depth (64, or 32 when up2_c + cin is no multiple of 64)";
+  if (d.aux_c_offset % 8 || d.aux_c_total % 8 || d.aux_c_offset < 0 || d.aux_c_offset + up2_c(d) > d.aux_c_total) return "bad view of the half-resolution source";
+  if (d.kpad < up2_c(d) + d.cin) return "kpad < up2_c + cin";
+  if (conv_x2_bytes(d) >= kOobOffset) return "half-resolution source larger than 3.75 GiB";
+  if (!lds_epilogue_views(d, false, false) || (t.conv_debug & kCdNoLdsEpilogue)) return "output view needs the LDS-staged epilogue";
+  return nullptr;
+}
+
 struct SplitK {
   int splits = 1;
   float* ws = nullptr;
@@ -761,9 +814,10 @@
 };
 
 int conv2d_launch_ex(const void* x, const void* w, const float* bias, const void* res, void* y, void* y_aux, const YoloConvDesc* dp,
-                     const HeadDecodeArgs* hd, const SplitK& sk, hipStream_t s, int dt = YOLO_DT_BF16) {
+                     const HeadDecodeArgs* hd, const SplitK& sk, hipStream_t s, int dt = YOLO_DT_BF16, const void* x2 = nullptr) {
   YOLO_REQUIRE(x && w && bias && (y || hd) && dp, "conv: null pointer");
   const YoloConvDesc& d = *dp;
+  YOLO_REQUIRE((d.res_c_total < 0) == (x2 != nullptr), "conv: res_c_total %d %s a half-resolution source (yolo_conv2d_up2_fwd)", d.res_c_total, x2 ? "with" : "without");
   YOLO_REQUIRE(d.ksize == 1 || d.ksize == 3, "conv: ksize %d unsupported (1 or 3)", d.ksize);
   YOLO_REQUIRE(d.stride == 1 || d.stride == 2, "conv: stride %d unsupported", d.stride);
   YOLO_REQUIRE(d.cin > 0 && d.cin % 8 == 0, "conv: cin %d must be a positive multiple of 8", d.cin);
@@ -786,7 +840,13 @@
   YOLO_REQUIRE(M > 0 && M < 0x7fffffffL / 4, "conv: M out of range");
 
   const Tuning& t = tuning();
+  if (x2) {
+    const char* why = (hd || sk.splits > 1 || dt != YOLO_DT_BF16) ? "bf16 conv launches only" : up2_form_error(d, res != nullptr, y_aux != nullptr, t);
+    if (why) return yolo_set_error(YOLO_E_UNSUPPORTED, "conv: not the two-source form: %s", why);
+  }
   ConvArgs a = make_conv_args(x, w, bias, res, y, y_aux, d);
+  a.x2 = (const bf16_t*)x2;
+  a.x2_bytes = x2 ? (uint32_t)conv_x2_bytes(d) : 0u;
   a.debug = t.conv_debug;
   a.splits = sk.splits;
   a.ws = sk.ws;
@@ -800,6 +860,18 @@
     return launch_igemm_f16(choose_igemm_f16(d, res != nullptr, y_aux != nullptr, hd != nullptr, g_launch_cus), a, s);
   }
   const bool others = !hd && t.variant < 0 && std_out && lds_epilogue_views(d, res != nullptr, y_aux != nullptr) && !(t.conv_debug & kCdNoLdsEpilogue);
+  if (x2) {
+    if (t.variant < 0 && !(t.families & kFamStreamNever)) {
+      const int rc = launch_stream1x1(a, t.families & kFamStreamAlways ? 1 : 0, s);
+      if (rc != 1) return rc;
+    }
+    YoloConvDesc whole = d;
+    whole.cin += up2_c(d);
+    whole.in_c_total = whole.cin;
+    whole.res_c_total = whole.aux_c_total = whole.aux_c_offset = 0;
+    const int rc = launch_igemm_up2(choose_igemm(whole, false, false, false, 1, g_launch_cus, t), a, s);
+    return rc == 1 ? yolo_set_error(YOLO_E_UNSUPPORTED, "conv: not the two-source form: no such instance of the gather kernel") : rc;
+  }
   if (others && !(t.families & kFamT20Never) && a.splits <= 1) {
     const int rc = launch_t20_3x3(a, t.families & kFamT20Always ? 1 : 0, s);
     if (rc != 1) return rc;
@@ -894,7 +966,7 @@
   yolo_conv::g_pick_len = out_len;
   static const char dummy[16] = {0};
   const int rc = conv2d_launch_ex(dummy, dummy, (const float*)dummy, has_residual ? dummy : nullptr, (void*)dummy,
-                                  has_preadd ? (void*)dummy : nullptr, d, nullptr, SplitK(), nullptr, dt);
+                                  has_preadd ? (void*)dummy : nullptr, d, nullptr, SplitK(), nullptr, dt, d->res_c_total < 0 ? dummy : nullptr);
   yolo_conv::g_pick = nullptr;
   return rc;
 }
@@ -908,6 +980,16 @@
 extern "C" int yolo_conv2d_f16_fwd(const void* x, const void* w_packed, const float* bias, const void* residual, void* y,
                                    void* y_preadd, const YoloConvDesc* d, yolo_stream_t s) {
   return conv2d_launch_ex(x, w_packed, bias, residual, y, y_preadd, d, nullptr, SplitK(), (hipStream_t)s, YOLO_DT_F16);
+}
+
+extern "C" int yolo_conv2d_up2_fwd(const void* a_half, const void* x, const void* w_packed, const float* bias, void* y,
+                                   const YoloConvDesc* d, yolo_stream_t s) {
+  YOLO_REQUIRE(a_half && d && d->res_c_total < 0, "conv2d_up2: needs the half-resolution source and d->res_c_total = -up2_c < 0");
+  return conv2d_launch_ex(x, w_packed, bias, nullptr, y, nullptr, d, nullptr, SplitK(), (hipStream_t)s, YOLO_DT_BF16, a_half);
+}
+extern "C" int yolo_conv2d_up2_supported(const YoloConvDesc* d) {
+  char name[128];
+  return d && d->res_c_total < 0 && conv2d_pick(d, 0, 0, name, (int)sizeof(name), YOLO_DT_BF16) == 0;
 }
 
 extern "C" int yolo_conv2d_fwd(const void* x, const void* w_packed, const float* bias, const void* residual, void* y,
diff --git a/pytorch_yolo_amd/csrc/runtime.hip b/pytorch_yolo_amd/csrc/runtime.hip
--- a/pytorch_yolo_amd/csrc/runtime.hip
+++ b/pytorch_yolo_amd/csrc/runtime.hip
@@ -48,6 +48,10 @@
     int rc;
     switch (o.kind) {
       case YOLO_OP_CONV:
+        if (d.res_c_total < 0) {
+          rc = yolo_conv2d_up2_fwd(o.w_pre, o.x, o.w, o.bias, o.y, &d, s);
+          break;
+        }
         rc = o.splits >= 2 ? yolo_conv2d_splitk_fwd(o.x, o.w, o.bias, o.residual, o.y, o.y_aux, &d, o.splits, o.workspace, o.ws_bytes,
                                                     o.counters, s)
                            : yolo_conv2d_launch(o.x, o.w, o.bias, o.residual, o.y, o.y_aux, &d, (hipStream_t)s);
diff --git a/pytorch_yolo_amd/csrc/tuning.h b/pytorch_yolo_amd/csrc/tuning.h
--- a/pytorch_yolo_amd/csrc/tuning.h
+++ b/pytorch_yolo_amd/csrc/tuning.h
@@ -33,6 +33,7 @@
   kFamT20Never = 64,
   kFamStreamNever = 1024,
   kFamStreamAlways = 2048,
+  kFamTwoSourceNever = 4096,
 };
 
 enum : int {
diff --git a/pytorch_yolo_amd/diag.py b/pytorch_yolo_amd/diag.py
--- a/pytorch_yolo_amd/diag.py
+++ b/pytorch_yolo_amd/diag.py
@@ -128,4 +128,6 @@
         sub.residual = op.residual + m_out * op.conv.res_c_total * 2
     if op.y_aux:
         sub.y_aux = op.y_aux + m_out * op.conv.aux_c_total * 2
+    if op.kind == OP_CONV and op.conv.res_c_total < 0:
+        sub.w_pre = op.w_pre + first * (op.conv.h // 2) * (op.conv.w // 2) * op.conv.aux_c_total * 2
     return sub, x_off
diff --git a/pytorch_yolo_amd/emit.py b/pytorch_yolo_amd/emit.py
--- a/pytorch_yolo_amd/emit.py
+++ b/pytorch_yolo_amd/emit.py
@@ -108,7 +108,8 @@
     pack, plain = (K.pack_conv_weight_f32, OP_CONV_F32) if plan.f32 else (K.pack_conv_weight, OP_CONV)
     if plan.f16:
         pack, plain = K.pack_conv_weight_f16, OP_CONV_F16
-    wp, bp, kpad, cout_pad = pack(w, b, x.c)
+    a2 = L.up2
+    wp, bp, kpad, cout_pad = pack(w, b, x.c + (a2.c if a2 is not None else 0))
     res = nd.srcs[1] if nd.attrs["has_res"] else None
     aux = nd.outs[1] if len(nd.outs) > 1 else None
     d = K.conv_desc(n=x.n, h=x.h, w=x.w, cin=x.c, in_c_total=x.buf.c_total if x.buf is not None else x.c, in_c_offset=x.c_offset,
@@ -116,7 +117,7 @@
                     ksize=w.shape[2], stride=nd.attrs["stride"], act=_ACT[nd.attrs["act"]],
                     kpad=kpad, cout_pad=cout_pad, upsample2x=1 if L.up else 0,
                     out_dtype=DT_F32 if (plan.f32 or y.f32) else (DT_F16 if plan.f16 else DT_BF16), pad=nd.attrs.get("pad"),
-                    res=_slice_of(res), aux=_slice_of(aux))
+                    res=_slice_of(res), aux=_slice_of(aux), up2=(a2.c, a2.buf.c_total, a2.c_offset) if a2 is not None else (0, 0, 0))
     if not L.up and not L.pooled:
         d.ho, d.wo = y.h, y.w
     if L.reads_nchw:
@@ -127,7 +128,7 @@
         if kind == OP_CONV_F16 and os.environ.get("YOLO_FP16_T20", "1") != "0" and K.conv3x3_t20_f16_supported(d, res is not None, aux is not None):
             kind = OP_CONV_T20_F16
     op = _op(kind, x=None if L.reads_nchw else _ptr(x), y=_ptr(dst), residual=_ptr(res) if res is not None else None,
-             y_aux=_ptr(aux) if aux is not None else None, conv=d)
+             y_aux=_ptr(aux) if aux is not None else None, conv=d, w_pre=_ptr(a2) if a2 is not None else None)
     op.w, op.bias = _keep(plan, wp, bp)
     if kind == OP_CONV and os.environ.get("YOLO_SPLITK", "0") == "1":
         sp, wb, _ = K.conv2d_splitk_plan(d, res is not None, aux is not None)
@@ -242,6 +243,10 @@
 _CONVS = (OP_CONV, OP_CONV1_NCHW, OP_CONV1_POOL, OP_CONV_POOL, OP_HEAD_DECODE, OP_CONV_F32, OP_CONV_F16, OP_HEAD_DECODE_F16, OP_CONV_T20_F16)
 
 
+def _up2_c(op) -> int:
+    return K.up2_c(op.conv) if op.kind == OP_CONV else 0
+
+
 def conv_flops(op_array, n_ops: int, c_in: int) -> float:
     total = 0.0
     first = True
@@ -249,7 +254,7 @@
         op = op_array[i]
         d = op.conv
         if op.kind in _CONVS:
-            cin = c_in if first else d.cin
+            cin = c_in if first else d.cin + _up2_c(op)
             first = False
             total += 2.0 * d.n * d.ho * d.wo * d.cout * d.ksize * d.ksize * cin
         elif op.kind == OP_STEM:
@@ -274,6 +279,7 @@
         m_in, m_out = d.n * d.h * d.w, d.n * d.ho * d.wo
         if op.kind in _CONVS:
             x_b = m_in * (c_in * 4 if (first and op.kind in (OP_CONV1_NCHW, OP_CONV1_POOL)) else d.cin * (4 if op.kind == OP_CONV_F32 else 2))
+            x_b += m_in / 4 * _up2_c(op) * 2
             first = False
             pooled = 4 if op.kind in (OP_CONV1_POOL, OP_CONV_POOL) else 1
             y_b = m_out * d.cout * (4 if d.out_dtype == DT_F32 else 2) * (4 if d.upsample2x else 1) / pooled
@@ -281,7 +287,7 @@
                 y_b = 2.0 * m_out * d.cout * 4
                 if detect:
                     y_b = m_out * op.head_na * 8.0
-            total += x_b + y_b + d.cout * d.ksize * d.ksize * d.cin * 2
+            total += x_b + y_b + d.cout * d.ksize * d.ksize * (d.cin + _up2_c(op)) * 2
             total += (m_out * d.cout * 2 if op.residual else 0) + (m_out * d.cout * 2 if op.y_aux else 0)
         elif op.kind == OP_STEM:
             first = False
diff --git a/pytorch_yolo_amd/engine.py b/pytorch_yolo_amd/engine.py
--- a/pytorch_yolo_amd/engine.py
+++ b/pytorch_yolo_amd/engine.py
@@ -49,7 +49,7 @@
 class Plan(GuardedAlloc, _Runs):
     n_streams = 1
 
-    def __init__(self, rec: Recorder, device, n_class: int, img_size: int, precision: str = "bf16"):
+    def __init__(self, rec: Recorder, device, n_class: int, img_size: int, precision: str = "bf16", two_source: bool = False):
         if precision not in ("bf16", "fp32", "fp16"):
             raise ValueError(f"precision must be 'bf16', 'fp32' or 'fp16', got {precision!r}")
         self.f32 = precision == "fp32"
@@ -67,7 +67,8 @@
         self._graph = None
         self._static_out = None
         self.depth_first, self._x_patch = [], [(0, 0)]
-        self.launches = planner.fuse(rec, self.f32, n_class, self.f16)
+        self.two_source = two_source and precision == "bf16"
+        self.launches = planner.fuse(rec, self.f32, n_class, self.f16, self.two_source)
         self.fused_input = any(L.reads_nchw for L in self.launches)
         self._bufs = planner.place(rec, self.launches)
         self.shared_buffers = planner.alloc(rec, self.launches, self._bufs, self.f32, self._zeros, self.f16)
diff --git a/pytorch_yolo_amd/kernels.py b/pytorch_yolo_amd/kernels.py
--- a/pytorch_yolo_amd/kernels.py
+++ b/pytorch_yolo_amd/kernels.py
@@ -188,7 +188,7 @@
 
 
 def conv_desc(*, n, h, w, cin, in_c_total, in_c_offset, cout, out_c_total, out_c_offset, ksize, stride,
-              act, kpad, cout_pad, upsample2x=0, out_dtype=DT_BF16, res=(0, 0), aux=(0, 0), pad=None) -> YoloConvDesc:
+              act, kpad, cout_pad, upsample2x=0, out_dtype=DT_BF16, res=(0, 0), aux=(0, 0), pad=None, up2=(0, 0, 0)) -> YoloConvDesc:
     pad = (ksize - 1) // 2 if pad is None else pad
     d = YoloConvDesc()
     d.n, d.h, d.w, d.cin, d.in_c_total, d.in_c_offset = n, h, w, cin, in_c_total, in_c_offset
@@ -198,6 +198,8 @@
     d.kpad, d.cout_pad = kpad, cout_pad
     d.res_c_total, d.res_c_offset = res
     d.aux_c_total, d.aux_c_offset = aux
+    if up2[0]:
+        d.res_c_total, d.res_c_offset, d.aux_c_total, d.aux_c_offset = -up2[0], 0, up2[1], up2[2]
     return d
 
 
@@ -205,6 +207,19 @@
     buf = C.create_string_buffer(256)
     check(load().yolo_conv2d_pick(C.byref(desc), int(has_residual), int(has_preadd), buf, 256), "conv2d_pick")
     return buf.value.decode()
+
+
+def up2_c(desc: YoloConvDesc) -> int:
+    return -desc.res_c_total if desc.res_c_total < 0 else 0
+
+
+def conv2d_up2_supported(desc: YoloConvDesc) -> bool:
+    return bool(load().yolo_conv2d_up2_supported(C.byref(desc)))
+
+
+def conv2d_up2(a_half, x, w_packed, bias, y, desc: YoloConvDesc):
+    _need_cuda(a_half, x, w_packed, bias, y)
+    check(load().yolo_conv2d_up2_fwd(_ptr(a_half), _ptr(x), _ptr(w_packed), _ptr(bias), _ptr(y), C.byref(desc), stream_ptr()), "conv2d_up2")
 
 
 def head_decode_pick(desc: YoloConvDesc, na: int, nc: int, filter: bool = False) -> str:
diff --git a/pytorch_yolo_amd/models/yolo_base.py b/pytorch_yolo_amd/models/yolo_base.py
--- a/pytorch_yolo_amd/models/yolo_base.py
+++ b/pytorch_yolo_amd/models/yolo_base.py
@@ -110,6 +110,7 @@
         self._plans = {}
         self._tensors = None
         self.use_hip_graph = False
+        self.two_source = True
         self.n_streams = 2
         self.precision = os.environ.get("YOLO_PRECISION", "bf16")
 
@@ -163,7 +164,7 @@
                                "(there is no CPU fallback)")
         bs, c, h, w = x.shape
         n_streams = self.n_streams if (self.n_streams > 1 and bs % self.n_streams == 0 and bs // self.n_streams >= 4) else 1
-        key = (tuple(x.shape), x.device, n_streams, self.precision)
+        key = (tuple(x.shape), x.device, n_streams, self.precision, self.two_source)
         fp = self._fingerprint()
         if self.__dict__.get("_plans_fp") != fp:
             self._plans = {}
@@ -178,7 +179,7 @@
             def make(sub_bs):
                 rec = engine.Recorder(sub_bs, c, h, w)
                 self._trace(rec, rec.input)
-                return engine.Plan(rec, x.device, self.n_class, max(h, w), self.precision)
+                return engine.Plan(rec, x.device, self.n_class, max(h, w), self.precision, self.two_source)
             with torch.cuda.device(x.device):
                 plan = make(bs) if n_streams == 1 else engine.StreamedPlan(make, bs, n_streams, x.device)
             self._plans[key] = plan
diff --git a/pytorch_yolo_amd/planner.py b/pytorch_yolo_amd/planner.py
--- a/pytorch_yolo_amd/planner.py
+++ b/pytorch_yolo_amd/planner.py
@@ -25,11 +25,12 @@
     pooled: bool = False
     reads_nchw: bool = False
     layer: object = None
+    up2: Optional[Sym] = None
 
 
 class _Fusion:
 
-    def __init__(self, rec: Recorder, f32: bool, n_class: int, f16: bool = False):
+    def __init__(self, rec: Recorder, f32: bool, n_class: int, f16: bool = False, two_source: bool = False):
         env = os.environ.get
         self.rec, self.n_class = rec, n_class
         plain = f32 or f16
@@ -39,6 +40,7 @@
             "YOLO_FUSE_POOL", "YOLO_FUSE_STEM", "YOLO_FUSE_CONV1_S2"))
         self.head = not f32 and env("YOLO_FUSE_HEAD", "1") == "1"
         self.nchw = not plain
+        self.up2 = two_source and not plain
 
 
 def _ksize(nd):
@@ -56,12 +58,34 @@
     return ndp
 
 
+def _two_source_conv(fz, up):
+    a, u = up.srcs[0], up.outs[0]
+    cat = _only_consumer(u, "cat")
+    if not fz.up2 or cat is None or len(cat.srcs) != 2 or cat.srcs[0] is not u or a.f32:
+        return None
+    r = cat.srcs[1]
+    nd = _only_consumer(cat.outs[0], "conv")
+    if (nd is None or nd.srcs[0] is not cat.outs[0] or nd.attrs["has_res"] or len(nd.outs) != 1 or nd.outs[0].f32 or nd.attrs["stride"] != 1
+            or _ksize(nd) != 1 or r.f32 or (r.h, r.w) != (u.h, u.w)):
+        return None
+    cout = nd.attrs["weight"][0].shape[0]
+    d = K.conv_desc(n=r.n, h=r.h, w=r.w, cin=r.c, in_c_total=K.roundup(r.c, 8), in_c_offset=0, cout=cout, out_c_total=K.roundup(cout, 8),
+                    out_c_offset=0, ksize=1, stride=1, act=0, kpad=K.roundup(a.c + r.c, 64), cout_pad=K.roundup(cout, 128),
+                    up2=(a.c, K.roundup(a.c, 8), 0))
+    if not K.conv2d_up2_supported(d):
+        return None
+    return Launch("conv", nd, pre=(up, cat), src=r, dst=nd.outs[0], up2=a)
+
+
 def fuse_upsample(fz, nd):
     if nd.kind != "up":
         return None
     x = nd.srcs[0]
     if x.producer.kind != "conv" or len(x.consumers) != 1:
         raise RuntimeError("upsample must directly follow a conv with no other consumer")
+    two = _two_source_conv(fz, nd)
+    if two is not None:
+        return two
     return Launch("conv", x.producer, pre=(nd,), src=x.producer.srcs[0], dst=nd.outs[0], up=True)
 
 
@@ -168,8 +192,8 @@
          fuse_head)
 
 
-def fuse(rec: Recorder, f32: bool, n_class: int, f16: bool = False) -> List[Launch]:
-    fz = _Fusion(rec, f32, n_class, f16)
+def fuse(rec: Recorder, f32: bool, n_class: int, f16: bool = False, two_source: bool = False) -> List[Launch]:
+    fz = _Fusion(rec, f32, n_class, f16, two_source)
     claimed = {}
     for rule in RULES:
         for nd in rec.nodes:
@@ -191,6 +215,7 @@
     order = {id(nd): i for i, nd in enumerate(nodes)}
     by_node = {id(L.node): L for L in launches}
     swallowed = {id(m) for L in launches for m in L.pre}
+    unplaced = {id(m) for L in launches if L.up2 is not None for m in L.pre}
     bufs = []
 
     def own_buf(s: Sym):
@@ -198,6 +223,8 @@
         bufs.append(s.buf)
 
     for nd in nodes:
+        if id(nd) in unplaced:
+            continue
         if nd.kind == "cat":
             y = nd.outs[0]
             if y.buf is None:
@@ -218,7 +245,7 @@
                 raise RuntimeError("spp input already placed")
             x.buf, x.c_offset = y.buf, 3 * x.c
     for nd in nodes:
-        if nd.kind == "up" and nd.outs[0].buf is None:
+        if nd.kind == "up" and nd.outs[0].buf is None and id(nd) not in unplaced:
             own_buf(nd.outs[0])
     in_place = []
     for L in launches:
@@ -269,6 +296,7 @@
                 pinned.add(id(s_.buf))
     for L in launches:
         touch(L.src, order[id(L.node)])
+        touch(L.up2, order[id(L.node)])
         touch(L.dst, order[id(L.node)])
     return rng, pinned
 
```
